# liuyuan-pal/Gen6D

Hardware: AMD Instinct MI355X
Metric: query images/sec (detect+select+3x refine), 64 ref views (higher is better)
Workload: dtype f32

## Files before the change

gen6d_amd/csrc/conv_igemm.hip:

```cpp
#include "g6d_common.h"
#include <type_traits>
#include <stdlib.h>

#define LDS_K 36
#define BK 32
#ifndef G6D_ABLATE
#define G6D_ABLATE 0
#endif

bool g6d_wino_eligible(const G6dConv& d);
int g6d_wino_launch(const G6dConv& d, hipStream_t stream);
bool g6d_wino43_eligible(const G6dConv& d);
int g6d_wino43_launch(const G6dConv& d, hipStream_t stream);
bool g6d_conv_patch_eligible(const G6dConv& d);
int g6d_conv_patch_launch(const G6dConv& d, int M, hipStream_t stream);

namespace {

__device__ __forceinline__ f32x4 ldg(const float* __restrict__ base, int elem_off) {
  return *reinterpret_cast<const f32x4*>(reinterpret_cast<const char*>(base) + ((unsigned)elem_off << 2));
}

template <int BM, int BN, int WGM, int WGN, int MODE, int MM>
__global__ void __launch_bounds__(256, 2) conv_igemm_kernel(const G6dConv p, const int M, const int T,
                                                         const int nChunks, const int itersPerSplit,
                                                         const int totalIters, const int splits, const unsigned in_bytes,
                                                         const unsigned w_bytes, const unsigned mul_bytes, const int pm_hw,
                                                         const int pm_tiles, const int pm_ny_count) {
  extern __shared__ __attribute__((aligned(16))) float lds[];
  constexpr int WM = BM / WGM, WN = BN / WGN;
  constexpr int MT = WM / 32, NT = WN / 32;
  constexpr int RA = BM / 32, RB = BN / 32;
  constexpr int STAGE = (BM + BN) * LDS_K;
  constexpr bool AFF = MODE != 0, PER_N = MODE == 2 || MODE == 4, MUL = MODE == 3 || MODE == 4;

  const int tid = threadIdx.x;
  const int lane = tid & 63, wave = tid >> 6;
  const int wm = wave / WGN, wn = wave % WGN;
  const int li = lane & 31, lh = lane >> 5;
  const int lrow = tid >> 3, lseg = tid & 7;

  int pm_pos = 0, pm_tile = blockIdx.x, pm_ny = blockIdx.y;
  if (pm_hw > 0) {
    const int per = 8 * pm_ny_count * pm_hw, g = blockIdx.x / per, r = blockIdx.x - g * per;
    const int m8 = min(8, pm_tiles - 8 * g);
    const int r2 = r / m8;
    pm_tile = 8 * g + (r - r2 * m8);
    pm_pos = r2 / pm_ny_count; pm_ny = r2 - pm_pos * pm_ny_count;
  }
  const int m0 = pm_tile * BM, n0 = pm_ny * BN;
  auto row_m = [&](int r) { return pm_hw > 0 ? (m0 + r) * pm_hw + pm_pos : m0 + r; };
  int ky0 = 0, ky1 = p.kh - 1, kx0 = 0, kx1 = p.kw - 1;
  if (pm_hw > 0) {
    const int oy = pm_pos / p.Wo, ox = pm_pos - oy * p.Wo;
    ky0 = max(0, p.ph - oy); ky1 = min(p.kh - 1, p.Hi - 1 + p.ph - oy);
    kx0 = max(0, p.pw - ox); kx1 = min(p.kw - 1, p.Wi - 1 + p.pw - ox);
  }
  const int it_begin = blockIdx.z * itersPerSplit;
  const int it_end = pm_hw > 0 ? p.kd * (ky1 - ky0 + 1) * (kx1 - kx0 + 1) * nChunks : min(totalIters, it_begin + itersPerSplit);

  const int Cin = p.Cin, khw = p.kh * p.kw;
  const float* __restrict__ gsc = p.in_scale;
  const float* __restrict__ gsh = p.in_shift;
  const int relu = p.in_relu;

  const int pad_a = ((p.pd * p.Hi + p.ph) * p.Wi + p.pw) * p.ld_in;
  const int pad_m = (p.ph * p.Wi + p.pw) * Cin;
  unsigned amz[RA], amy[RA], amx[RA], avoff[RA], mvoff[MUL ? RA : 1];
  int nbase[PER_N ? RA : 1];
#pragma unroll
  for (int j = 0; j < RA; ++j) {
    const int m = row_m(lrow + 32 * j);
    amz[j] = amy[j] = amx[j] = 0u; avoff[j] = 0u;
    if constexpr (MUL) mvoff[j] = 0u;
    if constexpr (PER_N) nbase[j] = 0;
    if (m < M) {
      const int ow = m % p.Wo, t1 = m / p.Wo;
      const int oh = t1 % p.Ho, t2 = t1 / p.Ho;
      const int od = t2 % p.Do, n = t2 / p.Do;
      const int az0 = od * p.sd - p.pd, ay0 = oh * p.sh - p.ph, ax0 = ow * p.sw - p.pw;
      for (int k = 0; k < p.kd; ++k) amz[j] |= (unsigned)((unsigned)(az0 + k) < (unsigned)p.Di) << k;
      for (int k = 0; k < p.kh; ++k) amy[j] |= (unsigned)((unsigned)(ay0 + k) < (unsigned)p.Hi) << k;
      for (int k = 0; k < p.kw; ++k) amx[j] |= (unsigned)((unsigned)(ax0 + k) < (unsigned)p.Wi) << k;
      const int n_in = p.in_image_mod > 0 ? n % p.in_image_mod : n;
      avoff[j] = (unsigned)((((n_in * p.Di + az0) * p.Hi + ay0) * p.Wi + ax0) * p.ld_in + pad_a + 4 * lseg) << 2;
      if constexpr (MUL) {
        const int mg = p.mul_group_images > 0 ? n / p.mul_group_images : 0;
        mvoff[j] = (unsigned)(((mg * p.Hi + ay0) * p.Wi + ax0) * Cin + pad_m + 4 * lseg) << 2;
      }
      if constexpr (PER_N) nbase[j] = (n / p.in_affine_per_n) * Cin;
    }
  }
  unsigned bvoff[RB];
#pragma unroll
  for (int j = 0; j < RB; ++j) {
    const int co = n0 + lrow + 32 * j;
    bvoff[j] = co < p.Cout ? (unsigned)(co * T * Cin + 4 * lseg) << 2 : 0x80000000u;
  }
  const auto rs_in = __builtin_amdgcn_make_buffer_rsrc(const_cast<float*>(p.in) - pad_a, 0, in_bytes, 0x00020000);
  const auto rs_w = __builtin_amdgcn_make_buffer_rsrc(const_cast<float*>(p.weight), 0, w_bytes, 0x00020000);
  const auto rs_mul = __builtin_amdgcn_make_buffer_rsrc(const_cast<float*>(MUL ? p.mul - pad_m : p.in), 0, mul_bytes, 0x00020000);
  const unsigned thr_last = 4 * lseg < Cin - 32 * (nChunks - 1) ? 0xffffffffu : 0u;

  f32x16 acc[MT][NT];
#pragma unroll
  for (int i = 0; i < MT; ++i)
#pragma unroll
    for (int j = 0; j < NT; ++j)
#pragma unroll
      for (int r = 0; r < 16; ++r) acc[i][j][r] = 0.f;

  f32x4 ra[2][RA], rm[2][MUL ? RA : 1], rb[2][RB], rsc[2][PER_N ? RA : 1], rsh[2][PER_N ? RA : 1];
  unsigned va[2][AFF ? RA : 1];

  int lt = it_begin;
  int cc = pm_hw > 0 ? 0 : it_begin / T;
  const int tap0 = it_begin - cc * T;
  int kz = pm_hw > 0 ? 0 : tap0 / khw, ky = pm_hw > 0 ? ky0 : (tap0 - kz * khw) / p.kw, kx = pm_hw > 0 ? kx0 : tap0 - kz * khw - ky * p.kw;
  auto advance = [&]() {
    lt += 1;
    kx += 1; const bool w1 = kx > kx1; kx = w1 ? kx0 : kx;
    ky += w1; const bool w2 = ky > ky1; ky = w2 ? ky0 : ky;
    kz += w2; const bool w3 = kz == p.kd; kz = w3 ? 0 : kz;
    cc += w3;
  };

  typedef unsigned u32x4 __attribute__((ext_vector_type(4)));
  auto bload = [&](const auto& rs, unsigned voff, int soff) {
    return __builtin_bit_cast(f32x4, __builtin_bit_cast(u32x4, __builtin_amdgcn_raw_buffer_load_b128(rs, voff, soff, 0)));
  };
  int toff = 0, moff = 0, cch = 0, woff = 0;
  unsigned cm = 0;
  bool cv = false;
  auto begin_step = [&](auto S) {
    constexpr int s = decltype(S)::value;
    const bool live = lt < it_end;
    cch = cc * BK + 4 * lseg;
    cv = (cch < Cin) & live;
    cm = live ? (cc == nChunks - 1 ? thr_last : 0xffffffffu) : 0u;
    toff = live ? (((kz * p.Hi + ky) * p.Wi + kx) * p.ld_in + cc * BK) << 2 : 0;
    moff = live ? ((ky * p.Wi + kx) * Cin + cc * BK) << 2 : 0;
    woff = live ? (((kz * p.kh + ky) * p.kw + kx) * Cin + cc * BK) << 2 : 0;
    if constexpr (AFF && !PER_N) { rsc[s][0] = ldg(gsc, cv ? cch : 0); rsh[s][0] = ldg(gsh, cv ? cch : 0); }
  };
  auto load_a = [&](auto S, int j) {
    constexpr int s = decltype(S)::value;
    const unsigned m = (unsigned)__builtin_amdgcn_sbfe(amz[j], kz, 1) & (unsigned)__builtin_amdgcn_sbfe(amy[j], ky, 1) &
                       (unsigned)__builtin_amdgcn_sbfe(amx[j], kx, 1) & cm;
    if constexpr (AFF) va[s][j] = m;
    ra[s][j] = bload(rs_in, (avoff[j] & m) | (~m & 0x80000000u), toff);
    if constexpr (MUL) rm[s][j] = bload(rs_mul, (mvoff[j] & m) | (~m & 0x80000000u), moff);
    if constexpr (PER_N) { rsc[s][j] = ldg(gsc, cv ? nbase[j] + cch : 0); rsh[s][j] = ldg(gsh, cv ? nbase[j] + cch : 0); }
  };
  auto load_b = [&](auto S, int j) {
    constexpr int s = decltype(S)::value;
    rb[s][j] = bload(rs_w, bvoff[j], woff);
  };
  auto store_a = [&](auto S, float* As, int j) {
    constexpr int s = decltype(S)::value;
    f32x4 v = ra[s][j];
    if constexpr (MUL) v *= rm[s][j];
    if constexpr (AFF) {
      v = v * rsc[s][PER_N ? j : 0] + rsh[s][PER_N ? j : 0];
      if (relu) {
#pragma unroll
        for (int e = 0; e < 4; ++e) asm("v_max_f32 %0, 0, %1" : "=v"(v[e]) : "v"(v[e]));
      }
      u32x4 b = __builtin_bit_cast(u32x4, v);
      b &= va[s][j];
      v = __builtin_bit_cast(f32x4, b);
    }
    *reinterpret_cast<f32x4*>(As + (lrow + 32 * j) * LDS_K + 4 * lseg) = v;
  };
  auto store_b = [&](auto S, float* Bs, int j) {
    constexpr int s = decltype(S)::value;
    *reinterpret_cast<f32x4*>(Bs + (lrow + 32 * j) * LDS_K + 4 * lseg) = rb[s][j];
  };

  f32x4 dummy = {0.f, 0.f, 0.f, 0.f};
  f32x4 fa[2][MT], fb[2][NT];
  auto read_frags = [&](const float* As, const float* Bs, int kc) {
#pragma unroll
    for (int i = 0; i < MT; ++i)
      fa[kc & 1][i] = *reinterpret_cast<const f32x4*>(As + (wm * WM + i * 32 + li) * LDS_K + kc * 8 + 4 * lh);
#pragma unroll
    for (int j = 0; j < NT; ++j)
      fb[kc & 1][j] = *reinterpret_cast<const f32x4*>(Bs + (wn * WN + j * 32 + li) * LDS_K + kc * 8 + 4 * lh);
  };
  constexpr bool ONE_ACC = MT * NT == 1;
  f32x16 acc_odd;
  if constexpr (ONE_ACC) {
#pragma unroll
    for (int r = 0; r < 16; ++r) acc_odd[r] = 0.f;
  }
  auto mfma_q = [&](int q) {
    const int kc = q / (4 * MT * NT), r = q % (4 * MT * NT);
    const int sidx = r / (MT * NT), i = (r % (MT * NT)) / NT, j = r % NT;
    if constexpr (ONE_ACC) {
      if (sidx & 1) { acc_odd = __builtin_amdgcn_mfma_f32_32x32x2f32(fa[kc & 1][0][sidx], fb[kc & 1][0][sidx], acc_odd, 0, 0, 0); return; }
    }
    acc[i][j] = __builtin_amdgcn_mfma_f32_32x32x2f32(fa[kc & 1][i][sidx], fb[kc & 1][j][sidx], acc[i][j], 0, 0, 0);
  };

  constexpr int NMFMA = MT * NT * 16, NP = NMFMA / 2, QPC = NMFMA / 4 / 2;
  constexpr int NROW = RA + RB;
  static_assert(NP >= NROW, "tile too small for the piece schedule");
  auto k_step = [&](auto PAR, const float* As, const float* Bs, float* An, float* Bn) {
    constexpr int par = decltype(PAR)::value;
    using SL = std::integral_constant<int, par>;
    using SS = std::integral_constant<int, par ^ 1>;
    if constexpr (MM != 0) {
#pragma unroll
      for (int j = 0; j < RA; ++j) load_a(SL{}, j);
#pragma unroll
      for (int j = 0; j < RB; ++j) load_b(SL{}, j);
#pragma unroll
      for (int kp = 0; kp < 2; ++kp) {
        f32x4 a0[MT], a1[MT], b0[NT], b1[NT];
#pragma unroll
        for (int i = 0; i < MT; ++i) {
          a0[i] = *reinterpret_cast<const f32x4*>(As + (wm * WM + i * 32 + li) * LDS_K + (2 * kp) * 8 + 4 * lh);
          a1[i] = *reinterpret_cast<const f32x4*>(As + (wm * WM + i * 32 + li) * LDS_K + (2 * kp + 1) * 8 + 4 * lh);
        }
#pragma unroll
        for (int j = 0; j < NT; ++j) {
          b0[j] = *reinterpret_cast<const f32x4*>(Bs + (wn * WN + j * 32 + li) * LDS_K + (2 * kp) * 8 + 4 * lh);
          b1[j] = *reinterpret_cast<const f32x4*>(Bs + (wn * WN + j * 32 + li) * LDS_K + (2 * kp + 1) * 8 + 4 * lh);
        }
#pragma unroll
        for (int i = 0; i < MT; ++i)
#pragma unroll
          for (int j = 0; j < NT; ++j) acc[i][j] = g6d_mfma_lowp<MM>(a0[i], a1[i], b0[j], b1[j], acc[i][j]);
      }
#pragma unroll
      for (int j = 0; j < RA; ++j) store_a(SS{}, An, j);
#pragma unroll
      for (int j = 0; j < RB; ++j) store_b(SS{}, Bn, j);
      advance(); begin_step(SS{});
      return;
    }
    read_frags(As, Bs, 0);
#pragma unroll
    for (int pc = 0; pc < NP; ++pc) {
      if (pc % QPC == 0 && pc / QPC < 3 && (G6D_ABLATE < 2 || G6D_ABLATE >= 6)) read_frags(As, Bs, pc / QPC + 1);
      mfma_q(2 * pc); mfma_q(2 * pc + 1);
      if (G6D_ABLATE < 1 || G6D_ABLATE >= 6) {
        if (pc < RA) load_a(SL{}, pc); else if (pc < NROW) load_b(SL{}, pc - RA);
        const int sr = pc - (NP - NROW);
        if (sr >= 0) {
          if (G6D_ABLATE == 6) {
            if (sr < RA) dummy += ra[par ^ 1][sr]; else dummy += rb[par ^ 1][sr - RA];
          } else if (sr < RA) store_a(SS{}, An, sr); else store_b(SS{}, Bn, sr - RA);
        }
        if (pc == NP - 1) { advance(); begin_step(SS{}); }
      }
      __builtin_amdgcn_sched_barrier(0);
    }
  };

  if (it_begin < it_end) {
    using S0 = std::integral_constant<int, 0>;
    using S1 = std::integral_constant<int, 1>;
    begin_step(S0{});
#pragma unroll
    for (int j = 0; j < RA; ++j) load_a(S0{}, j);
#pragma unroll
    for (int j = 0; j < RB; ++j) load_b(S0{}, j);
    advance(); begin_step(S1{});
#pragma unroll
    for (int j = 0; j < RA; ++j) load_a(S1{}, j);
#pragma unroll
    for (int j = 0; j < RB; ++j) load_b(S1{}, j);
#pragma unroll
    for (int j = 0; j < RA; ++j) store_a(S0{}, lds, j);
#pragma unroll
    for (int j = 0; j < RB; ++j) store_b(S0{}, lds + BM * LDS_K, j);
    advance(); begin_step(S0{});
    __syncthreads();
    float* L0 = lds; float* L1 = lds + STAGE;
    for (int it = it_begin; it < it_end; it += 2) {
      k_step(S0{}, L0, L0 + BM * LDS_K, L1, L1 + BM * LDS_K);
      if (G6D_ABLATE < 3 || G6D_ABLATE == 6) __syncthreads();
      if (it + 1 < it_end) {
        k_step(S1{}, L1, L1 + BM * LDS_K, L0, L0 + BM * LDS_K);
        if (G6D_ABLATE < 3 || G6D_ABLATE == 6) __syncthreads();
      }
    }
    if (G6D_ABLATE == 6) acc[0][0][0] += dummy[0] + dummy[1] + dummy[2] + dummy[3];
  }

  if constexpr (ONE_ACC) {
#pragma unroll
    for (int r = 0; r < 16; ++r) acc[0][0][r] += acc_odd[r];
  }
  const int Cout = p.Cout;
  if (splits > 1) {
    constexpr int TILE = BM * BN;
    constexpr int PIECES = MT * NT * 4;
    constexpr int ZU = 16 / PIECES;
    const int ntiles = gridDim.x * gridDim.y, tile = blockIdx.y * gridDim.x + blockIdx.x;
    float* part = p.workspace + G6D_WS_COUNTERS + (size_t)tile * TILE + tid * 4;
    const size_t zstride = (size_t)ntiles * TILE;
    float* mine = part + blockIdx.z * zstride;
#pragma unroll
    for (int i = 0; i < MT; ++i)
#pragma unroll
      for (int j = 0; j < NT; ++j)
#pragma unroll
        for (int q = 0; q < 4; ++q)
          g6d_store_wt(mine + ((i * NT + j) * 4 + q) * 1024,
                       f32x4{acc[i][j][4 * q], acc[i][j][4 * q + 1], acc[i][j][4 * q + 2], acc[i][j][4 * q + 3]});
    if (!g6d_split_arrive(reinterpret_cast<int*>(p.workspace) + tile, splits, reinterpret_cast<int*>(lds))) return;
    __syncthreads();
    f32x4 sum[PIECES];
#pragma unroll
    for (int k = 0; k < PIECES; ++k) sum[k] = f32x4{0.f, 0.f, 0.f, 0.f};
    for (int z0 = 0; z0 < splits; z0 += ZU) {
      f32x4 v[ZU][PIECES];
#pragma unroll
      for (int u = 0; u < ZU; ++u) {
        const float* src = part + (size_t)min(z0 + u, splits - 1) * zstride;
#pragma unroll
        for (int k = 0; k < PIECES; ++k) v[u][k] = *reinterpret_cast<const f32x4*>(src + k * 1024);
      }
#pragma unroll
      for (int u = 0; u < ZU; ++u)
        if (z0 + u < splits) {
#pragma unroll
          for (int k = 0; k < PIECES; ++k) sum[k] += v[u][k];
        }
    }
#pragma unroll
    for (int i = 0; i < MT; ++i)
#pragma unroll
      for (int j = 0; j < NT; ++j)
#pragma unroll
        for (int q = 0; q < 4; ++q) {
          const f32x4 t = sum[(i * NT + j) * 4 + q];
          acc[i][j][4 * q] = t[0]; acc[i][j][4 * q + 1] = t[1]; acc[i][j][4 * q + 2] = t[2]; acc[i][j][4 * q + 3] = t[3];
        }
  }

  const bool do_stats = p.stats != nullptr;
  const int rpg = p.stat_rows_per_group;
  const int mlast = pm_hw > 0 ? min(row_m(BM - 1), M - pm_hw + pm_pos) : min(m0 + BM, M) - 1;
  const int g0 = rpg > 0 ? row_m(0) / rpg : 0;
  const bool one_group = rpg <= 0 || (mlast / rpg) == g0;
  float* sred = lds;
  if (do_stats && one_group) {
    for (int i = tid; i < BN * 2; i += 256) sred[i] = 0.f;
    __syncthreads();
  }
#pragma unroll
  for (int j = 0; j < NT; ++j) {
    const int col = n0 + wn * WN + j * 32 + li;
    const bool cval = col < Cout;
    const float bv = (p.bias && cval) ? p.bias[col] : 0.f;
    float s1 = 0.f, s2 = 0.f;
#pragma unroll
    for (int i = 0; i < MT; ++i) {
#pragma unroll
      for (int r = 0; r < 16; ++r) {
        const int row = row_m(wm * WM + i * 32 + (r & 3) + 8 * (r >> 2) + 4 * lh);
        float v = apply_act(acc[i][j][r] + bv, p.out_act);
        if (row < M && cval) {
          p.out[(size_t)row * p.ld_out + col] = v;
          if (do_stats) {
            if (one_group) { s1 += v; s2 += v * v; }
            else {
              double* st = p.stats + ((size_t)(row / rpg) * Cout + col) * 2;
              atomicAdd(st, (double)v); atomicAdd(st + 1, (double)v * v);
            }
          }
        }
      }
    }
    if (do_stats && one_group) {
      s1 += __shfl_xor(s1, 32, 64);
      s2 += __shfl_xor(s2, 32, 64);
      if (lh == 0) {
        atomicAdd(&sred[(wn * WN + j * 32 + li) * 2], s1);
        atomicAdd(&sred[(wn * WN + j * 32 + li) * 2 + 1], s2);
      }
    }
  }
  if (do_stats && one_group) {
    __syncthreads();
    if (tid < BN && n0 + tid < Cout) {
      double* st = p.stats + ((size_t)g0 * Cout + n0 + tid) * 2;
      atomicAdd(st, (double)sred[tid * 2]);
      atomicAdd(st + 1, (double)sred[tid * 2 + 1]);
    }
  }
  if (do_stats && p.fin_scale) {
    __syncthreads();
    g6d_finalize_stats(g6d_fin_of(p), gridDim.x * gridDim.y, reinterpret_cast<int*>(lds));
  }
}

bool igemm_position_major(const G6dConv& d, int bm, int splits) {
  const int pm = (int)g6d_knob(G6D_KNOB_CONV_PM);
  return pm != 0 && (pm == 2 || d.in_scale != nullptr) && splits == 1 && d.Di == 1 && d.Do == 1 && d.kd == 1 && d.sh == 1 && d.sw == 1 && d.Ho == d.Hi &&
         d.Wo == d.Wi && d.Ho * d.Wo <= 64 && d.Ho * d.Wo > 1 && (d.kh > 1 || d.kw > 1) && d.kh == 2 * d.ph + 1 && d.kw == 2 * d.pw + 1 &&
         d.N >= 4 * bm;
}

template <int BM, int BN, int WGM, int WGN, int MODE, int MM>
int launch_mm(const G6dConv& d, int M, int T, int nChunks, int splits, hipStream_t stream) {
  const int total = T * nChunks;
  const int ips = (total + splits - 1) / splits;
  splits = (total + ips - 1) / ips;
  const bool pm = igemm_position_major(d, BM, splits);
  const int pm_hw = pm ? d.Ho * d.Wo : 0, pm_tiles = pm ? (d.N + BM - 1) / BM : 0;
  const int ny = (d.Cout + BN - 1) / BN;
  dim3 grid(pm ? pm_hw * pm_tiles * ny : (M + BM - 1) / BM, pm ? 1 : ny, splits);
  const size_t lds_bytes = 2 * (size_t)(BM + BN) * LDS_K * sizeof(float);
  g6d_allow_lds(reinterpret_cast<const void*>(&conv_igemm_kernel<BM, BN, WGM, WGN, MODE, MM>), (int)lds_bytes);
  const long long pad_a = ((long long)(d.pd * d.Hi + d.ph) * d.Wi + d.pw) * d.ld_in, pad_m = (long long)(d.ph * d.Wi + d.pw) * d.Cin;
  const long long n_in = d.in_image_mod > 0 ? d.in_image_mod : d.N;
  const long long n_mul = d.mul_group_images > 0 ? (d.N + d.mul_group_images - 1) / d.mul_group_images : 1;
  const unsigned in_bytes = (unsigned)((n_in * d.Di * d.Hi * d.Wi * d.ld_in + pad_a) * 4);
  const unsigned w_bytes = (unsigned)((long long)d.Cout * T * d.Cin * 4);
  const unsigned mul_bytes = (unsigned)((n_mul * d.Hi * d.Wi * d.Cin + pad_m) * 4);
  hipLaunchKernelGGL((conv_igemm_kernel<BM, BN, WGM, WGN, MODE, MM>), grid, dim3(256), lds_bytes, stream, d, M, T, nChunks,
                     ips, total, splits, in_bytes, w_bytes, mul_bytes, pm_hw, pm_tiles, ny);
  return g6d_check_launch("conv_igemm");
}

template <int BM, int BN, int WGM, int WGN, int MODE>
int launch_mode(const G6dConv& d, int M, int T, int nChunks, int splits, hipStream_t stream) {
  if (d.math_mode == 1) return launch_mm<BM, BN, WGM, WGN, MODE, 1>(d, M, T, nChunks, splits, stream);
  if (d.math_mode == 2) return launch_mm<BM, BN, WGM, WGN, MODE, 2>(d, M, T, nChunks, splits, stream);
  return launch_mm<BM, BN, WGM, WGN, MODE, 0>(d, M, T, nChunks, splits, stream);
}

template <int BM, int BN, int WGM, int WGN>
int launch_cfg(const G6dConv& d, int M, int T, int nChunks, int splits, hipStream_t stream) {
  if (d.mul) return d.in_affine_per_n ? launch_mode<BM, BN, WGM, WGN, 4>(d, M, T, nChunks, splits, stream)
                                      : launch_mode<BM, BN, WGM, WGN, 3>(d, M, T, nChunks, splits, stream);
  if (!d.in_scale) return launch_mode<BM, BN, WGM, WGN, 0>(d, M, T, nChunks, splits, stream);
  if (d.in_affine_per_n) return launch_mode<BM, BN, WGM, WGN, 2>(d, M, T, nChunks, splits, stream);
  return launch_mode<BM, BN, WGM, WGN, 1>(d, M, T, nChunks, splits, stream);
}

constexpr int NARROW_RUN = 8;
__global__ void __launch_bounds__(256) conv_narrow_kernel(const float* __restrict__ in, const float* __restrict__ w, const float* __restrict__ bias,
                                                         float* __restrict__ out, int NH, int H, int W, int Cin, int ld_in, int Cout, int ld_out,
                                                         int act, int runs_per_row, int nruns) {
  const int lane = threadIdx.x & 63;
  const int c4 = lane * 4;
  const bool on = c4 < Cin;
  f32x4 wr[4][9];
#pragma unroll
  for (int co = 0; co < 4; ++co)
#pragma unroll
    for (int t = 0; t < 9; ++t)
      wr[co][t] = (on && co < Cout) ? *reinterpret_cast<const f32x4*>(w + ((long)co * 9 + t) * Cin + c4) : f32x4{0.f, 0.f, 0.f, 0.f};
  const int wave = __builtin_amdgcn_readfirstlane((int)((blockIdx.x * blockDim.x + threadIdx.x) >> 6)), nwaves = (gridDim.x * blockDim.x) >> 6;
  const f32x4 zero = {0.f, 0.f, 0.f, 0.f};
  for (int run = wave; run < nruns; run += nwaves) {
    const int g = run / runs_per_row, x0 = (run - g * runs_per_row) * NARROW_RUN;
    const int y = g % H;
    const float* rowp[3];
    bool rv[3];
#pragma unroll
    for (int ky = 0; ky < 3; ++ky) {
      const int yy = y + ky - 1;
      rv[ky] = yy >= 0 && yy < H;
      rowp[ky] = in + ((long)(g + ky - 1) * W) * ld_in + c4;
    }
    auto column = [&](int x, f32x4 (&col)[3]) {
      const bool xv = x >= 0 && x < W;
#pragma unroll
      for (int ky = 0; ky < 3; ++ky) col[ky] = (on && xv && rv[ky]) ? *reinterpret_cast<const f32x4*>(rowp[ky] + (long)x * ld_in) : zero;
    };
    f32x4 win[3][3];
    column(x0 - 1, win[0]);
    column(x0, win[1]);
#pragma unroll
    for (int i = 0; i < NARROW_RUN; ++i) {
      const int x = x0 + i;
      column(x + 1, win[2]);
      float acc[4];
#pragma unroll
      for (int co = 0; co < 4; ++co) {
        f32x4 a = zero;
#pragma unroll
        for (int ky = 0; ky < 3; ++ky)
#pragma unroll
          for (int kx = 0; kx < 3; ++kx) a += win[kx][ky] * wr[co][3 * ky + kx];
        acc[co] = (a[0] + a[1]) + (a[2] + a[3]);
      }
#pragma unroll
      for (int off = 32; off >= 1; off >>= 1)
#pragma unroll
        for (int co = 0; co < 4; ++co) acc[co] += __shfl_xor(acc[co], off, 64);
      if (lane == 0 && x < W) {
#pragma unroll
        for (int co = 0; co < 4; ++co)
          if (co < Cout) {
            float v = acc[co] + (bias ? bias[co] : 0.f);
            if (act == 1) v = fmaxf(v, 0.f);
            else if (act == 2) v = v > 0.f ? v : 0.1f * v;
            out[((long)g * W + x) * ld_out + co] = v;
          }
      }
#pragma unroll
      for (int ky = 0; ky < 3; ++ky) { win[0][ky] = win[1][ky]; win[1][ky] = win[2][ky]; }
    }
  }
}

bool conv_narrow_eligible(const G6dConv& d) {
  return g6d_knob(G6D_KNOB_CONV_NARROW) != 0 && d.Cout <= 4 && d.Cin <= 256 && d.kd == 1 && d.kh == 3 && d.kw == 3 && d.sd == 1 && d.sh == 1 && d.sw == 1 &&
         d.pd == 0 && d.ph == 1 && d.pw == 1 && d.Di == 1 && d.Do == 1 && d.Ho == d.Hi && d.Wo == d.Wi && !d.mul && !d.in_scale && !d.stats &&
         !d.in_image_mod && d.out_act >= 0 && d.out_act <= 2;
}

int conv_narrow_launch(const G6dConv& d, hipStream_t stream) {
  const int rpr = (d.Wi + NARROW_RUN - 1) / NARROW_RUN;
  const long nruns = (long)d.N * d.Hi * rpr;
  if (nruns >= (1l << 31)) { g6d_set_error("conv (narrow): too many pixel runs"); return G6D_EINVAL; }
  const int blocks = (int)((nruns + 3) / 4 < 2048 ? (nruns + 3) / 4 : 2048);
  hipLaunchKernelGGL(conv_narrow_kernel, dim3(blocks), dim3(256), 0, stream, d.in, d.weight, d.bias, d.out, d.N * d.Hi, d.Hi, d.Wi, d.Cin, d.ld_in, d.Cout,
                     d.ld_out, d.out_act, rpr, (int)nruns);
  return g6d_check_launch("conv_narrow");
}

}

extern "C" int g6d_conv_plan(const G6dConv* desc) {
  if (!desc) return G6D_EINVAL;
  if (conv_narrow_eligible(*desc)) return 4;
  if (g6d_wino43_eligible(*desc)) return 3;
  if (g6d_wino_eligible(*desc)) return 2;
  const bool use_patch = g6d_knob(G6D_KNOB_CONV_PATCH) != 0;
  return (use_patch && g6d_conv_patch_eligible(*desc)) ? 1 : 0;
}

extern "C" int g6d_conv_igemm(const G6dConv* desc, g6d_stream_t stream_) {
  if (!desc) return G6D_EINVAL;
  const G6dConv& d = *desc;
  hipStream_t stream = reinterpret_cast<hipStream_t>(stream_);
  if (!d.in || !d.weight || !d.out) { g6d_set_error("conv: null pointer"); return G6D_EINVAL; }
  if (d.math_mode < 0 || d.math_mode > 2) { g6d_set_error("conv: math_mode must be 0 (fp32), 1 (bf16) or 2 (fp16)"); return G6D_EINVAL; }
  if (d.N <= 0 || d.Cin <= 0 || d.Cout <= 0 || d.Do <= 0 || d.Ho <= 0 || d.Wo <= 0 || d.kd <= 0 || d.kh <= 0 || d.kw <= 0) {
    g6d_set_error("conv: bad shape"); return G6D_EINVAL;
  }
  if ((d.Cin & 3) || (d.ld_in & 3) || d.ld_in < d.Cin || d.ld_out < d.Cout) { g6d_set_error("conv: Cin/ld_in must be multiples of 4"); return G6D_EINVAL; }
  if (!g6d_aligned16(d.in) || !g6d_aligned16(d.weight) || (d.mul && !g6d_aligned16(d.mul)) ||
      (d.in_scale && (!g6d_aligned16(d.in_scale) || !d.in_shift || !g6d_aligned16(d.in_shift)))) {
    g6d_set_error("conv: operand pointers must be 16-byte aligned"); return G6D_EINVAL;
  }
  if (d.mul && !d.in_scale) { g6d_set_error("conv: mul requires in_scale/in_shift"); return G6D_EINVAL; }
  if (d.in_affine_per_n < 0 || d.in_image_mod < 0 || d.mul_group_images < 0 || (d.mul_group_images > 0 && !d.mul) ||
      d.in_image_mod > d.N) {
    g6d_set_error("conv: in_affine_per_n / in_image_mod / mul_group_images must be >= 0 (mul_group_images needs mul; in_image_mod <= N)");
    return G6D_EINVAL;
  }
  if ((long long)(d.mul_group_images > 0 ? (d.N + d.mul_group_images - 1) / d.mul_group_images : 1) * d.Hi * d.Wi * d.Cin >= (1ll << 29)) {
    g6d_set_error("conv: multiplier tensor exceeds 2^31 bytes"); return G6D_EINVAL;
  }
  if (d.fin_scale && (!d.stats || !d.fin_shift || !d.fin_counter || d.fin_count <= 0 || d.fin_groups <= 0)) {
    g6d_set_error("conv: fin_scale needs stats, fin_shift, fin_counter, fin_count > 0 and fin_groups"); return G6D_EINVAL;
  }
  if ((long long)(d.in_image_mod > 0 ? d.in_image_mod : d.N) * d.Di * d.Hi * d.Wi * d.ld_in + ((long long)(d.pd * d.Hi + d.ph) * d.Wi + d.pw) * d.ld_in >= (1ll << 29) ||
      (long long)d.Cout * d.kd * d.kh * d.kw * d.Cin >= (1ll << 29) || d.kd > 32 || d.kh > 32 || d.kw > 32) {
    g6d_set_error("conv: tensor exceeds 2^31 bytes (buffer-load offsets) or kernel extent > 32"); return G6D_EINVAL;
  }
  const long long Mll = (long long)d.N * d.Do * d.Ho * d.Wo;
  if (Mll > (1ll << 30)) { g6d_set_error("conv: M too large"); return G6D_EINVAL; }
  const int M = (int)Mll;
  if (conv_narrow_eligible(d)) return conv_narrow_launch(d, stream);
  if (g6d_wino43_eligible(d)) return g6d_wino43_launch(d, stream);
  if (g6d_wino_eligible(d)) return g6d_wino_launch(d, stream);
  const bool use_patch = g6d_knob(G6D_KNOB_CONV_PATCH) != 0;
  if (use_patch && g6d_conv_patch_eligible(d)) return g6d_conv_patch_launch(d, M, stream);
  const int T = d.kd * d.kh * d.kw;
  const int nChunks = (d.Cin + BK - 1) / BK;
  const int total = T * nChunks;

  int bm = 128, bn = d.Cout <= 32 ? 32 : (d.Cout <= 64 ? 64 : 128);
  if (bn == 128 && (d.mul || (d.in_scale && d.in_affine_per_n))) bn = 64;
  if (M <= 64 && d.Cout > 32) { bm = 64; bn = 64; }
  const bool tile_policy = g6d_knob(G6D_KNOB_TILE_POLICY) != 0;
  bool no_split = false;
  if (tile_policy && d.Cout > 32 && bm == 128 && d.split_k <= 0) {
    const long long blocks128 = (long long)((M + 127) / 128) * ((d.Cout + bn - 1) / bn);
    const long long blocks64 = (long long)((M + 63) / 64) * ((d.Cout + 63) / 64);
    if (blocks128 < 256) {
      if (blocks64 >= 256) { bm = 64; bn = 64; no_split = true; }
      else if (M >= 2048) { bm = 64; bn = 64; }
      else if (M <= 1024 && bn == 128) bn = 64;
    }
  }
  const long long blocks = (long long)((M + bm - 1) / bm) * ((d.Cout + bn - 1) / bn);

  int splits = d.split_k;
  if (splits <= 0) {
    splits = 1;
    const int split_target = (int)g6d_knob(G6D_KNOB_SPLIT_TARGET);
    if (blocks < (split_target < 256 ? split_target : 256) && total >= 8 && !no_split) {
      splits = (int)((split_target + blocks - 1) / blocks);
      if (splits > total / 4) splits = total / 4;
      if (splits > 64) splits = 64;
      if (splits < 1) splits = 1;
    }
  }
  if (splits > total) splits = total;
  if (splits > 1) {
    const size_t per = (size_t)blocks * bm * bn * sizeof(float);
    const size_t room = d.workspace && d.workspace_bytes > G6D_WS_COUNTER_BYTES ? d.workspace_bytes - G6D_WS_COUNTER_BYTES : 0;
    if (room < (size_t)splits * per || blocks > G6D_WS_COUNTERS) {
      if (d.split_k > 1) { g6d_set_error("conv: workspace too small for forced split_k"); return G6D_ENOSPC; }
      splits = blocks > G6D_WS_COUNTERS ? 1 : (int)(room / per);
      if (splits < 2) splits = 1;
    }
  }
  if (bm == 64) return launch_cfg<64, 64, 2, 2>(d, M, T, nChunks, splits, stream);
  if (bn == 32) return launch_cfg<128, 32, 4, 1>(d, M, T, nChunks, splits, stream);
  if (bn == 64) return launch_cfg<128, 64, 2, 2>(d, M, T, nChunks, splits, stream);
  return launch_cfg<128, 128, 2, 2>(d, M, T, nChunks, splits, stream);
}
```

gen6d_amd/lib.py:

```python
import ctypes as C
import os

_HERE = os.path.dirname(os.path.abspath(__file__))
LIB_PATH = os.path.join(_HERE, "libgen6d_hip.so")

G6D_ERRORS = {-1: "G6D_EINVAL", -2: "G6D_ENOSPC", -3: "G6D_ELAUNCH"}


class G6dWinoSeg(C.Structure):
    _fields_ = [("in_", C.c_void_p), ("out_full", C.c_void_p), ("out_pool", C.c_void_p),
                ("N", C.c_int32), ("H", C.c_int32), ("W", C.c_int32), ("ld_in", C.c_int32), ("ld_full", C.c_int32), ("ld_pool", C.c_int32)]


class G6dConv16Seg(C.Structure):
    _fields_ = [("in_", C.c_void_p), ("out_full", C.c_void_p), ("out_pool", C.c_void_p),
                ("N", C.c_int32), ("D", C.c_int32), ("H", C.c_int32), ("W", C.c_int32), ("ld_in", C.c_int32), ("ld_full", C.c_int32),
                ("ld_pool", C.c_int32)]


class G6dRange16(C.Structure):
    _fields_ = [("exps", C.c_void_p), ("rec", C.c_void_p), ("slot_in", C.c_int32), ("slot_out", C.c_int32)]


class G6dCorrSeg(C.Structure):
    _fields_ = [("in_", C.c_void_p), ("out", C.c_void_p), ("H", C.c_int32), ("W", C.c_int32), ("ld_in", C.c_int32), ("ld_out", C.c_int32),
                ("N", C.c_int32), ("reserved_", C.c_int32)]


class G6dFrame(C.Structure):
    _fields_ = [("plane0", C.c_void_p), ("plane1", C.c_void_p), ("pitch0", C.c_int32), ("pitch1", C.c_int32), ("width", C.c_int32),
                ("height", C.c_int32), ("format", C.c_int32), ("rotate", C.c_int32), ("matrix", C.c_int32), ("slot", C.c_int32),
                ("out_w", C.c_int32), ("out_h", C.c_int32), ("K", C.c_float * 9)]


class G6dMesh(C.Structure):
    _fields_ = [("nodes", C.c_void_p), ("nx", C.c_int32), ("ny", C.c_int32), ("step_log2", C.c_int32), ("reserved", C.c_int32)]


class G6dSink(C.Structure):
    _fields_ = [("plane0", C.c_void_p), ("plane1", C.c_void_p), ("pitch0", C.c_int32), ("pitch1", C.c_int32), ("width", C.c_int32),
                ("height", C.c_int32), ("format", C.c_int32), ("matrix", C.c_int32), ("slot", C.c_int32), ("pic_w", C.c_int32),
                ("pic_h", C.c_int32), ("thickness", C.c_int32), ("dot_radius", C.c_int32), ("line_rgb", C.c_int32), ("dot_rgb", C.c_int32),
                ("box", C.c_int32)]


class G6dConv(C.Structure):
    _fields_ = [
        ("in_", C.c_void_p), ("mul", C.c_void_p), ("in_scale", C.c_void_p), ("in_shift", C.c_void_p),
        ("weight", C.c_void_p), ("bias", C.c_void_p), ("out", C.c_void_p), ("stats", C.c_void_p),
        ("workspace", C.c_void_p), ("workspace_bytes", C.c_size_t),
        ("N", C.c_int32), ("Di", C.c_int32), ("Hi", C.c_int32), ("Wi", C.c_int32), ("Cin", C.c_int32), ("ld_in", C.c_int32),
        ("Do", C.c_int32), ("Ho", C.c_int32), ("Wo", C.c_int32), ("Cout", C.c_int32), ("ld_out", C.c_int32),
        ("kd", C.c_int32), ("kh", C.c_int32), ("kw", C.c_int32),
        ("sd", C.c_int32), ("sh", C.c_int32), ("sw", C.c_int32),
        ("pd", C.c_int32), ("ph", C.c_int32), ("pw", C.c_int32),
        ("in_relu", C.c_int32), ("in_affine_per_n", C.c_int32), ("out_act", C.c_int32),
        ("stat_rows_per_group", C.c_int32), ("split_k", C.c_int32), ("math_mode", C.c_int32),
        ("weight_wino", C.c_void_p),
        ("fin_scale", C.c_void_p), ("fin_shift", C.c_void_p), ("fin_counter", C.c_void_p),
        ("fin_count", C.c_double), ("fin_eps", C.c_double), ("fin_groups", C.c_int32),
        ("in_image_mod", C.c_int32), ("mul_group_images", C.c_int32), ("reserved_", C.c_int32),
        ("weight_wino16", C.c_void_p), ("weight_wino43", C.c_void_p),
    ]


_P, _I, _F, _D = C.c_void_p, C.c_int, C.c_float, C.c_double

SIGNATURES = {
    "g6d_marker": [_I, _P],
    "g6d_conv_igemm": [C.POINTER(G6dConv), _P],
    "g6d_conv_plan": [C.POINTER(G6dConv)],
    "g6d_corr2d_patch": [_P, _I, _I, _I, _I, _P, _I, _I, _I, _P, _I, _P, C.c_size_t, _I, _P],
    "g6d_corr2d_patch_multi": [_P, _I, _I, _P, _I, _I, _I, _P, C.c_size_t, _I, _P],
    "g6d_corr2d_wino_multi": [_P, _I, _I, _P, _I, _I, _P, C.c_size_t, _P],
    "g6d_corr2d_patch16_multi": [_P, _I, _I, _P, _I, _I, _I, _P, C.c_size_t, _I, _P],
    "g6d_stats_finalize": [_P, _I, _D, _D, _P, _P, _P],
    "g6d_affine_act_pool": [_P, _I, _P, _P, _I, _I, _I, _I, _I, _I, _I, _P, _I, _P],
    "g6d_upsample_bilinear": [_P, _I, _P, _P, _I, _I, _I, _I, _I, _I, _P, _I, _P],
    "g6d_bias_relu_pool_nchw": [_P, _P, _I, _I, _I, _I, _I, _I, _P, _P],
    "g6d_vgg_conv1_pool": [_P, _I, _I, _I, _P, _P, _I, _I, _P, _P],
    "g6d_vgg_conv1_pool_nhwc": [_P, _I, _I, _I, _P, _P, _I, _I, _P, _P],
    "g6d_vgg_conv1_pool_nhwc16": [_P, _I, _I, _I, _P, _P, _I, _I, _P, _P, _P, _I, _P],
    "g6d_conv16_direct_multi": [_P, _I, _I, _P, _I, _F, _P, _I, _I, _I, _I, _I, _I, _P, _I, _P],
    "g6d_corr16_multi": [_P, _I, _I, _P, _F, _I, _I, _I, _P],
    "g6d_product_split16": [_P, _P, _P, _P, _P, _I, _I, _I, _I, _I, _P],
    "g6d_affine_split16": [_P, _I, _P, _P, _I, _I, _I, _I, _I, _I, _I, _P, _I, _P],
    "g6d_vgg_conv1_pool_nhwc16_ex": [_P, _I, _I, _I, _P, _P, _I, _I, _P, _P, _P, _I, _P, _P],
    "g6d_conv16_direct_multi_ex": [_P, _I, _I, _P, _I, _F, _P, _I, _I, _I, _I, _I, _I, _P, _I, _P, _P],
    "g6d_corr16_multi_ex": [_P, _I, _I, _P, _F, _I, _I, _I, _P, _P],
    "g6d_product_split16_ex": [_P, _P, _P, _P, _P, _I, _I, _I, _I, _I, _P, _P],
    "g6d_affine_split16_ex": [_P, _I, _P, _P, _I, _I, _I, _I, _I, _I, _I, _P, _I, _P, _P],
    "g6d_conv16_direct_plan": [_P, _I, _I, _P, _I, _I, _I, _I, _I, _I, _P, _I],
    "g6d_affine_split16_to": [_P, _I, _P, _P, _I, _I, _I, _I, _I, _I, _I, _P, _I, _I, _I, _I, _P, _P],
    "g6d_upsample_bilinear_split16": [_P, _I, _P, _P, _I, _I, _I, _I, _I, _I, _P, _I, _I, _I, _I, _P, _P],
    "g6d_l2norm_split16": [_P, _I, _I, _I, _P, _I, _P, _P],
    "g6d_vgg_conv1_pool_nhwc_norm": [_P, _I, _I, _I, _P, _P, _I, _I, _P, _P, _P, _P],
    "g6d_wino_conv3x3": [_P, _I, _I, _I, _I, _I, _P, _P, _I, _I, _P, _I, _P, _I, _P, C.c_size_t, _P],
    "g6d_wino_conv3x3_multi": [_P, _I, _I, _P, _P, _I, _I, _P, C.c_size_t, _P],
    "g6d_wino16_conv3x3_multi": [_P, _I, _I, _P, _P, _I, _I, _I, _P, C.c_size_t, _P],
    "g6d_wino43_conv3x3_multi": [_P, _I, _I, _P, _P, _I, _I, _P, C.c_size_t, _P],
    "g6d_corr2d_wino43_multi": [_P, _I, _I, _P, _I, _I, _P, C.c_size_t, _P],
    "g6d_l2norm_rows": [_P, _I, _I, _I, _P],
    "g6d_nchw_to_nhwc": [_P, _I, _I, _I, _I, _I, _P, _I, _P],
    "g6d_selector_ref_sums": [_P, _I, _I, _I, _P, _P, _P],
    "g6d_selector_prod_affine": [_P, _P, _P, _I, _I, _I, _D, _P, _P, _P],
    "g6d_selector_scan": [_P, _P, _I, _I, _I, _P, _P, _P],
    "g6d_selector_levels": [_I, _I, _P, _P, _P, _P, _P, _I, _I, _I, _D, _P, _P, _P, _P, _P],
    "g6d_refiner_volume": [_P, _P, _P, _P, _I, _I, _I, _I, _I, _I, _I, _P, _P, _P],
    "g6d_refiner_volume_kp": [_P, _P, _P, _P, _P, _P, _I, _I, _I, _I, _I, _I, _I, _P, _P, _I, _P],
    "g6d_refiner_volume_kp_pairs": [_P, _P, _P, _P, _P, _P, _I, _I, _I, _I, _I, _I, _I, _P, _P, _I, _P, _P, _P],
    "g6d_detector_assemble": [_P, _P, _P, _I, _I, _I, C.POINTER(C.c_float), _F, _I, _I, _I, _I, _P, _I, _P],
    "g6d_detector_score_mlp_max": [_P, _I, _I, _I, _P, _P, _P, _P, _P, _P],
    "g6d_detector_decode": [_P, _I, _P, _I, _P, _I, _I, _I, _I, _P, _I, _P],
    "g6d_resize_bilinear_pyramid": [_P, _I, _I, _I, _I, C.POINTER(C.c_int), C.POINTER(C.c_int), C.POINTER(C.c_void_p), _P],
    "g6d_zero_bytes": [_P, C.c_size_t, _P],
    "g6d_vps_norm": [_P, _I, _P, _I, _I, _I, _P],
    "g6d_max_an_add": [_P, _I, _I, _I, _I, _P, _P, _I, _I, _P],
    "g6d_attention": [_P, _P, _P, _I, _I, _I, _I, _P, _I, _I, _P],
    "g6d_layernorm": [_P, _I, _I, _I, _P, _P, _F, _P, _I, _P],
    "g6d_affine_act_add": [_P, _I, _P, _P, _I, _P, _I, _I, _I, _P, _I, _I, _P],
    "g6d_linear_gemv": [_P, _I, _I, _P, _P, _I, _I, _P, _P],
    "g6d_linear_gemv_batch": [_P, _I, _I, _P, _P, _I, _I, _P, _P, C.c_size_t, _P],
    "g6d_chain_crop_from_detection": [_P, _F, _P, _I, _P],
    "g6d_chain_pose_from_selection": [_P, _P, _P, _I, _P, _P, _P, _P, _P, _P, _I, _P],
    "g6d_chain_refine_prepare": [_P, _P, _P, _F, _F, _P, _P, _I, _I, _P, _P, _F, _P, _I, _P],
    "g6d_chain_refine_update": [_P, _P, _P, _P, _I, _P, _P, _I, _P],
    "g6d_warp_batch": [_P, _P, _P, _I, _I, _I, _I, _P, _P, _I, _I, _P],
    "g6d_warp_perspective": [_P, _I, _I, _I, C.POINTER(C.c_float), _P, _I, _I, _I, _F, _P],
    "g6d_track_gather": [_P, _P, _P, _P, _I, _P],
    "g6d_track_commit": [_P, _P, _P, _I, _P, _I, _F, _P, _P, _P, _P, _P, _I, _P],
    "g6d_track_gate": [_P, _P, _P, _P, _I, _P],
    "g6d_track_health": [_P, _P, _P, _P, _I, _I, _P, _I, _P, _D, _I, _D, _D, _D, _D, _D, _D, _P, _P, _P, _P, _I, _P],
    "g6d_track_verify": [_P, _P, _P, _P, _P, _D, _D, _D, _D, _I, _P, _P, _I, _P],
    "g6d_frame_ingest": [_P, _I, _P, _I, _I, _I, _P, _P],
    "g6d_sizeof_frame_desc": [],
    "g6d_frame_ingest_mesh": [_P, _P, _I, _P, _I, _I, _I, _P, _P],
    "g6d_sizeof_mesh_desc": [],
    "g6d_track_corners": [_P, _P, _P, _P, _P, _P, _I, _P],
    "g6d_frame_emit": [_P, _I, _P, _I, _I, _I, _P, _P, _P],
    "g6d_sizeof_sink_desc": [],
    "g6d_frame_emit_source": [_P, _I, _P, _I, _P, _P, _I, _I, _I, _I, _P],
}

_lib = None


def load():
    global _lib
    if _lib is not None:
        return _lib
    if not os.path.exists(LIB_PATH):
        raise RuntimeError(f"{LIB_PATH} is missing: build it with `python __graft_entry__.py` "
                           "(make -C gen6d_amd/csrc). There is no fallback path.")
    import torch
    lib = C.CDLL(LIB_PATH)
    for name, args in SIGNATURES.items():
        fn = getattr(lib, name)
        fn.argtypes = args
        fn.restype = C.c_int
    lib.g6d_abi_version.restype = C.c_int
    lib.g6d_sizeof_conv_desc.restype = C.c_int
    if lib.g6d_sizeof_conv_desc() != C.sizeof(G6dConv):
        raise RuntimeError("libgen6d_hip.so: G6dConv layout differs from the ctypes binding (stale build?)")
    if lib.g6d_sizeof_frame_desc() != C.sizeof(G6dFrame):
        raise RuntimeError("libgen6d_hip.so: G6dFrame layout differs from the ctypes binding (stale build?)")
    if lib.g6d_sizeof_mesh_desc() != C.sizeof(G6dMesh):
        raise RuntimeError("libgen6d_hip.so: G6dMesh layout differs from the ctypes binding (stale build?)")
    if lib.g6d_sizeof_sink_desc() != C.sizeof(G6dSink):
        raise RuntimeError("libgen6d_hip.so: G6dSink layout differs from the ctypes binding (stale build?)")
    lib.g6d_last_error.restype = C.c_char_p
    lib.g6d_set_knob.argtypes, lib.g6d_set_knob.restype = [C.c_char_p, C.c_double], C.c_int
    lib.g6d_get_knob.argtypes, lib.g6d_get_knob.restype = [C.c_char_p], C.c_double
    lib.g6d_reset_knobs.argtypes, lib.g6d_reset_knobs.restype = [], None
    _lib = lib
    return lib


def set_knob(name, value):
    check(load().g6d_set_knob(name.encode(), float(value)), f"g6d_set_knob({name})")


def get_knob(name):
    return load().g6d_get_knob(name.encode())


def reset_knobs():
    load().g6d_reset_knobs()


def check(rc, what):
    if rc != 0:
        msg = load().g6d_last_error().decode()
        raise RuntimeError(f"{what} failed: {G6D_ERRORS.get(rc, rc)} ({msg})")
```

gen6d_amd/network/refiner.py:

```python
import numpy as np
import torch
import torch.nn.functional as F

from .. import ops, specs
from .backbone import pack_trunk, trunk_features
from .operator import pose_apply_th
from .params import ParamBank, fold_vgg

F43_MIN_QUERIES = 4
FEATNET_F43_LAYERS = {("conv1", 0), ("conv_out", 0), ("conv_out", 3)}
FEATNET_PAIR_BRANCHES = ("conv0", "conv1", "conv2", "conv_out")
VOLUME_PAIR_LAYERS = ("mean_embed", "var_embed", "conv0", "conv2")
VOLUME_F43_LAYERS = ("conv0",)
MAX_BATCH = 32
_K3, _P3 = (3, 3, 3), (1, 1, 1)
_K2, _P2 = (1, 3, 3), (0, 1, 1)


_LIN = {}


def _linspace(sn, dev):
    key = (sn, str(dev))
    if key not in _LIN:
        _LIN[key] = torch.linspace(-1, 1, sn, dtype=torch.float32, device=dev)
    return _LIN[key]


class RefFeatureCache:

    def __init__(self, max_entries=2048):
        from collections import OrderedDict
        self.store, self.max_entries = OrderedDict(), max_entries
        self.hits = self.misses = 0

    def get(self, key):
        f = self.store.get(key)
        if f is None:
            self.misses += 1
            return None
        self.store.move_to_end(key)
        self.hits += 1
        return f

    def put(self, key, feat):
        self.store[key] = feat
        while len(self.store) > self.max_entries:
            self.store.popitem(last=False)

    def clear(self):
        self.store.clear()
        self.hits = self.misses = 0

    @property
    def hit_rate(self):
        return self.hits / max(1, self.hits + self.misses)


class VolumeRefiner(ParamBank):
    default_cfg = {"refiner_sample_num": 32, "ref_feat_cache_deg": 0.0, "lowp_keep_fp32": (), "lowp_only": None}

    def __init__(self, cfg):
        self.cfg = {**self.default_cfg, **cfg}
        super().__init__(specs.refiner_rows())
        self.ref_database = None
        self.ref_ids = None
        self.feat_cache = RefFeatureCache()

    def load_state_dict(self, *a, **k):
        self.feat_cache.clear()
        return super().load_state_dict(*a, **k)

    def _mm(self, *names):
        only = self.cfg.get("lowp_only")
        keep = self.cfg.get("lowp_keep_fp32") or ()
        fp32 = (not any(n in only for n in names)) if only is not None else any(n in keep for n in names)
        return ops.math_mode("fp32" if fp32 else None, inherit_if_none=True)

    def angle_step(self):
        return float(np.radians(self.cfg.get("ref_feat_cache_deg") or 0.0))

    def cached_ref_feats(self, keys, make_imgs):
        with ops.math_mode(self.cfg.get("math_mode"), inherit_if_none=True):
            keys = [(k, ops.MATH_MODE) for k in keys]
            got = [self.feat_cache.get(k) for k in keys]
            miss = [i for i, f in enumerate(got) if f is None]
            feats = self.run_feature_net(make_imgs(miss), f43=False) if miss else None
        if miss:
            for j, i in enumerate(miss):
                got[i] = feats[j].clone()
                self.feat_cache.put(keys[i], got[i])
        return torch.stack(got, 0)

    def _pack(self):
        if self._packed is None:
            pk = {"vgg": pack_trunk(fold_vgg(self, "feature_net.backbone.features"))}
            for name in ("conv0", "conv1", "conv2", "conv_out"):
                pk[name] = [self.conv_w(f"feature_net.{name}.{i}", wino_kd=1, f43=(name, i) in FEATNET_F43_LAYERS) for i in (0, 3)]
            for name in ("mean_embed", "var_embed", "conv5"):
                pk["v_" + name] = [self.conv_w(f"volume_net.{name}.{i}", wino_kd=0 if name == "conv5" else 3, f43=True) for i in (0, 3)]
            for name in ("conv0", "conv1", "conv2", "conv3", "conv4"):
                pk["v_" + name] = self.conv_w(f"volume_net.{name}.0", wino_kd=3 if name in ("conv0", "conv2", "conv4") else 0,
                                              f43=name in VOLUME_F43_LAYERS)
            w = self.p("regressor.fc.0.0.weight")
            pk["fc0"] = (w.reshape(512, 512, 64).permute(0, 2, 1).reshape(512, 32768).contiguous(),
                         self.p("regressor.fc.0.0.bias").contiguous())
            pk["fc1"] = (self.p("regressor.fc.1.0.weight").contiguous(), self.p("regressor.fc.1.0.bias").contiguous())
            heads = ("fcr", "fct", "fcs")
            pk["heads"] = (torch.cat([self.p(f"regressor.{h}.weight") for h in heads], 0).contiguous(),
                           torch.cat([self.p(f"regressor.{h}.bias") for h in heads], 0).contiguous())
            self._packed = pk
        return self._packed

    def run_feature_net(self, imgs, f43=None):
        pk = self._pack()
        n, _, h, w = imgs.shape
        dev = imgs.device
        big = (n >= F43_MIN_QUERIES * 7) if f43 is None else bool(f43)
        rng = self._pair_rng()
        on16 = self._featnet_pair_branches(n, h, w) if (big and rng is not None) else ()
        with self._mm("trunk"):
            f3, f5, f7 = trunk_features(pk["vgg"], imgs, ("c3", "c5", "c7_pre"), False, f43=big, rng=rng, pairs=self.pairs_on)

        def tap(name, f, slot):
            if name in on16:
                return ops.l2norm_split16(f[:, 0], 3, rng=(rng, rng.slot(slot)))
            ops.l2norm_rows(f)
            return f

        def pair(name, x):
            if name in on16:
                return pair16(name, x)
            (w0, b0), (w1, b1) = pk[name]
            u0, u1 = pk[name][0].u, pk[name][1].u
            v0, v1 = (pk[name][0].u43, pk[name][1].u43) if big else (None, None)
            _, _, hh, ww, _ = x.shape
            y0 = torch.empty((n, 1, hh, ww, w0.shape[0]), dtype=torch.float32, device=dev)
            s0 = ops.new_stats(n, w0.shape[0], dev)
            y1 = torch.empty((n, 1, hh, ww, w1.shape[0]), dtype=torch.float32, device=dev)
            s1 = ops.new_stats(n, w1.shape[0], dev)
            sc0, sh0 = ops.conv(x, w0, b0, y0, ksize=_K2, pad=_P2, stats=s0, rows_per_group=hh * ww, w_wino=u0, w_wino43=v0, finalize=hh * ww)
            sc1, sh1 = ops.conv(y0, w1, b1, y1, ksize=_K2, pad=_P2, in_scale=sc0, in_shift=sh0, in_relu=True, per_n=True,
                                stats=s1, rows_per_group=hh * ww, w_wino=u1, w_wino43=v1, finalize=hh * ww)
            return y1, sc1, sh1

        def pair16(name, x):
            _, hh, ww, _, _ = x.shape

            def conv16(layer, xin):
                co = layer[0].shape[0]
                y = torch.empty((n, 1, hh, ww, co), dtype=torch.float32, device=dev)
                st = ops.new_stats(n, co, dev)
                ops.conv16_direct_multi([xin], layer.w16(3), layer[1], relu=False, full=torch.float32, stats=st, rows_per_group=hh * ww,
                                        out_full=[y[:, 0]])
                return (y,) + ops.stats_finalize(st, hh * ww)

            y0, sc0, sh0 = conv16(pk[name][0], x)
            mid = ops.affine_split16(y0, sc0, sh0, 1, True, False, 3, rng=(rng, rng.slot(f"featnet.{name}.mid")))
            return conv16(pk[name][1], mid)

        hq, wq = h // 4, w // 4
        cat16 = "conv_out" in on16
        cat = ops.new_map16(n, hq, wq, 192, 3, dev, rng=(rng, rng.slot("featnet.cat"))) if cat16 else \
            torch.empty((n, 1, hq, wq, 192), dtype=torch.float32, device=dev)

        def branch(name, f, slot, c_off, factor):
            y, sc, sh = pair(name, tap(name, f, slot))
            if cat16:
                if factor == 1:
                    ops.affine_split16_to(y, sc, sh, 1, False, 3, cat, c_off)
                else:
                    ops.upsample_bilinear_split16(y, cat, c_off, factor, sc, sh, 1, 3)
            elif factor == 1:
                ops.affine_act_pool(y, cat[..., c_off:c_off + 64], sc, sh, per_n=True)
            else:
                ops.upsample_bilinear(y, cat[..., c_off:c_off + 64], factor, sc, sh, per_n=True)

        with self._mm("featnet"):
            ops.fork_join([lambda: branch("conv0", f3, "featnet.f3", 0, 1), lambda: branch("conv1", f5, "featnet.f5", 64, 2),
                           lambda: branch("conv2", f7, "featnet.f7", 128, 4)], dev)
            y, sc, sh = pair("conv_out", cat)
        out = torch.empty((n, 1, hq, wq, 128), dtype=torch.float32, device=dev)
        ops.affine_act_pool(y, out, sc, sh, per_n=True)
        return out.view(n, hq, wq, 128)

    def _featnet_pair_branches(self, n, h, w):
        key = (n, h, w)
        memo = self.__dict__.setdefault("_featnet16", {})
        if key not in memo:
            shapes = {"conv0": (4, 256, 64, 64), "conv1": (8, 512, 256, 64), "conv2": (16, 512, 256, 64), "conv_out": (4, 192, 128, 128)}

            def fits(name):
                d, ci, cm, co = shapes[name]
                hh, ww = h // d, w // d
                return all(ops.conv16_direct_plan(n, hh, ww, a, b, 3, stats_rows=hh * ww) in (1, 2) for a, b in ((ci, cm), (cm, co)))
            memo[key] = tuple(name for name in FEATNET_PAIR_BRANCHES if h % 16 == 0 and w % 16 == 0 and fits(name))
        return memo[key]

    def volume_pair_route(self, qn, sn):
        if qn < F43_MIN_QUERIES or self._pair_rng() is None or not {"mean_embed", "var_embed"} <= set(VOLUME_PAIR_LAYERS):
            return False
        memo = self.__dict__.setdefault("_volume16", {})
        key = (qn, sn, tuple(VOLUME_PAIR_LAYERS))
        if key not in memo:
            shapes = [(sn, 256, 64), (sn, 128, 64), (sn, 64, 64)] + ([(sn, 128, 64)] if "conv0" in VOLUME_PAIR_LAYERS else []) + \
                ([(sn // 2, 128, 128)] if "conv2" in VOLUME_PAIR_LAYERS else [])
            memo[key] = all(ops.conv16_direct_plan(qn, s, s, ci, co, 3, stats_rows=s ** 3, D=s) == 1 for s, ci, co in shapes)
        return memo[key]

    def feature_volumes(self, feats, ref_Ks, ref_poses, K_in, pose_in, h_in, w_in, sn):
        dev = feats.device
        lin = _linspace(sn, dev)
        C = feats.shape[-1]
        args = (feats, ref_Ks.contiguous(), ref_poses.contiguous(), K_in.contiguous(), pose_in.contiguous(), lin, h_in, w_in)
        if feats.dim() == 5 and self.volume_pair_route(feats.shape[0], sn):
            rng = self._pair_rng()
            return ops.refiner_volume_kp_pairs(*args, rng_mean=(rng, rng.slot("volume.mean_in")), rng_std=(rng, rng.slot("volume.std")))
        lead = (feats.shape[0],) if feats.dim() == 5 else ()
        mean_in = torch.empty(lead + (sn ** 3, 2 * C), dtype=torch.float32, device=dev)
        std = torch.empty(lead + (sn ** 3, C), dtype=torch.float32, device=dev)
        return ops.refiner_volume_kp(*args, mean_in, std)

    def run_volume_net(self, mean_in, std, sn):
        pk = self._pack()
        pairs_in = isinstance(mean_in, ops.PairMap)
        dev = mean_in.data.device if pairs_in else mean_in.device
        batched = pairs_in or mean_in.dim() == 3
        qn = mean_in.shape[0] if batched else 1
        pn = 1 if qn > 1 else 0

        def c3(x, wb, out, stride=1, aff=None, stats_c=None, count=None):
            st = ops.new_stats(qn, stats_c, dev) if stats_c else None
            sc, sh = aff if aff is not None else (None, None)
            return ops.conv(x, wb[0], wb[1], out, ksize=_K3, stride=(stride,) * 3, pad=_P3, in_scale=sc, in_shift=sh,
                            in_relu=aff is not None, per_n=pn if aff is not None else 0, stats=st,
                            rows_per_group=pn * (count or 0) if stats_c else 0,
                            w_wino=getattr(wb, "u", None) if stride == 1 else None,
                            w_wino43=getattr(wb, "u43", None) if (stride == 1 and qn >= F43_MIN_QUERIES) else None,
                            finalize=count if stats_c else None)

        def buf(s, c):
            return torch.empty((qn, s, s, s, c), dtype=torch.float32, device=dev)

        vox = sn ** 3
        rng = self._pair_rng() if pairs_in else None
        cat16 = pairs_in and "conv0" in VOLUME_PAIR_LAYERS
        cat = ops.new_map16(qn * sn, sn, sn, 128, 3, dev, rng=(rng, rng.slot("volume.cat"))) if cat16 else buf(sn, 128)

        def c16(layer, xin, y, stats_c=None, count=vox):
            st = ops.new_stats(qn, stats_c, dev) if stats_c else None
            ops.conv16_direct_multi([xin], layer.w16(3, layout=2), layer[1], relu=False, full=torch.float32, kd=3, stats=st,
                                    rows_per_group=count if stats_c else 0, out_full=[y])
            return ops.stats_finalize(st, count) if stats_c else None

        def embed(name, x, c_off):
            if pairs_in:
                return embed16(name, x, c_off)
            y = buf(sn, 64)
            aff = c3(x, pk[name][0], y, stats_c=64, count=vox)
            c3(y, pk[name][1], cat[..., c_off:c_off + 64], aff=aff)

        def embed16(name, x, c_off):
            y0 = buf(sn, 64)
            sc, sh = c16(pk[name][0], x, y0, stats_c=64)
            mid = ops.affine_split16(y0.view(qn * sn, 1, sn, sn, 64), sc, sh, sn, True, False, 3, rng=(rng, rng.slot(f"volume.{name[2:]}.mid")))
            if not cat16:
                c16(pk[name][1], mid.view(qn, sn, sn, sn, 2, 64), cat[..., c_off:c_off + 64])
                return
            y1 = buf(sn, 64)
            c16(pk[name][1], mid.view(qn, sn, sn, sn, 2, 64), y1)
            ops.affine_split16_to(y1.view(qn * sn, 1, sn, sn, 64), None, None, 0, False, 3, cat, c_off)

        with self._mm("embed"):
            embed("v_mean_embed", mean_in.view(qn, sn, sn, sn, 2, 256) if pairs_in else mean_in.view(qn, sn, sn, sn, 256), 0)
            embed("v_var_embed", std.view(qn, sn, sn, sn, 2, 128) if pairs_in else std.view(qn, sn, sn, sn, 128), 64)
        x, aff, s = cat, None, sn
        with self._mm("stack"):
            for name, co, stride in (("v_conv0", 64, 1), ("v_conv1", 128, 2), ("v_conv2", 128, 1), ("v_conv3", 256, 2),
                                     ("v_conv4", 256, 1)):
                s = s // stride
                y = buf(s, co)
                if name == "v_conv0" and cat16:
                    x, aff = y, c16(pk[name], cat.view(qn, sn, sn, sn, 2, 128), y, stats_c=co)
                    continue
                if name == "v_conv2" and pairs_in and "conv2" in VOLUME_PAIR_LAYERS:
                    xin = ops.affine_split16(x.view(qn * s, 1, s, s, 128), aff[0], aff[1], s, True, False, 3, rng=(rng, rng.slot("volume.conv2.in")))
                    x, aff = y, c16(pk[name], xin.view(qn, s, s, s, 2, 128), y, stats_c=co, count=s ** 3)
                    continue
                x, aff = y, c3(x, pk[name], y, stride=stride, aff=aff, stats_c=co, count=s ** 3)
        s = s // 2
        y = buf(s, 512)
        with self._mm("tail"):
            aff = c3(x, pk["v_conv5"][0], y, stride=2, aff=aff, stats_c=512, count=s ** 3)
            code = buf(s, 512)
            c3(y, pk["v_conv5"][1], code, aff=aff)
        return code.view(qn, s ** 3, 512) if batched else code.view(s ** 3, 512)

    def run_regressor(self, code):
        pk = self._pack()
        qn = code.shape[0] if code.dim() == 3 else 1
        x = ops.linear_gemv(code.reshape(qn, -1), pk["fc0"][0], pk["fc0"][1], act=2)
        x = ops.linear_gemv(x, pk["fc1"][0], pk["fc1"][1], act=2)
        o = ops.linear_gemv(x, pk["heads"][0], pk["heads"][1])
        ops.l2norm_rows(o[:, 0:4])
        return o[:, 0:4], o[:, 4:6], o[:, 6:7]

    def _step(self, *a, **k):
        with ops.math_mode(self.cfg.get("math_mode"), inherit_if_none=True):
            return self._step_fp(*a, **k)

    def _step_fp(self, que_img, K_in, pose_in, ref_imgs, ref_Ks, ref_poses, ref_feats=None):
        sn = self.cfg["refiner_sample_num"]
        dev = que_img.device
        ops.stats_arena_begin(dev)
        if ref_feats is not None:
            return self._step_from_feats(que_img, K_in, pose_in, ref_feats, ref_Ks, ref_poses)
        batched = ref_imgs.dim() == 5
        qn = ref_imgs.shape[0] if batched else 1
        rfn = ref_imgs.shape[-4]
        h_in, w_in = ref_imgs.shape[-2:]
        if batched:
            imgs = torch.cat([ref_imgs, que_img[:, None]], 1).reshape(qn * (rfn + 1), *ref_imgs.shape[-3:])
        else:
            imgs = torch.cat([ref_imgs, que_img], 0)
        feats = self.run_feature_net(imgs)
        feats = feats.contiguous()
        if batched:
            feats = feats.view(qn, rfn + 1, *feats.shape[1:])
        mean_in, std = self.feature_volumes(feats, ref_Ks, ref_poses, K_in, pose_in, h_in, w_in, sn)
        return self.run_regressor(self.run_volume_net(mean_in, std, sn))

    def _step_from_feats(self, que_img, K_in, pose_in, ref_feats, ref_Ks, ref_poses):
        sn = self.cfg["refiner_sample_num"]
        dev = que_img.device
        h_in, w_in = que_img.shape[-2:]
        batched = ref_feats.dim() == 5
        qf = self.run_feature_net(que_img)
        if batched:
            feats = torch.cat([ref_feats, qf[:, None]], 1).contiguous()
        else:
            feats = torch.cat([ref_feats, qf], 0).contiguous()
        mean_in, std = self.feature_volumes(feats, ref_Ks, ref_poses, K_in, pose_in, h_in, w_in, sn)
        return self.run_regressor(self.run_volume_net(mean_in, std, sn))

    def forward(self, data):
        is_inference = data["inference"] if "inference" in data else False
        que, ref = data["que_imgs_info"], data["ref_imgs_info"]
        qn_all = que["imgs"].shape[0]
        if qn_all == 1:
            outs = [self._step(que["imgs"], que["Ks_in"][0], que["poses_in"][0], ref["imgs"][0], ref["Ks"][0], ref["poses"][0])]
        else:
            outs = [self._step(que["imgs"][q0:q0 + MAX_BATCH], que["Ks_in"][q0:q0 + MAX_BATCH], que["poses_in"][q0:q0 + MAX_BATCH],
                               ref["imgs"][q0:q0 + MAX_BATCH], ref["Ks"][q0:q0 + MAX_BATCH], ref["poses"][q0:q0 + MAX_BATCH])
                    for q0 in range(0, qn_all, MAX_BATCH)]
        out = {"rotation": ops.cat1([o[0] for o in outs], 0), "offset": ops.cat1([o[1] for o in outs], 0),
               "scale": ops.cat1([o[2] for o in outs], 0)}
        if not is_inference:
            sn = self.cfg["refiner_sample_num"]
            g = torch.linspace(-1, 1, sn, dtype=torch.float32, device=que["imgs"].device)
            V = torch.stack(torch.meshgrid(g, g, g, indexing="ij"), -1).reshape(1, sn ** 3, 3) @ que["poses_in"][:, :3, :3]
            out["grids"] = pose_apply_th(que["poses_in"], V)
        return out

    def load_ref_imgs(self, ref_database, ref_ids):
        cache = getattr(self, "image_cache", None)
        if ref_database is not self.ref_database and cache is not None and not cache.holds(ref_database):
            cache.clear()
        if ref_database is not self.ref_database:
            self.feat_cache.clear()
        self.ref_database = ref_database
        self.ref_ids = ref_ids

    def refine_que_imgs(self, que_img, que_K, in_pose, size=128, ref_num=6, ref_even=False):
        from .. import estimator as E
        from .. import geometry as G
        margin, even_num = 0.05, min(128, len(self.ref_ids))
        dev = self.device_()
        cache = getattr(self, "image_cache", None)
        if cache is None:
            cache = self.image_cache = E.DeviceImageCache(dev)
        db = E.NormalizedDatabase(self.ref_database)
        in_pose = G.normalize_pose(np.asarray(in_pose, np.float64), db.scale, db.offset)
        center, diameter = db.object_center, db.object_diameter
        que_K = np.asarray(que_K, np.float64)
        _, new_f = G.let_me_look_at(in_pose, que_K, center)
        in_dist = np.linalg.norm(G.pose_inverse(in_pose)[:, 3] - center)
        scale = size * (1 - margin) / diameter * in_dist / new_f
        position = G.project_points(center[None], in_pose, que_K)[0][0]
        K_warp, pose_warp, pose_rect, H = G.look_at_crop_params(que_K, in_pose, position, 0, scale, size, size)
        if not torch.is_tensor(que_img):
            que_img = torch.from_numpy(np.ascontiguousarray(que_img)).to(dev)
        que_warp = ops.warp_perspective(que_img, H, size, size)
        ref_ids = E.select_reference_img_ids_refinement(db, center, self.ref_ids, pose_warp, ref_num, ref_even, even_num, cache)
        f = lambda a: torch.from_numpy(np.ascontiguousarray(a, dtype=np.float32)).to(dev)
        que_t = que_warp.float().div_(255).permute(2, 0, 1)[None].contiguous()
        step = self.angle_step()
        with torch.no_grad():
            out = self.range_guarded(lambda: self._refine_step(step, db, ref_ids, size, margin, pose_warp, K_warp, cache, que_t, f))
        quat, offset, scale_pr = out[:4], out[4:6], 2 ** out[6]
        pose_sim = G.compose_sim_pose(scale_pr, quat, offset, pose_warp, center)
        pose_pr = G.pose_sim_to_pose_rigid(pose_sim, pose_warp, K_warp, K_warp, center)
        pose_pr = G.pose_compose(pose_pr, G.pose_inverse(pose_rect))
        return G.denormalize_pose(pose_pr, db.scale, db.offset)

    def _range_fallback(self):
        self.feat_cache.clear()

    def _refine_step(self, step, db, ref_ids, size, margin, pose_warp, K_warp, cache, que_t, f):
        from .. import estimator as E
        if step > 0:
            ref_Ks, ref_poses, Hs, buckets = E.reference_view_params(db, ref_ids, size, margin, True, pose_warp, K_warp, angle_step=step)
            keys = [(id(self.ref_database), str(i), int(b), int(size)) for i, b in zip(ref_ids, buckets)]
            make = lambda miss: torch.stack([ops.warp_perspective(cache.get(db, ref_ids[k]), Hs[k], size, size) for k in miss], 0) \
                .float().div_(255).permute(0, 3, 1, 2).contiguous()
            ref_feats = self.cached_ref_feats(keys, make)
            rot, off, scl = self._step(que_t, f(K_warp), f(pose_warp), None, f(ref_Ks), f(ref_poses), ref_feats=ref_feats)
        else:
            ref_imgs, _, ref_Ks, ref_poses, _ = E.normalize_reference_views(db, ref_ids, size, margin, cache, True, pose_warp, K_warp,
                                                                         with_masks=False)
            rot, off, scl = self._step(que_t, f(K_warp), f(pose_warp), ref_imgs.float().div_(255).permute(0, 3, 1, 2).contiguous(),
                                       f(ref_Ks), f(ref_poses))
        return torch.cat([rot[0], off[0], scl[0]]).cpu().numpy()

    def refine_step_tensors(self, que_img_u8, K_in, pose_in, ref_imgs_u8, ref_Ks, ref_poses):
        dev = self.device_()
        f = lambda a: torch.from_numpy(np.ascontiguousarray(a, dtype=np.float32)).to(dev)
        q = torch.from_numpy(np.ascontiguousarray(que_img_u8)).to(dev).float().div_(255).permute(2, 0, 1)[None].contiguous()
        r = torch.from_numpy(np.ascontiguousarray(ref_imgs_u8)).to(dev).float().div_(255).permute(0, 3, 1, 2).contiguous()
        with torch.no_grad():
            rot, off, scl = self._step(q, f(K_in), f(pose_in), r, f(ref_Ks), f(ref_poses))
        return rot[0].cpu().numpy(), 2 ** scl[0].cpu().numpy(), off[0].cpu().numpy()
```

gen6d_amd/network/selector.py:

```python
import numpy as np
import torch
import torch.nn.functional as F

from .. import ops, parallel, specs
from .backbone import pack_trunk, trunk_features
from .params import ParamBank, fold_vgg

_CORR = (
    ((1, 1, 1, 0), (4, 1, 0, 1), (7, 1, 1, 0), (10, 1, 0, 1), (13, 1, 1, 0), (16, 0, 0, 0)),
    ((1, 1, 1, 0), (4, 1, 0, 1), (7, 1, 1, 0), (10, 0, 0, 0)),
    ((1, 1, 1, 0), (4, 0, 0, 0)),
)
_K133, _P011 = (1, 3, 3), (0, 1, 1)
MAX_BATCH = 32
FEAT_LD = 516


class ViewpointSelector(ParamBank):
    default_cfg = {"selector_angle_num": 5, "lowp_keep_fp32": ("trunk", "tail"), "lowp_only": None}

    def __init__(self, cfg):
        self.cfg = {**self.default_cfg, **cfg}
        super().__init__(specs.selector_rows(self.cfg["selector_angle_num"]))
        self.ref_feats_cache = None
        self.ref_sums = None
        self.ref_pose_embed = None
        self.rfn = self.an = None
        self.rank, self.world, self.group = 0, 1, None
        self.sharded = False
        self.r_begin, self.r_end = 0, None

    def set_shard(self, rank, world, group=None, force_collectives=False):
        self.rank, self.world, self.group = int(rank), int(world), group
        self.sharded = self.world > 1 or bool(force_collectives)

    def _allreduce(self, tensors):
        if not self.sharded:
            return
        flat = torch.cat([t.reshape(-1) for t in tensors])
        parallel.all_reduce_(flat, "sum", self.group)
        o = 0
        for t in tensors:
            t.copy_(flat[o:o + t.numel()].view_as(t)); o += t.numel()

    def _allgather_rows(self, rows, n_total):
        if not self.sharded:
            return rows
        return parallel.all_gather_ragged_rows(rows, n_total, self.world, self.group)

    def _allgather_batch(self, t, qn, n_local, n_total):
        if not self.sharded:
            return t
        F_ = t.shape[1]
        rows = t.view(qn, n_local, F_).permute(1, 0, 2).reshape(n_local, qn * F_).contiguous()
        return self._allgather_rows(rows, n_total).view(n_total, qn, F_).permute(1, 0, 2).reshape(qn * n_total, F_)

    def _pack(self):
        if self._packed is None:
            an = self.cfg["selector_angle_num"]
            pk = {"vgg": pack_trunk(fold_vgg(self, "backbone.features"))}
            pk["corr"] = [[self.conv_w(f"corr_conv_list.{l}.{i}", wino_kd=1) for i, *_ in layers] for l, layers in enumerate(_CORR)]
            pk["fuse0"] = self.conv_w("corr_feats_conv.0")
            pk["fuse3"] = self.conv_w("corr_feats_conv.3")
            pk["sp0"] = self.conv_w("score_process.0", cin_pad=FEAT_LD)
            pk["sp2"] = self.conv_w("score_process.2")
            pk["att"] = []
            for i in range(2):
                qkv = [self.conv_w(f"atts.{i}.{n}") for n in ("conv_query", "conv_key", "conv_feats")]
                pk["att"].append({
                    "qkv": (torch.cat([w for w, _ in qkv], 0).contiguous(), torch.cat([b for _, b in qkv], 0).contiguous()),
                    "merge": self.conv_w(f"atts.{i}.conv_merge"),
                    "ln": (self.p(f"atts.{i}.norm.norm.weight").contiguous(), self.p(f"atts.{i}.norm.norm.bias").contiguous()),
                    "mlp0": self.conv_w(f"mlps.{i}.0"), "mlp3": self.conv_w(f"mlps.{i}.3")})
            pk["pred0"] = self.conv_w("score_predict.0")
            pk["pred2"] = self.conv_w("score_predict.2")
            w, b = self.p("angle_predict.0.weight"), self.p("angle_predict.0.bias")
            w = w.reshape(512, 515, an).permute(0, 2, 1)
            w = F.pad(w, (0, FEAT_LD - 515)).reshape(512, 1, an * FEAT_LD).contiguous()
            pk["ang0"] = (w, b.contiguous())
            pk["ang2"] = self.conv_w("angle_predict.2")
            pk["ang4"] = self.conv_w("angle_predict.4")
            self._packed = pk
        return self._packed

    def _mm(self, *names):
        only = self.cfg.get("lowp_only")
        keep = self.cfg.get("lowp_keep_fp32") or ()
        fp32 = (not any(n in only for n in names)) if only is not None else any(n in keep for n in names)
        return ops.math_mode("fp32" if fp32 else None, inherit_if_none=True)

    def get_feats(self, imgs):
        with self._mm("trunk"):
            return trunk_features(self._pack()["vgg"], imgs, ("c5", "c7_pre", "p7"), True)

    def extract_ref_feats(self, ref_imgs, ref_poses, object_center, object_vert, is_train=False):
        if is_train:
            raise NotImplementedError("inference-only implementation (random object_forward is a training augmentation)")
        an, rfn, _, h, w = ref_imgs.shape
        if an != self.cfg["selector_angle_num"]:
            raise ValueError("number of rotations does not match selector_angle_num")
        self.rfn, self.an = rfn, an
        self.r_begin, self.r_end = parallel.shard_range(rfn, self.rank, self.world)
        if self.r_end == self.r_begin:
            raise ValueError("more ranks than reference views")
        ref_imgs = ref_imgs[:, self.r_begin:self.r_end]
        D = (self.r_end - self.r_begin) * an
        imgs = ref_imgs.permute(1, 0, 2, 3, 4).reshape(D, 3, h, w)
        dev = imgs.device
        cache = [torch.empty((D, 1, h >> s, w >> s, 512), dtype=torch.float32, device=dev) for s in (3, 4, 5)]
        for i0 in range(0, D, 64):
            feats = self.get_feats(imgs[i0:i0 + 64].contiguous())
            for l in range(3):
                cache[l][i0:i0 + 64].copy_(feats[l])
        self.ref_feats_cache = cache
        self.ref_sums = [ops.selector_ref_sums(c.view(D, -1, 512)) for c in cache]
        self._allreduce([t for pair in self.ref_sums for t in pair])

        cam = (-ref_poses[:, :3, :3].transpose(1, 2) @ ref_poses[:, :3, 3:])[..., 0] - object_center[None]
        fwd = cam[0]
        y = torch.linalg.cross(object_vert, fwd)
        x = torch.linalg.cross(y, object_vert)
        R = torch.stack([F.normalize(x, dim=0), F.normalize(y, dim=0), F.normalize(object_vert, dim=0)], 0)
        v = F.normalize(cam @ R.T, dim=1)
        for i in (0, 2, 4):
            v = F.linear(v, self.p(f"view_point_encoder.{i}.weight"), self.p(f"view_point_encoder.{i}.bias"))
            if i != 4: v = F.relu(v)
        self.ref_pose_embed = v.contiguous()

    def _level(self, l, q, cat, scale, shift, qn=1):
        pk = self._pack()
        cache = self.ref_feats_cache[l]
        D, _, h, w, _ = cache.shape
        dev = cache.device
        Dg = self.rfn * self.an
        grp = D if qn > 1 else 0
        x, mul, relu = cache, (q.view(qn, h, w, 512) if qn > 1 else q.view(h, w, 512)), False
        first = True
        layers = _CORR[l]
        for li, (idx, has_in, has_relu, has_pool) in enumerate(layers):
            wgt, bias = pk["corr"][l][li]
            wu = pk["corr"][l][li].u
            co = wgt.shape[0]
            last = li == len(layers) - 1
            out = cat[..., 256 * l:256 * l + 256] if last else torch.empty((qn * D, 1, h, w, co), dtype=torch.float32, device=dev)
            stats = ops.new_stats(qn, co, dev) if has_in else None
            fin = Dg * h * w if (has_in and not last and not self.sharded) else None
            with self._mm("product" if first else "stack", f"corr{l}.{li}"):
                mode16 = self._product16_mode(first, D * h * w, co) if first else self._stack16_mode(D * h * w, co, wgt.shape[2])
                if mode16 and not first:
                    x16 = ops.affine_split16(x, scale, shift, grp if scale is not None else 0, relu, False, mode16, **self._rng_kw(mode16, f"stack{l}.{li}"))
                    filt = pk["corr"][l][li].w16(mode16)
                    ci = wgt.shape[2]
                    per = max(1, ((1 << 31) - 1) // (D * h * w * ci * (4 if mode16 == 3 else 2)))
                    for q0 in range(0, qn, per):
                        q1 = min(qn, q0 + per)
                        ops.conv16_direct_multi([x16[q0 * D:q1 * D]], filt, bias, relu=False, full=torch.float32, pool=None,
                                                stats=stats[q0:q1] if stats is not None else None, rows_per_group=D * h * w,
                                                out_full=[out[q0 * D:q1 * D, 0]])
                    res, fin = out, None
                elif mode16:
                    prod = ops.product_split16(cache.view(D, h * w, 512), q.view(qn, h * w, 512), scale, shift, mode16, **self._rng_kw(mode16, f"prod{l}"))
                    prod = prod.view(qn * D, h, w, 2, 512) if mode16 == 3 else prod.view(qn * D, h, w, 512)
                    filt = pk["corr"][l][li].w16(mode16)
                    per = max(1, ((1 << 31) - 1) // (D * h * w * 512 * (4 if mode16 == 3 else 2)))
                    for q0 in range(0, qn, per):
                        q1 = min(qn, q0 + per)
                        ops.conv16_direct_multi([prod[q0 * D:q1 * D]], filt, bias, relu=False, full=torch.float32, pool=None, stats=stats[q0:q1],
                                                rows_per_group=D * h * w, out_full=[out[q0 * D:q1 * D]])
                    res, fin = out, None
                else:
                    res = ops.conv(x, wgt, bias, out, ksize=_K133, pad=_P011, mul=mul, in_scale=scale, in_shift=shift, in_relu=relu, stats=stats,
                                   w_wino=wu, finalize=fin, per_n=grp if scale is not None else 0, rows_per_group=grp * h * w,
                                   in_mod=grp if first else 0, mul_group=grp if mul is not None else 0)
            mul, first = None, False
            if last:
                break
            if fin is not None:
                scale, shift = res
            else:
                yield stats
                scale, shift = ops.stats_finalize(stats, Dg * h * w)
            if has_pool:
                pooled = torch.empty((qn * D, 1, h // 2, w // 2, co), dtype=torch.float32, device=dev)
                ops.affine_act_pool(out, pooled, scale, shift, per_n=grp, relu=bool(has_relu), pool=1)
                h, w = h // 2, w // 2
                x, scale, shift, relu = pooled, None, None, False
            else:
                x, relu = out, bool(has_relu)

    def _product16_mode(self, first, rows_per_query, co):
        if not (first and rows_per_query % 128 == 0):
            return 0
        mm = ops.MATH_MODE
        if mm == 0:
            return 3 if self.pairs_on else 0
        return mm if co % 128 == 0 else 0

    def _stack16_mode(self, rows_per_query, co, ci):
        if rows_per_query % 128:
            return 0
        mm = ops.MATH_MODE
        if mm == 0:
            return 3 if (co % 64 == 0 and ci % 32 == 0 and self.pairs_on) else 0
        return mm if (co % 128 == 0 and ci % 64 == 0) else 0

    def _rng_kw(self, mode16, name):
        r = self._pair_rng() if mode16 == 3 else None
        return {"rng": (r, r.slot(name))} if r is not None else {}

    def _query_batch(self, que_imgs):
        pk = self._pack()
        an = self.an
        qn = que_imgs.shape[0]
        rfn_all, rfn = self.rfn, self.r_end - self.r_begin
        D, Dg = rfn * an, rfn_all * an
        dev = que_imgs.device
        grp = D if qn > 1 else 0
        ops.stats_arena_begin(dev)
        qf = self.get_feats(que_imgs)
        cat = torch.empty((qn * D, 1, 4, 4, 768), dtype=torch.float32, device=dev)
        caches = [c.view(c.shape[0], c.shape[2] * c.shape[3], 512) for c in self.ref_feats_cache]
        vps, psc, psh, _ = ops.selector_levels([qf[l].view(qn, -1, 512) for l in range(3)], caches, self.ref_sums, Dg)
        levels = [self._level(l, qf[l], cat, psc[:, l].contiguous(), psh[:, l].contiguous(), qn) for l in range(3)]
        if not self.sharded:
            ops.fork_join([(lambda g=g: sum(1 for _ in g)) for g in levels], dev)
        else:
            while levels:
                pending, alive = [], []
                for g in levels:
                    st = next(g, None)
                    if st is not None:
                        pending.append(st); alive.append(g)
                if pending:
                    self._allreduce(pending)
                levels = alive

        with self._mm("fuse"):
            y = torch.empty((qn * D, 1, 4, 4, 512), dtype=torch.float32, device=dev)
            st = ops.new_stats(qn, 512, dev)
            if not self.sharded:
                sc, sh = ops.conv(cat, pk["fuse0"][0], pk["fuse0"][1], y, stats=st, finalize=Dg * 16, rows_per_group=grp * 16)
            else:
                ops.conv(cat, pk["fuse0"][0], pk["fuse0"][1], y, stats=st, rows_per_group=grp * 16)
                self._allreduce([st])
                sc, sh = ops.stats_finalize(st, Dg * 16)
            pooled = torch.empty((qn * D, 1, 1, 1, 512), dtype=torch.float32, device=dev)
            ops.affine_act_pool(y, pooled, sc, sh, per_n=grp, relu=True, pool=2)
            feats = torch.zeros((qn * D, FEAT_LD), dtype=torch.float32, device=dev)
            ops.conv(pooled.view(1, 1, 1, qn * D, 512), pk["fuse3"][0], pk["fuse3"][1], feats.view(1, 1, 1, qn * D, FEAT_LD)[..., :512])
        if not self.sharded:
            ops.vps_norm(vps, feats, 512)
        else:
            rows = vps.reshape(qn, 3, rfn, an).permute(2, 3, 0, 1).reshape(rfn, an * qn * 3).contiguous()
            vall = self._allgather_rows(rows, rfn_all).view(rfn_all, an, qn, 3).permute(2, 3, 0, 1).reshape(qn, 3, Dg).contiguous()
            fall = torch.zeros((qn * Dg, FEAT_LD), dtype=torch.float32, device=dev)
            ops.vps_norm(vall, fall, 512)
            feats.view(qn, D, FEAT_LD)[:, :, 512:515] = fall.view(qn, Dg, FEAT_LD)[:, self.r_begin * an:self.r_end * an, 512:515]

        with self._mm("tail"):
            t0 = torch.empty((1, 1, 1, qn * D, 512), dtype=torch.float32, device=dev)
            ops.conv(feats.view(1, 1, 1, qn * D, FEAT_LD), pk["sp0"][0], pk["sp0"][1], t0, out_act=1)
            t1 = torch.empty_like(t0)
            ops.conv(t0, pk["sp2"][0], pk["sp2"][1], t1)
            xl = torch.empty((qn * rfn, 512), dtype=torch.float32, device=dev)
            ops.max_an_add(t1.view(qn * D, 512), rfn, an, self.ref_pose_embed[self.r_begin:self.r_end].contiguous(), xl, batch=qn)
            feats_l, rfn_l = feats, rfn
            rfn = rfn_all
            xm = torch.empty((qn * rfn, 1024), dtype=torch.float32, device=dev)
            xm[:, :512] = self._allgather_batch(xl, qn, rfn_l, rfn_all)

            def tok(t, n_tok=None):
                n_tok = rfn if n_tok is None else n_tok
                return t.as_strided((qn, 1, 1, n_tok, t.shape[1]), (n_tok * t.stride(0), 0, 0, t.stride(0), 1), t.storage_offset())

            pn = 1 if qn > 1 else 0
            for i in range(2):
                a = pk["att"][i]
                qkv = torch.empty((qn * rfn, 1536), dtype=torch.float32, device=dev)
                ops.conv(tok(xm[:, :512]), a["qkv"][0], a["qkv"][1], tok(qkv))
                att = torch.empty((qn * rfn, 512), dtype=torch.float32, device=dev)
                ops.attention(qkv[:, 0:512], qkv[:, 512:1024], qkv[:, 1024:1536], 8, att, batch=qn)
                mrg = torch.empty((qn * rfn, 512), dtype=torch.float32, device=dev)
                ops.conv(tok(att), a["merge"][0], a["merge"][1], tok(mrg))
                ops.layernorm(mrg, a["ln"][0], a["ln"][1], xm[:, 512:])
                y0 = torch.empty((qn * rfn, 512), dtype=torch.float32, device=dev)
                s0 = ops.new_stats(qn, 512, dev)
                sc0, sh0 = ops.conv(tok(xm), a["mlp0"][0], a["mlp0"][1], tok(y0), stats=s0, finalize=rfn, rows_per_group=pn * rfn)
                y1 = torch.empty((qn * rfn, 512), dtype=torch.float32, device=dev)
                s1 = ops.new_stats(qn, 512, dev)
                sc1, sh1 = ops.conv(tok(y0), a["mlp3"][0], a["mlp3"][1], tok(y1), in_scale=sc0, in_shift=sh0, in_relu=True, per_n=pn, stats=s1,
                                    finalize=rfn, rows_per_group=pn * rfn)
                xn = torch.empty((qn * rfn, 1024), dtype=torch.float32, device=dev)
                ops.affine_act_add(y1, xn[:, :512], sc1, sh1, relu=True, residual=xm[:, :512], rows_per_group=pn * rfn)
                xm = xn
            p0 = torch.empty((qn * rfn, 512), dtype=torch.float32, device=dev)
            ops.conv(tok(xm[:, :512]), pk["pred0"][0], pk["pred0"][1], tok(p0), out_act=1)
            logits = torch.empty((qn * rfn, 1), dtype=torch.float32, device=dev)
            ops.conv(tok(p0), pk["pred2"][0], pk["pred2"][1], tok(logits))

            a0 = torch.empty((qn * rfn_l, 512), dtype=torch.float32, device=dev)
            ops.conv(tok(feats_l.view(qn * rfn_l, an * FEAT_LD), rfn_l), pk["ang0"][0], pk["ang0"][1], tok(a0, rfn_l), out_act=1)
            a1 = torch.empty_like(a0)
            ops.conv(tok(a0, rfn_l), pk["ang2"][0], pk["ang2"][1], tok(a1, rfn_l), out_act=1)
            angles = torch.empty((qn * rfn_l, 1), dtype=torch.float32, device=dev)
            ops.conv(tok(a1, rfn_l), pk["ang4"][0], pk["ang4"][1], tok(angles, rfn_l))
        return logits.view(qn, rfn), self._allgather_batch(angles, qn, rfn_l, rfn_all).view(qn, rfn_all)

    def compute_view_point_feats(self, *a, **k):
        with ops.math_mode(self.cfg.get("math_mode"), inherit_if_none=True):
            return self._compute_view_point_feats_fp(*a, **k)

    def _compute_view_point_feats_fp(self, que_imgs):
        c0 = self.ref_feats_cache[0]
        d_max = -(-self.rfn // self.world) * self.an
        per_query = d_max * c0.shape[2] * c0.shape[3] * 64 * 4
        step = max(1, min(MAX_BATCH, ((1 << 31) - 1) // per_query))
        if step >= 8:
            step -= step % 8
        outs = [self._query_batch(que_imgs[i:i + step].contiguous()) for i in range(0, que_imgs.shape[0], step)]
        return ops.cat1([o[0] for o in outs], 0), ops.cat1([o[1] for o in outs], 0)

    def forward(self, data):
        self.extract_ref_feats(data["ref_imgs"], data["ref_imgs_info"]["poses"], data["object_center"],
                               data["object_vert"], "eval" not in data)
        logits, angles = self.compute_view_point_feats(data["que_imgs_info"]["imgs"])
        return {"ref_vp_logits": logits, "angles_pr": angles}

    def load_ref_imgs(self, ref_imgs, ref_poses, object_center, object_vert):
        dev = self.device_()
        x = torch.from_numpy(np.ascontiguousarray(ref_imgs)).to(dev).float().div_(255).permute(0, 1, 4, 2, 3)
        f = lambda a: torch.from_numpy(np.asarray(a, dtype=np.float32)).to(dev)
        with torch.no_grad():
            self.range_guarded(lambda: self.extract_ref_feats(x, f(ref_poses), f(object_center), f(object_vert)))

    def select_que_imgs(self, que_imgs):
        x = torch.from_numpy(np.ascontiguousarray(que_imgs)).to(self.device_()).float().div_(255).permute(0, 3, 1, 2)
        with torch.no_grad():
            logits, angles = self.range_guarded(lambda: self.compute_view_point_feats(x.contiguous()))
            idx = torch.argmax(logits, 1)
            ang = angles[torch.arange(idx.shape[0], device=idx.device), idx]
        return {"ref_idx": idx.cpu().numpy(), "angles": ang.cpu().numpy(), "scores": logits.cpu().numpy()}
```

gen6d_amd/ops.py:

```python
import ctypes as C
import math

import numpy as np
import torch

from . import lib as _lib

_WS = {}
WORKSPACE_BYTES = 96 << 20
MATH_MODE = 0
_MATH_NAMES = {"fp32": 0, "f32": 0, "bf16": 1, "fp16": 2, "f16": 2, 0: 0, 1: 1, 2: 2, None: 0}


class math_mode:

    def __init__(self, mode, inherit_if_none=False):
        self.mode = None if (mode is None and inherit_if_none) else _MATH_NAMES[mode]

    def __enter__(self):
        global MATH_MODE
        self.prev = MATH_MODE
        if self.mode is not None:
            MATH_MODE = self.mode
        return self

    def __exit__(self, *exc):
        global MATH_MODE
        MATH_MODE = self.prev
        return False
PROFILE = None
PROFILE_HBM = None


_T16 = {1: torch.bfloat16, 2: torch.float16, 3: torch.float16}


def _timed(on, launch, book):
    if not on:
        return launch()
    e0, e1 = torch.cuda.Event(enable_timing=True), torch.cuda.Event(enable_timing=True)
    e0.record()
    launch()
    e1.record()
    book(e0, e1)


def _timed_hbm(name, nbytes, launch):
    _timed(PROFILE_HBM is not None, launch, lambda e0, e1: PROFILE_HBM.setdefault(name, []).append((float(nbytes), e0, e1)))


def _stream():
    return C.c_void_p(torch.cuda.current_stream().cuda_stream)


def _ptr(t):
    return C.c_void_p(t.data_ptr()) if t is not None else C.c_void_p(0)


def _need_gpu(*ts):
    for t in ts:
        if t is not None and not t.is_cuda:
            raise RuntimeError("gen6d_amd.ops: tensors must live on the GPU (HIP kernels only, no CPU fallback)")


def marker(i):
    _lib.check(_lib.load().g6d_marker(int(i), _stream()), "g6d_marker")


def workspace(device):
    key = (str(device), torch.cuda.current_stream(device).cuda_stream)
    if key not in _WS:
        _WS[key] = torch.zeros(WORKSPACE_BYTES // 4, dtype=torch.float32, device=device)
    return _WS[key]


_SIDE = {}
SERIAL = False


def fork_join(fns, device):
    if SERIAL:
        return [fn() for fn in fns]
    main = torch.cuda.current_stream(device)
    streams = _SIDE.setdefault((str(device), main.cuda_stream), [])
    while len(streams) < len(fns) - 1:
        streams.append(torch.cuda.Stream(device=device))
    results = [None] * len(fns)
    for i, fn in enumerate(fns[1:]):
        s = streams[i]
        s.wait_stream(main)
        with torch.cuda.stream(s):
            workspace(device)
            results[i + 1] = fn()
    results[0] = fns[0]()
    for i in range(len(fns) - 1):
        main.wait_stream(streams[i])
    return results


def _cl5(t, name):
    if t.dim() != 5 or t.dtype != torch.float32:
        raise ValueError(f"{name}: expected float32 [N,D,H,W,C], got {tuple(t.shape)} {t.dtype}")
    N, D, H, W, Cc = t.shape
    ld = t.stride(3)
    s = t.stride()
    ok = s[4] == 1 and ld >= Cc
    exp = (D * H * W * ld, H * W * ld, W * ld, ld)
    for dim, (got, want) in enumerate(zip(s[:4], exp)):
        if t.shape[dim] > 1 and got != want:
            ok = False
    if not ok:
        raise ValueError(f"{name}: not a channels-last view (shape {tuple(t.shape)}, strides {s})")
    return N, D, H, W, Cc, ld


FUSED_FINALIZE = True


def conv(x, w, bias, out, ksize=(1, 1, 1), stride=(1, 1, 1), pad=(0, 0, 0), mul=None, in_scale=None, in_shift=None,
         in_relu=False, per_n=False, out_act=0, stats=None, rows_per_group=0, split_k=0, w_wino=None, finalize=None, eps=1e-5,
         in_mod=0, mul_group=0, w_wino43=None):
    _need_gpu(x, w, out)
    Nx, Di, Hi, Wi, Cin, ld_in = _cl5(x, "conv.x")
    No, Do, Ho, Wo, Cout, ld_out = _cl5(out, "conv.out")
    N = No if in_mod else Nx
    if in_mod and Nx != in_mod:
        raise ValueError("conv: with in_mod the input must hold exactly in_mod images")
    per_n = int(per_n)
    kd, kh, kw = ksize
    if tuple(w.shape) != (Cout, kd * kh * kw, Cin) or not w.is_contiguous():
        raise ValueError(f"conv.w: expected contiguous {(Cout, kd * kh * kw, Cin)}, got {tuple(w.shape)}")
    for i, (di, do, k, s, p) in enumerate(zip((Di, Hi, Wi), (Do, Ho, Wo), ksize, stride, pad)):
        if do != (di + 2 * p - k) // s + 1:
            raise ValueError(f"conv: output extent mismatch on axis {i}: in {di} k {k} s {s} p {p} -> out {do}")
    if No != N:
        raise ValueError("conv: batch mismatch")
    if mul is not None:
        want = ((N + mul_group - 1) // mul_group, Hi, Wi, Cin) if mul_group else (Hi, Wi, Cin)
        if tuple(mul.shape) != want or not mul.is_contiguous():
            raise ValueError(f"conv.mul: expected contiguous {want}")
    if w_wino is not None and (tuple(w_wino.shape) != (kd * (Cin // 8), 16, Cout, 8) or not w_wino.is_contiguous()):
        raise ValueError(f"conv.w_wino: expected contiguous {(kd * (Cin // 8), 16, Cout, 8)}, got {tuple(w_wino.shape)}")
    if w_wino43 is not None and (tuple(w_wino43.shape) != w43_shape(kd * (Cin // 8), Cout) or not w_wino43.is_contiguous()):
        raise ValueError(f"conv.w_wino43: expected contiguous {w43_shape(kd * (Cin // 8), Cout)}, got {tuple(w_wino43.shape)}")
    u16 = None
    if MATH_MODE and w_wino is not None and Cin % 16 == 0 and Cout % 64 == 0:
        cache = w_wino.__dict__.setdefault("_g6d_u16", {})
        if MATH_MODE not in cache:
            from .network.backbone import winograd_filters16_taps
            cache[MATH_MODE] = winograd_filters16_taps(w, kd, _T16[MATH_MODE])
        u16 = cache[MATH_MODE]
    ws = workspace(x.device)
    d = _lib.G6dConv(
        in_=x.data_ptr(), mul=mul.data_ptr() if mul is not None else None,
        in_scale=in_scale.data_ptr() if in_scale is not None else None,
        in_shift=in_shift.data_ptr() if in_shift is not None else None,
        weight=w.data_ptr(), bias=bias.data_ptr() if bias is not None else None, out=out.data_ptr(),
        stats=stats.data_ptr() if stats is not None else None, workspace=ws.data_ptr(), workspace_bytes=ws.numel() * 4,
        N=N, Di=Di, Hi=Hi, Wi=Wi, Cin=Cin, ld_in=ld_in, Do=Do, Ho=Ho, Wo=Wo, Cout=Cout, ld_out=ld_out,
        kd=kd, kh=kh, kw=kw, sd=stride[0], sh=stride[1], sw=stride[2], pd=pad[0], ph=pad[1], pw=pad[2],
        in_relu=int(in_relu), in_affine_per_n=int(per_n), out_act=int(out_act),
        stat_rows_per_group=int(rows_per_group), split_k=int(split_k), math_mode=int(MATH_MODE),
        weight_wino=w_wino.data_ptr() if w_wino is not None else None, in_image_mod=int(in_mod), mul_group_images=int(mul_group),
        weight_wino16=u16.data_ptr() if u16 is not None else None,
        weight_wino43=w_wino43.data_ptr() if (w_wino43 is not None and not MATH_MODE) else None)
    fin = None
    if finalize is not None:
        if stats is None:
            raise ValueError("conv: finalize needs stats")
        if FUSED_FINALIZE:
            G = stats.shape[0]
            fin = (torch.empty((G, Cout), dtype=torch.float32, device=x.device), torch.empty((G, Cout), dtype=torch.float32, device=x.device))
            cnt = new_counter(x.device)
            d.fin_scale, d.fin_shift, d.fin_counter = fin[0].data_ptr(), fin[1].data_ptr(), cnt.data_ptr()
            d.fin_count, d.fin_eps, d.fin_groups = float(finalize), float(eps), G

    def book(e0, e1):
        fam = _lib.load().g6d_conv_plan(C.byref(d))
        fl = 2.0 * N * Do * Ho * Wo * Cout * kd * kh * kw * Cin
        if fam == 4:
            if PROFILE_HBM is not None:
                PROFILE_HBM.setdefault("conv_narrow", []).append((4.0 * (N * Di * Hi * Wi * Cin + w.numel() + N * Do * Ho * Wo * Cout), e0, e1))
        else:
            PROFILE.append((fl / 4 if fam == 3 else (fl / 2.25 if fam == 2 else fl), e0, e1,
                        ("wino3x3 F43 " if fam == 3 else "wino3x3 " if fam == 2 else "") + f"conv N={N} in={Di}x{Hi}x{Wi}x{Cin} out={Do}x{Ho}x{Wo}x{Cout} k={kd}x{kh}x{kw} s={stride[0]}{stride[1]}{stride[2]}"
                        f"{' mul' if mul is not None else ''}{' aff' if in_scale is not None else ''}{' stats' if stats is not None else ''}",
                        4.0 * ((in_mod or N) * Di * Hi * Wi * Cin + (mul.numel() if mul is not None else 0) + w.numel() + N * Do * Ho * Wo * Cout), fl))
    _timed(PROFILE is not None, lambda: _lib.check(_lib.load().g6d_conv_igemm(C.byref(d), _stream()), "g6d_conv_igemm"), book)
    if finalize is not None:
        return fin if fin is not None else stats_finalize(stats, finalize, eps)
    return out


def corr2d_patch(x, w, out, k):
    _need_gpu(x, w, out)
    N, D, H, W, Cin, ld_in = _cl5(x, "corr2d.x")
    _, _, Ho, Wo, Cout, ld_out = _cl5(out, "corr2d.out")
    if N * D != 1 or (Ho, Wo) != (H, W) or tuple(w.shape) != (Cout, k * k, Cin) or not w.is_contiguous():
        raise ValueError("corr2d_patch: shape mismatch")
    ws = workspace(x.device)
    _timed(PROFILE is not None,
           lambda: _lib.check(_lib.load().g6d_corr2d_patch(_ptr(x), H, W, Cin, ld_in, _ptr(w), Cout, k, k, _ptr(out), ld_out, _ptr(ws),
                                                          ws.numel() * 4, int(MATH_MODE), _stream()), "g6d_corr2d_patch"),
           lambda e0, e1: PROFILE.append((2.0 * H * W * Cout * k * k * Cin, e0, e1, f"corr2d_patch in={H}x{W}x{Cin} out={Cout} k={k}x{k}",
                                          4.0 * (H * W * (Cin + Cout) + w.numel()))))
    return out


def corr_filters16(w, k, dtype):
    Cout, taps, Cin = w.shape
    assert taps == k * k and Cin % 32 == 0 and Cout <= 32
    v = w.reshape(Cout, k, k, Cin // 32, 32).permute(3, 1, 2, 0, 4)
    out = torch.zeros((Cin // 32, k, k, 32, 40), dtype=dtype, device=w.device)
    out[:, :, :, :Cout, :32] = v.to(dtype)
    return torch.cat([out.reshape(-1), torch.zeros(512, dtype=dtype, device=w.device)]).contiguous()


def _corr_table(name, what, xs, outs, Cin, Cout, k, strided_single=False):
    segs = (_lib.G6dCorrSeg * len(xs))()
    flops, sizes = 0.0, []
    for i, (x, o) in enumerate(zip(xs, outs)):
        N, D, H, W, Cx, ld_in = _cl5(x, f"{what}.x")
        No, _, Ho, Wo, Co, ld_out = _cl5(o, f"{what}.out")
        dense = x.is_contiguous() and o.is_contiguous()
        if D != 1 or No != N or (Ho, Wo) != (H, W) or Cx != Cin or Co != Cout or not (dense or (strided_single and N == 1)):
            raise ValueError(f"{name}: shape mismatch ({'batched ' if strided_single else ''}maps must be dense)")
        segs[i] = _lib.G6dCorrSeg(in_=x.data_ptr(), out=o.data_ptr(), H=H, W=W, ld_in=ld_in, ld_out=ld_out, N=N)
        flops += 2.0 * N * H * W * Cout * k * k * Cin
        sizes.append(f"{N}x{H}x{W}" if N > 1 else f"{H}x{W}")
    return segs, flops, "+".join(sizes)


def _numel(*lists):
    return sum(t.numel() for ts in lists for t in ts)


def corr2d_patch_multi(xs, w, outs, k):
    _need_gpu(w, *xs, *outs)
    if not 1 <= len(xs) <= 4 or len(outs) != len(xs):
        raise ValueError("corr2d_patch_multi: 1..4 maps")
    Cout, _, Cin = w.shape
    segs, flops, sizes = _corr_table("corr2d_patch_multi", "corr2d_multi", xs, outs, Cin, Cout, k, strided_single=True)
    if tuple(w.shape) != (Cout, k * k, Cin) or not w.is_contiguous():
        raise ValueError("corr2d_patch_multi: filter shape mismatch")
    ws = workspace(w.device)
    wk, sfx = w, ""
    if MATH_MODE and Cin % 32 == 0 and k <= 15:
        cache = w.__dict__.setdefault("_g6d_c16", {})
        if MATH_MODE not in cache:
            cache[MATH_MODE] = corr_filters16(w, k, _T16[MATH_MODE])
        wk, sfx = cache[MATH_MODE], "16"
    entry = f"g6d_corr2d_patch{sfx}_multi"
    _timed(PROFILE is not None,
           lambda: _lib.check(getattr(_lib.load(), entry)(segs, len(xs), Cin, _ptr(wk), Cout, k, k, _ptr(ws), ws.numel() * 4, int(MATH_MODE), _stream()), entry),
           lambda e0, e1: PROFILE.append((flops, e0, e1, f"corr2d_patch{sfx} multi in={sizes}x{Cin} out={Cout} k={k}x{k}",
                                          4.0 * (_numel(xs, outs) + w.numel()))))
    return outs


def corr2d_wino_multi(xs, U, outs, kblocks=5):
    _need_gpu(U, *xs, *outs)
    if not 1 <= len(xs) <= 4 or len(outs) != len(xs):
        raise ValueError("corr2d_wino_multi: 1..4 map sizes")
    Cin, Cout = xs[0].shape[4], U.shape[2]
    if tuple(U.shape) != (kblocks * kblocks * (Cin // 8), 16, Cout, 8) or not U.is_contiguous():
        raise ValueError(f"corr2d_wino_multi: U must be contiguous {(kblocks * kblocks * (Cin // 8), 16, Cout, 8)}")
    k = 3 * kblocks
    segs, flops, sizes = _corr_table("corr2d_wino_multi", "corr2d_wino", xs, outs, Cin, Cout, k)
    ws = workspace(U.device)
    _timed(PROFILE is not None,
           lambda: _lib.check(_lib.load().g6d_corr2d_wino_multi(segs, len(xs), Cin, _ptr(U), Cout, int(kblocks), _ptr(ws), ws.numel() * 4, _stream()),
                              "g6d_corr2d_wino_multi"),
           lambda e0, e1: PROFILE.append((flops / 2.25, e0, e1, f"wino3x3 corr multi in={sizes}x{Cin} out={Cout} k={k}x{k} ({kblocks}x{kblocks} blocks of 3x3)",
                                          4.0 * (_numel(xs, outs) + U.numel()))))
    return outs


_ARENA = {}
_CUR_ARENA = None
USE_ARENA = True
ARENA_DOUBLES = 1 << 21


def stats_arena_begin(device):
    global _CUR_ARENA
    key = (str(device), torch.cuda.current_stream(device).cuda_stream)
    if key not in _ARENA:
        _ARENA[key] = [torch.zeros(ARENA_DOUBLES, dtype=torch.float64, device=device), 0, 0]
    a = _ARENA[key]
    n_clear = ARENA_DOUBLES if (a[0].is_cuda and torch.cuda.is_current_stream_capturing()) else a[2]
    if n_clear:
        _lib.check(_lib.load().g6d_zero_bytes(_ptr(a[0]), n_clear * 8, _stream()), "g6d_zero_bytes")
    a[1] = 0
    _CUR_ARENA = a


def new_stats(groups, channels, device):
    a = _CUR_ARENA if USE_ARENA else None
    n = groups * channels * 2
    if a is None or a[0].device != torch.device(device) or a[1] + n > ARENA_DOUBLES:
        return torch.zeros((groups, channels, 2), dtype=torch.float64, device=device)
    t = a[0][a[1]:a[1] + n].view(groups, channels, 2)
    a[1] += n
    a[2] = max(a[2], a[1])
    return t


def new_counter(device):
    a = _CUR_ARENA if USE_ARENA else None
    if a is None or a[0].device != torch.device(device) or a[1] + 1 > ARENA_DOUBLES:
        return torch.zeros((2,), dtype=torch.int32, device=device)
    t = a[0][a[1]:a[1] + 1].view(torch.int32)
    a[1] += 1
    a[2] = max(a[2], a[1])
    return t


def stats_finalize(stats, count, eps=1e-5):
    _need_gpu(stats)
    G, Cc, _ = stats.shape
    scale = torch.empty((G, Cc), dtype=torch.float32, device=stats.device)
    shift = torch.empty_like(scale)
    _lib.check(_lib.load().g6d_stats_finalize(_ptr(stats), G * Cc, float(count), float(eps), _ptr(scale), _ptr(shift),
                                             _stream()), "g6d_stats_finalize")
    return scale, shift


def affine_act_pool(x, out, scale=None, shift=None, per_n=False, relu=False, pool=0):
    _need_gpu(x, out)
    N, D, H, W, Cc, ld_in = _cl5(x, "affine_act_pool.x")
    _, _, _, _, Co, ld_out = _cl5(out, "affine_act_pool.out")
    if Co != Cc:
        raise ValueError("affine_act_pool: channel mismatch")
    _lib.check(_lib.load().g6d_affine_act_pool(_ptr(x), ld_in, _ptr(scale), _ptr(shift), int(per_n) * D, int(relu), int(pool),
                                              N * D, H, W, Cc, _ptr(out), ld_out, _stream()), "g6d_affine_act_pool")
    return out


def upsample_bilinear(x, out, factor, scale=None, shift=None, per_n=False):
    _need_gpu(x, out)
    N, D, H, W, Cc, ld_in = _cl5(x, "upsample.x")
    _, _, Ho, Wo, Co, ld_out = _cl5(out, "upsample.out")
    if (Ho, Wo, Co) != (H * factor, W * factor, Cc):
        raise ValueError("upsample: output shape mismatch")
    _lib.check(_lib.load().g6d_upsample_bilinear(_ptr(x), ld_in, _ptr(scale), _ptr(shift), int(per_n) * D, N * D, H, W, Cc,
                                                int(factor), _ptr(out), ld_out, _stream()), "g6d_upsample_bilinear")
    return out


def bias_relu_pool_nchw(x, bias, relu, pool):
    _need_gpu(x, bias)
    if not x.is_contiguous() or x.dtype != torch.float32:
        raise ValueError("bias_relu_pool_nchw: x must be contiguous float32 NCHW")
    N, Cc, H, W = x.shape
    out = torch.empty((N, Cc, H // 2, W // 2) if pool else (N, Cc, H, W), dtype=torch.float32, device=x.device)
    _lib.check(_lib.load().g6d_bias_relu_pool_nchw(_ptr(x), _ptr(bias), N, Cc, H, W, int(relu), int(pool), _ptr(out), _stream()),
               "g6d_bias_relu_pool_nchw")
    return out


def vgg_conv1_pool(x, w_oihw, bias):
    _need_gpu(x, w_oihw, bias)
    if x.dtype != torch.float32 or x.dim() != 4 or not x.is_contiguous() or not w_oihw.is_contiguous():
        raise ValueError("vgg_conv1_pool: x and w must be contiguous float32 NCHW / OIHW")
    N, Cin, H, W = x.shape
    Cout = w_oihw.shape[0]
    if tuple(w_oihw.shape) != (Cout, Cin, 3, 3) or bias.numel() != Cout:
        raise ValueError("vgg_conv1_pool: weight / bias shape mismatch")
    out = torch.empty((N, Cout, H // 2, W // 2), dtype=torch.float32, device=x.device)
    _lib.check(_lib.load().g6d_vgg_conv1_pool(_ptr(x), N, H, W, _ptr(w_oihw), _ptr(bias), Cin, Cout, _ptr(out), _stream()),
               "g6d_vgg_conv1_pool")
    return out


def vgg_conv1_pool_nhwc(x, w_oihw, bias, out=None, norm=None):
    _need_gpu(x, w_oihw, bias)
    if x.dtype != torch.float32 or x.dim() != 4 or not x.is_contiguous() or not w_oihw.is_contiguous():
        raise ValueError("vgg_conv1_pool_nhwc: x and w must be contiguous float32 NCHW / OIHW")
    N, Cin, H, W = x.shape
    Cout = w_oihw.shape[0]
    if tuple(w_oihw.shape) != (Cout, Cin, 3, 3) or bias.numel() != Cout:
        raise ValueError("vgg_conv1_pool_nhwc: weight / bias shape mismatch")
    if out is None:
        out = torch.empty((N, H // 2, W // 2, Cout), dtype=torch.float32, device=x.device)
    elif tuple(out.shape) != (N, H // 2, W // 2, Cout) or not out.is_contiguous() or out.dtype != torch.float32:
        raise ValueError("vgg_conv1_pool_nhwc: out must be contiguous float32 [N,H/2,W/2,Cout]")
    if norm is not None:
        m, sd = (C.c_float * 3)(*norm[0]), (C.c_float * 3)(*norm[1])
        _lib.check(_lib.load().g6d_vgg_conv1_pool_nhwc_norm(_ptr(x), N, H, W, _ptr(w_oihw), _ptr(bias), Cin, Cout, m, sd, _ptr(out),
                                                            _stream()), "g6d_vgg_conv1_pool_nhwc_norm")
        return out
    _lib.check(_lib.load().g6d_vgg_conv1_pool_nhwc(_ptr(x), N, H, W, _ptr(w_oihw), _ptr(bias), Cin, Cout, _ptr(out), _stream()),
               "g6d_vgg_conv1_pool_nhwc")
    return out


def wino_conv3x3(x, U, bias, relu=True, full=True, pool=False):
    _need_gpu(x, U, bias)
    if x.dim() != 4 or x.dtype != torch.float32 or x.stride(3) != 1:
        raise ValueError("wino_conv3x3: x must be a float32 channels-last [N,H,W,C] view")
    N, H, W, Cin = x.shape
    ld_in = x.stride(2)
    if (N > 1 and x.stride(0) != H * W * ld_in) or (H > 1 and x.stride(1) != W * ld_in):
        raise ValueError("wino_conv3x3: x rows must be dense")
    Cout = U.shape[2]
    if tuple(U.shape) != (Cin // 8, 16, Cout, 8) or not U.is_contiguous() or bias.numel() != Cout:
        raise ValueError(f"wino_conv3x3: U must be contiguous {(Cin // 8, 16, Cout, 8)}")
    y = torch.empty((N, H, W, Cout), dtype=torch.float32, device=x.device) if full else None
    yp = torch.empty((N, H // 2, W // 2, Cout), dtype=torch.float32, device=x.device) if pool else None
    ws = workspace(x.device)
    _timed(PROFILE is not None,
           lambda: _lib.check(_lib.load().g6d_wino_conv3x3(_ptr(x), N, H, W, Cin, ld_in, _ptr(U), _ptr(bias), Cout, int(relu), _ptr(y), Cout,
                                                          _ptr(yp), Cout, _ptr(ws), ws.numel() * 4, _stream()), "g6d_wino_conv3x3"),
           lambda e0, e1: PROFILE.append((2.0 * N * H * W * Cout * 9 * Cin / 2.25, e0, e1,
                                          f"wino3x3 N={N} in={H}x{W}x{Cin} out={Cout}{' full' if full else ''}{' pool' if pool else ''}",
                                          4.0 * (x.numel() + U.numel() + (y.numel() if full else 0) + (yp.numel() if pool else 0)))))
    return y, yp


def alloc_like_segments(shapes, device):
    sizes = [int(torch.Size(sh).numel()) for sh in shapes]
    starts, tot = [], 0
    for n in sizes:
        starts.append(tot)
        tot += (n + 3) // 4 * 4
    buf = torch.empty((max(tot, 1),), dtype=torch.float32, device=device)
    return [buf[st:st + n].view(sh) for st, n, sh in zip(starts, sizes, shapes)]


def _wino_table(name, xs, Cout, full, pool):
    if not 1 <= len(xs) <= 4:
        raise ValueError(f"{name}: 1..4 segments")
    Cin = xs[0].shape[3]
    for x in xs:
        if x.dim() != 4 or x.dtype != torch.float32 or not x.is_contiguous() or x.shape[3] != Cin:
            raise ValueError(f"{name}: segments must be contiguous float32 [N,H,W,Cin]")
    dev = xs[0].device
    ys = alloc_like_segments([(x.shape[0], x.shape[1], x.shape[2], Cout) for x in xs], dev) if full else None
    yps = alloc_like_segments([(x.shape[0], x.shape[1] // 2, x.shape[2] // 2, Cout) for x in xs], dev) if pool else None
    segs = (_lib.G6dWinoSeg * len(xs))()
    flops = 0.0
    for i, x in enumerate(xs):
        N, H, W, _ = x.shape
        segs[i] = _lib.G6dWinoSeg(in_=x.data_ptr(), out_full=ys[i].data_ptr() if full else None,
                                  out_pool=yps[i].data_ptr() if pool else None, N=N, H=H, W=W, ld_in=Cin, ld_full=Cout, ld_pool=Cout)
        flops += 2.0 * N * H * W * Cout * 9 * Cin

    def describe():
        sizes = "+".join(f"{x.shape[0]}x{x.shape[1]}x{x.shape[2]}" for x in xs)
        return f"in={sizes}x{Cin} out={Cout}{' full' if full else ''}{' pool' if pool else ''}", _numel(xs, ys or (), yps or ())
    return segs, Cin, ys, yps, flops, describe


def _wino_book(flops, kind, describe, filter_floats, *direct):
    def book(e0, e1):
        label, act = describe()
        PROFILE.append((flops, e0, e1, f"wino3x3 {kind}multi {label}", 4.0 * (act + filter_floats)) + direct)
    return book


def wino_conv3x3_multi(xs, U, bias, relu=True, full=True, pool=False):
    _need_gpu(U, bias, *xs)
    Cout = U.shape[2]
    segs, Cin, ys, yps, flops, describe = _wino_table("wino_conv3x3_multi", xs, Cout, full, pool)
    if tuple(U.shape) != (Cin // 8, 16, Cout, 8) or not U.is_contiguous() or bias.numel() != Cout:
        raise ValueError(f"wino_conv3x3_multi: U must be contiguous {(Cin // 8, 16, Cout, 8)}")
    ws = workspace(xs[0].device)
    _timed(PROFILE is not None,
           lambda: _lib.check(_lib.load().g6d_wino_conv3x3_multi(segs, len(xs), Cin, _ptr(U), _ptr(bias), Cout, int(relu), _ptr(ws), ws.numel() * 4,
                                                                _stream()), "g6d_wino_conv3x3_multi"),
           _wino_book(flops / 2.25, "", describe, U.numel()))
    return ys, yps


def w43_shape(chunks, Cout):
    cb = 32 if Cout % 64 else 64
    return (chunks, 2, Cout // cb, 18, cb // 32, 4, 16, 4)


def wino43_conv3x3_multi(xs, U43, bias, relu=True, full=True, pool=False):
    _need_gpu(U43, bias, *xs)
    Cout = bias.numel()
    segs, Cin, ys, yps, flops, describe = _wino_table("wino43_conv3x3_multi", xs, Cout, full, pool)
    if tuple(U43.shape) != w43_shape(Cin // 8, Cout) or not U43.is_contiguous():
        raise ValueError(f"wino43_conv3x3_multi: U43 must be contiguous {w43_shape(Cin // 8, Cout)}")
    ws = workspace(xs[0].device)
    _timed(PROFILE is not None,
           lambda: _lib.check(_lib.load().g6d_wino43_conv3x3_multi(segs, len(xs), Cin, _ptr(U43), _ptr(bias), Cout, int(relu), _ptr(ws), ws.numel() * 4,
                                                                  _stream()), "g6d_wino43_conv3x3_multi"),
           _wino_book(flops / 4, "F43 ", describe, U43.numel(), flops))
    return ys, yps


def corr2d_wino43_multi(xs, U43, outs, kblocks=5, k_true=None):
    _need_gpu(U43, *xs, *outs)
    if not 1 <= len(xs) <= 4 or len(outs) != len(xs):
        raise ValueError("corr2d_wino43_multi: 1..4 map sizes")
    Cin, Cout = xs[0].shape[4], outs[0].shape[4]
    if tuple(U43.shape) != w43_shape(kblocks * kblocks * (Cin // 8), Cout) or not U43.is_contiguous():
        raise ValueError(f"corr2d_wino43_multi: U43 must be contiguous {w43_shape(kblocks * kblocks * (Cin // 8), Cout)}")
    k = 3 * kblocks
    segs, flops, sizes = _corr_table("corr2d_wino43_multi", "corr2d_wino43", xs, outs, Cin, Cout, k)
    kt = k_true or k
    ws = workspace(U43.device)
    _timed(PROFILE is not None,
           lambda: _lib.check(_lib.load().g6d_corr2d_wino43_multi(segs, len(xs), Cin, _ptr(U43), Cout, int(kblocks), _ptr(ws), ws.numel() * 4, _stream()),
                              "g6d_corr2d_wino43_multi"),
           lambda e0, e1: PROFILE.append((flops / 4, e0, e1, f"wino3x3 F43 corr multi in={sizes}x{Cin} out={Cout} k={kt}x{kt} ({kblocks}x{kblocks} blocks of 3x3)",
                                          4.0 * (_numel(xs, outs) + U43.numel()), flops * kt * kt / (k * k))))
    return outs


def wino16_conv3x3_multi(xs, U16, bias, relu=True, full=True, pool=False):
    _need_gpu(U16, bias, *xs)
    mm = {torch.bfloat16: 1, torch.float16: 2}.get(U16.dtype)
    Cout = U16.shape[2]
    segs, Cin, ys, yps, flops, describe = _wino_table("wino16_conv3x3_multi", xs, Cout, full, pool)
    if mm is None or tuple(U16.shape) != (Cin // 16, 16, Cout, 16) or not U16.is_contiguous() or bias.numel() != Cout:
        raise ValueError(f"wino16_conv3x3_multi: U16 must be contiguous bfloat16 / float16 {(Cin // 16, 16, Cout, 16)}")
    ws = workspace(xs[0].device)
    _timed(PROFILE is not None,
           lambda: _lib.check(_lib.load().g6d_wino16_conv3x3_multi(segs, len(xs), Cin, _ptr(U16), _ptr(bias), Cout, int(relu), mm, _ptr(ws), ws.numel() * 4,
                                                                  _stream()), "g6d_wino16_conv3x3_multi"),
           _wino_book(flops / 2.25, "bf16 " if mm == 1 else "fp16 ", describe, U16.numel() / 2))
    return ys, yps


PAIR_KEEP = (2.0 ** -4, 2.0 ** 14)
PAIR_LIMIT = (2.0 ** -4, 2.0 ** 15)
PAIR_EXP_MAX = 100


def pair_exponent(a, e=0):
    if not math.isfinite(a):
        return e
    if a == 0.0 or PAIR_KEEP[0] <= a < PAIR_KEEP[1]:
        return 0
    return max(-PAIR_EXP_MAX, min(PAIR_EXP_MAX, math.frexp(a)[1] - 1))


def pair_out_of_window(a, e):
    if not math.isfinite(a):
        return True
    if a == 0.0:
        return False
    s = math.ldexp(a, -e)
    return s >= PAIR_LIMIT[1] or s < PAIR_LIMIT[0]


def bits_to_float(bits):
    return np.asarray(bits, dtype=np.int64).astype(np.uint32).view(np.float32).astype(np.float64)


class RangeTable:
    CAP = 64

    def __init__(self, device):
        self.device = device
        self.exps = torch.zeros(self.CAP, dtype=torch.int32, device=device)
        self.rec = torch.zeros(self.CAP, dtype=torch.int32, device=device)
        self.e = [0] * self.CAP
        self.names = {}

    def slot(self, name):
        if name not in self.names:
            if len(self.names) == self.CAP:
                raise RuntimeError("RangeTable: out of slots")
            self.names[name] = len(self.names)
        return self.names[name]

    def arg(self, slot_in=-1, slot_out=-1):
        return _lib.G6dRange16(exps=self.exps.data_ptr(), rec=self.rec.data_ptr(), slot_in=int(slot_in), slot_out=int(slot_out))

    def clear(self):
        _lib.check(_lib.load().g6d_zero_bytes(_ptr(self.rec), self.rec.numel() * 4, _stream()), "g6d_zero_bytes")

    def reset(self):
        self.e = [0] * self.CAP
        self.set_exponents({})
        self.clear()

    def read(self):
        a = bits_to_float(self.rec.cpu().numpy())
        return {n: float(a[i]) for n, i in self.names.items()}

    def set_exponents(self, es):
        for n, e in es.items():
            self.e[self.slot(n)] = int(e)
        self.exps.copy_(torch.tensor(self.e, dtype=torch.int32), non_blocking=False)


class PairMap:
    __slots__ = ("data", "table", "slot")

    def __init__(self, data, table, slot):
        self.data, self.table, self.slot = data, table, slot

    @property
    def shape(self):
        return self.data.shape

    def __getitem__(self, idx):
        return PairMap(self.data[idx], self.table, self.slot)

    def view(self, *shape):
        return PairMap(self.data.view(*shape), self.table, self.slot)


def _pair_inputs(xs):
    maps = [x for x in xs if isinstance(x, PairMap)]
    if not maps:
        return list(xs), None, -1
    if len(maps) != len(xs) or len({(id(m.table), m.slot) for m in maps}) != 1:
        raise ValueError("pair inputs of one launch must all be PairMaps of one slot")
    return [m.data for m in maps], maps[0].table, maps[0].slot


def _range_arg(table_in, slot_in, rng):
    table = rng[0] if rng is not None else table_in
    if table is None:
        return None
    if table_in is not None and table_in is not table:
        raise ValueError("pair input and output belong to different range tables")
    return C.byref(table.arg(slot_in, rng[1] if rng is not None else -1))


def _wrap(t, rng):
    return PairMap(t, rng[0], rng[1]) if (rng is not None and t is not None) else t


class Conv16Filters:

    def __init__(self, data, layout, mode, acc_scale, Cout, taps, Cin):
        self.data, self.layout, self.mode, self.acc_scale, self.Cout, self.taps, self.Cin = data, layout, mode, acc_scale, Cout, taps, Cin


def _split_hi_lo(w_taps):
    S = 2.0 ** min(14, math.floor(math.log2(2048.0 / max(float(w_taps.abs().max()), 1e-30))))
    w = w_taps.double() * S
    hi = w.to(torch.float16)
    return hi, (w - hi.double()).to(torch.float16), 1.0 / S


def conv16_fold_depth(w_taps):
    co, taps, ci = w_taps.shape
    if taps != 27:
        raise ValueError("conv16_fold_depth: [Cout, 27, Cin] expected")
    return w_taps.reshape(co, 3, 9, ci).permute(0, 2, 1, 3).reshape(co, 9, 3 * ci).contiguous()


def conv16_pack(w_taps, mode, layout=1):
    if layout == 2:
        if mode != 3 or w_taps.shape[1] != 27:
            raise ValueError("conv16_pack: the depth-folded layout takes 27-tap filters in mode 3 (fp16 pairs)")
        f = conv16_pack(conv16_fold_depth(w_taps), mode, layout=1)
        return Conv16Filters(f.data, 2, mode, f.acc_scale, f.Cout, 27, w_taps.shape[2])
    co, taps, ci = w_taps.shape
    bk = 32 if mode == 3 else 64
    co_true = co
    if co == 64 and layout == 1 and taps == 9:
        w_taps = torch.cat([w_taps, torch.zeros_like(w_taps)], 0)
        co = 128
    if co % 128 or ci % bk:
        raise ValueError("conv16_pack: Cout % 128 == 0 (pairs, 2-D: also 64) and Cin % 64 (pairs: 32) == 0 expected")
    acc_scale = 1.0
    if mode == 3:
        hi, lo, acc_scale = _split_hi_lo(w_taps)
        planes = torch.stack([hi, lo], 0)
    else:
        planes = w_taps.to(_T16[mode])[None]
    if layout == 0:
        if mode == 3:
            raise ValueError("conv16_pack: pairs need the fragment-major layout")
        return Conv16Filters(planes[0].contiguous(), 0, mode, 1.0, co, taps, ci)
    P, ks = planes.shape[0], bk // 16
    x = planes.reshape(P, co // 128, 4, 32, taps, ci // bk, ks, 2, 8)
    x = x.permute(1, 5, 4, 6, 0, 2, 7, 3, 8).contiguous()
    return Conv16Filters(x.reshape(-1), 1, mode, acc_scale, co_true, taps, ci)


def product_split16(ref, que, scale, shift, mode, rng=None):
    if rng is not None and mode != 3:
        raise ValueError("product_split16: a range applies to pairs (mode 3) only")
    _need_gpu(ref, que, scale, shift)
    D, P, Cc = ref.shape
    qn = que.shape[0]
    if tuple(que.shape) != (qn, P, Cc) or tuple(scale.shape) != (qn, Cc) or tuple(shift.shape) != (qn, Cc) or not all(
            t.is_contiguous() and t.dtype == torch.float32 for t in (ref, que, scale, shift)):
        raise ValueError("product_split16: dense fp32 ref [D,P,C], que [qn,P,C], scale / shift [qn,C] expected")
    out = torch.empty((qn * D, P, 2, Cc) if mode == 3 else (qn * D, P, Cc), dtype=_T16[mode], device=ref.device)
    nbytes = 4.0 * (ref.numel() + que.numel()) + 2.0 * out.numel()
    ra = _range_arg(None, -1, rng)
    _timed_hbm("product_split16", nbytes, lambda: _lib.check(_lib.load().g6d_product_split16_ex(
        _ptr(ref), _ptr(que), _ptr(scale), _ptr(shift), _ptr(out), qn, D, P, Cc, int(mode), ra, _stream()), "g6d_product_split16"))
    return _wrap(out, rng)


def affine_split16(x, scale, shift, per_n, relu, pool, mode, rng=None):
    if rng is not None and mode != 3:
        raise ValueError("affine_split16: a range applies to pairs (mode 3) only")
    _need_gpu(x)
    N, D, H, W, Cc, ld_in = _cl5(x, "affine_split16.x")
    if D != 1:
        raise ValueError("affine_split16: 2-D maps expected")
    Ho, Wo = (H // 2, W // 2) if pool else (H, W)
    out = torch.empty((N, Ho, Wo, 2, Cc) if mode == 3 else (N, Ho, Wo, Cc), dtype=_T16[mode], device=x.device)
    ra = _range_arg(None, -1, rng)
    _timed_hbm("affine_split16", 4.0 * N * H * W * Cc + 2.0 * out.numel(), lambda: _lib.check(_lib.load().g6d_affine_split16_ex(
        _ptr(x), ld_in, _ptr(scale), _ptr(shift), int(per_n), int(bool(relu)), int(bool(pool)), N, H, W, Cc, _ptr(out), int(mode), ra, _stream()),
        "g6d_affine_split16"))
    return _wrap(out, rng)


def new_map16(N, H, W, Cc, mode, device, rng=None):
    if rng is not None and mode != 3:
        raise ValueError("new_map16: a range applies to pairs (mode 3) only")
    return _wrap(torch.empty((N, H, W, 2, Cc) if mode == 3 else (N, H, W, Cc), dtype=_T16[mode], device=device), rng)


def _slice16(out, N, Ho, Wo, Cc, c_off, mode, what):
    table, slot = (out.table, out.slot) if isinstance(out, PairMap) else (None, -1)
    t = out.data if isinstance(out, PairMap) else out
    if table is not None and mode != 3:
        raise ValueError(f"{what}: a PairMap output needs mode 3")
    _need_gpu(t)
    Ct = t.shape[-1]
    want = (N, Ho, Wo, 2, Ct) if mode == 3 else (N, Ho, Wo, Ct)
    if t.dtype != _T16[mode] or not t.is_contiguous() or tuple(t.shape) != want or c_off < 0 or c_off % 8 or Ct % 8 or c_off + Cc > Ct:
        raise ValueError(f"{what}: out must be a dense {_T16[mode]} map of shape {want[:-1]} + (C,) that holds channels [{c_off}, {c_off + Cc})")
    return t, (2 * Ct if mode == 3 else Ct), Ct, (C.byref(table.arg(-1, slot)) if table is not None else None)


def affine_split16_to(x, scale, shift, per_n, relu, mode, out, c_off=0):
    _need_gpu(x)
    N, D, H, W, Cc, ld_in = _cl5(x, "affine_split16_to.x")
    if D != 1:
        raise ValueError("affine_split16_to: 2-D maps expected")
    t, ld_out, plane, ra = _slice16(out, N, H, W, Cc, c_off, mode, "affine_split16_to")
    _timed_hbm("affine_split16", (4.0 + (4.0 if mode == 3 else 2.0)) * N * H * W * Cc, lambda: _lib.check(_lib.load().g6d_affine_split16_to(
        _ptr(x), ld_in, _ptr(scale), _ptr(shift), int(per_n), int(bool(relu)), 0, N, H, W, Cc, _ptr(t), ld_out, plane, int(c_off), int(mode), ra,
        _stream()), "g6d_affine_split16_to"))
    return out


def upsample_bilinear_split16(x, out, c_off, factor, scale, shift, per_n, mode):
    _need_gpu(x)
    N, D, H, W, Cc, ld_in = _cl5(x, "upsample_bilinear_split16.x")
    if D != 1:
        raise ValueError("upsample_bilinear_split16: 2-D maps expected")
    Ho, Wo = H * int(factor), W * int(factor)
    t, ld_out, plane, ra = _slice16(out, N, Ho, Wo, Cc, c_off, mode, "upsample_bilinear_split16")
    _timed_hbm("upsample_split16", 4.0 * N * H * W * Cc + (4.0 if mode == 3 else 2.0) * N * Ho * Wo * Cc, lambda: _lib.check(
        _lib.load().g6d_upsample_bilinear_split16(_ptr(x), ld_in, _ptr(scale), _ptr(shift), int(per_n), N, H, W, Cc, int(factor), _ptr(t), ld_out,
                                                  plane, int(c_off), int(mode), ra, _stream()), "g6d_upsample_bilinear_split16"))
    return out


def l2norm_split16(x, mode, rng=None):
    if rng is not None and mode != 3:
        raise ValueError("l2norm_split16: a range applies to pairs (mode 3) only")
    _need_gpu(x)
    if x.dtype != torch.float32 or not x.is_contiguous() or x.dim() != 4:
        raise ValueError("l2norm_split16: a dense float32 [N,H,W,C] tap expected")
    N, H, W, Cc = x.shape
    out = torch.empty((N, H, W, 2, Cc) if mode == 3 else (N, H, W, Cc), dtype=_T16[mode], device=x.device)
    ra = _range_arg(None, -1, rng)
    _timed_hbm("l2norm_split16", 4.0 * x.numel() + 2.0 * out.numel(), lambda: _lib.check(_lib.load().g6d_l2norm_split16(
        _ptr(x), Cc, N * H * W, Cc, _ptr(out), int(mode), ra, _stream()), "g6d_l2norm_split16"))
    return _wrap(out, rng)


def vgg_conv1_pool_nhwc16(x, w_oihw, bias, out=None, norm=None, mode=None, rng=None):
    _need_gpu(x, w_oihw, bias)
    mode = MATH_MODE if mode is None else mode
    if mode not in _T16:
        raise RuntimeError("vgg_conv1_pool_nhwc16: mode 1 (bf16), 2 (fp16) or 3 (fp16 pairs)")
    if rng is not None and mode != 3:
        raise ValueError("vgg_conv1_pool_nhwc16: a range applies to pairs (mode 3) only")
    N, Cin, H, W = x.shape
    Cout = w_oihw.shape[0]
    shape = (N, H // 2, W // 2, 2, Cout) if mode == 3 else (N, H // 2, W // 2, Cout)
    if out is None:
        out = torch.empty(shape, dtype=_T16[mode], device=x.device)
    if out.dtype != _T16[mode] or not out.is_contiguous() or tuple(out.shape) != shape:
        raise ValueError(f"vgg_conv1_pool_nhwc16: out must be a dense {_T16[mode]} tensor of shape {shape}")
    mean = std = None
    if norm is not None:
        mean, std = (C.c_float * 3)(*norm[0]), (C.c_float * 3)(*norm[1])
    _lib.check(_lib.load().g6d_vgg_conv1_pool_nhwc16_ex(_ptr(x.contiguous()), N, H, W, _ptr(w_oihw.contiguous()), _ptr(bias), Cin, Cout,
                                                        mean, std, _ptr(out), int(mode), _range_arg(None, -1, rng), _stream()),
               "g6d_vgg_conv1_pool_nhwc16")
    return _wrap(out, rng)


def conv16_direct_multi(xs, filt, bias, relu=True, full=None, pool=None, kd=1, stats=None, rows_per_group=0, out_full=None, rng=None):
    xs, table_in, slot_in = _pair_inputs(xs)
    if (table_in is not None or rng is not None) and filt.mode != 3:
        raise ValueError("conv16_direct_multi: ranges apply to pairs (mode 3) only")
    ra = _range_arg(table_in, slot_in, rng)
    _need_gpu(filt.data, *xs)
    mode = filt.mode
    t16 = _T16[mode]
    Cout, taps, Cin = filt.Cout, filt.taps, filt.Cin
    if taps != 9 * kd:
        raise ValueError("conv16_direct_multi: filters / kd mismatch")
    pair = mode == 3
    code = {None: 0, "t16": 3 if pair else 1, torch.float32: 2}
    if full not in code or pool not in code:
        raise ValueError('conv16_direct_multi: output types are None, torch.float32 or "t16"')
    segs = (_lib.G6dConv16Seg * len(xs))()
    fulls, pools, flops, sizes, nbytes = [], [], 0.0, [], 2.0 * filt.data.numel()
    nd = (4 if kd == 1 else 5) + (1 if pair else 0)
    for i, x in enumerate(xs):
        if x.dtype != t16 or not x.is_contiguous() or x.dim() != nd or x.shape[-1] != Cin or (pair and x.shape[-2] != 2):
            raise ValueError(f"conv16_direct_multi: input {i} must be a dense {t16} channels-last tensor with {Cin} channels{' in hi / lo planes' if pair else ''}")
        N, D, H, W = (x.shape[0], 1, x.shape[1], x.shape[2]) if kd == 1 else tuple(x.shape[:4])
        lead = (N, H, W) if kd == 1 else (N, D, H, W)

        def alloc(kind, lead_):
            if kind is None:
                return None
            if kind == "t16":
                return torch.empty(lead_ + ((2, Cout) if pair else (Cout,)), dtype=t16, device=x.device)
            return torch.empty(lead_ + (Cout,), dtype=torch.float32, device=x.device)
        q = alloc(pool, (N, H // 2, W // 2))
        ld_f = None
        if out_full is not None:
            f = out_full[i]
            want_t = torch.float32 if full is torch.float32 else t16
            nel = N * D * H * W * Cout * (2 if (pair and full == "t16") else 1)
            if full is None or f.dtype != want_t or f.numel() != nel or f.stride(-1) != 1:
                raise ValueError("conv16_direct_multi: out_full must hold the outputs' type and size")
            if not f.is_contiguous():
                ld_f = f.stride(-2)
                if full is not torch.float32 or f.shape[-1] != Cout or any(f.stride(d) != f.stride(d + 1) * f.shape[d + 1] for d in range(f.dim() - 2)):
                    raise ValueError("conv16_direct_multi: a strided out_full must be an fp32 channel slice of dense rows")
        else:
            f = alloc(full, lead)
        fulls.append(f); pools.append(q)
        ld = lambda t_: (2 * Cout if t_.dtype != torch.float32 and pair else Cout)
        segs[i] = _lib.G6dConv16Seg(in_=x.data_ptr(), out_full=f.data_ptr() if f is not None else None,
                                    out_pool=q.data_ptr() if q is not None else None, N=N, D=D, H=H, W=W, ld_in=(2 if pair else 1) * Cin,
                                    ld_full=(ld_f or ld(f)) if f is not None else 0, ld_pool=ld(q) if q is not None else 0)
        flops += 2.0 * N * D * H * W * Cout * taps * Cin
        nbytes += x.numel() * 2.0 + sum(t.numel() * t.element_size() for t in (f, q) if t is not None)
        sizes.append("x".join(str(v) for v in lead))
    _timed(PROFILE is not None,
           lambda: _lib.check(_lib.load().g6d_conv16_direct_multi_ex(
               segs, len(xs), Cin, _ptr(filt.data), int(filt.layout), float(filt.acc_scale), _ptr(bias), Cout, int(kd), int(bool(relu)), code[full],
               code[pool], int(mode), _ptr(stats), int(rows_per_group), ra, _stream()), "g6d_conv16_direct_multi"),
           lambda e0, e1: PROFILE.append((flops, e0, e1, f"{'conv16x3' if pair else 'conv16'} direct in={'+'.join(sizes)}x{Cin} out={Cout} k={'3x' if kd == 3 else ''}3x3"
                                          f"{' full' if full is not None else ''}{' pool' if pool is not None else ''}{' stats' if stats is not None else ''}", nbytes, flops)))
    if rng is not None:
        fulls = [_wrap(f, rng) if full == "t16" else f for f in fulls]
        pools = [_wrap(q, rng) if pool == "t16" else q for q in pools]
    return fulls, pools


def conv16_direct_plan(N, H, W, Cin, Cout, mode, stats_rows=0, full=torch.float32, D=None):
    pair = mode == 3
    code = {None: 0, "t16": 3 if pair else 1, torch.float32: 2}[full]
    any_ = 1 << 12
    ldf = 2 * Cout if code == 3 else Cout
    seg = (_lib.G6dConv16Seg * 1)(_lib.G6dConv16Seg(in_=any_, out_full=any_ if code else None, out_pool=None, N=N, D=D or 1, H=H, W=W,
                                                    ld_in=(2 if pair else 1) * Cin, ld_full=ldf if code else 0, ld_pool=0))
    rc = _lib.load().g6d_conv16_direct_plan(seg, 1, Cin, C.c_void_p(any_), 2 if D else 1, Cout, 3 if D else 1, code, 0, int(mode),
                                            C.c_void_p(any_ if stats_rows else 0), int(stats_rows))
    return rc if rc >= 0 else None


def corr16_pack(w_taps, mode):
    co, taps, ci = w_taps.shape
    if co != 32 or ci % 32:
        raise ValueError("corr16_pack: 32 references and Cin % 32 == 0 expected")
    acc_scale = 1.0
    if mode == 3:
        hi, lo, acc_scale = _split_hi_lo(w_taps)
        x = torch.stack([hi, lo], 0).reshape(2, 32, taps, ci // 16, 2, 8)
        x = x.permute(3, 2, 0, 4, 1, 5).contiguous()
    else:
        x = w_taps.to(_T16[mode]).reshape(32, taps, ci // 32, 2, 2, 8)
        x = x.permute(2, 1, 3, 4, 0, 5).contiguous()
    k = int(round(taps ** 0.5))
    f = Conv16Filters(x.reshape(-1), 1, mode, acc_scale, co, taps, ci)
    f.k = k
    return f


def corr16_multi(xs, filt, outs):
    xs, table_in, slot_in = _pair_inputs(xs)
    if table_in is not None and filt.mode != 3:
        raise ValueError("corr16_multi: PairMaps need pair filters (mode 3)")
    ra = _range_arg(table_in, slot_in, None)
    _need_gpu(filt.data, *xs, *outs)
    mode, Cin = filt.mode, filt.Cin
    pair = mode == 3
    segs = (_lib.G6dConv16Seg * len(xs))()
    flops, sizes, nbytes = 0.0, [], 2.0 * filt.data.numel()
    for i, (x, o) in enumerate(zip(xs, outs)):
        if x.dtype != _T16[mode] or not x.is_contiguous() or x.dim() != (5 if pair else 4) or x.shape[-1] != Cin or not o.is_contiguous() \
                or o.dtype != torch.float32 or o.shape[-1] != 32:
            raise ValueError("corr16_multi: dense 16-bit channels-last inputs and dense fp32 outputs with 32 channels expected")
        N, H, W = x.shape[0], x.shape[1], x.shape[2]
        if o.numel() != N * H * W * 32:
            raise ValueError("corr16_multi: output shape mismatch")
        segs[i] = _lib.G6dConv16Seg(in_=x.data_ptr(), out_full=o.data_ptr(), out_pool=None, N=N, D=1, H=H, W=W, ld_in=(2 if pair else 1) * Cin,
                                    ld_full=32, ld_pool=0)
        flops += 2.0 * N * H * W * 32 * filt.taps * Cin
        nbytes += x.numel() * 2.0 + o.numel() * 4.0
        sizes.append(f"{N}x{H}x{W}")
    _timed(PROFILE is not None,
           lambda: _lib.check(_lib.load().g6d_corr16_multi_ex(segs, len(xs), Cin, _ptr(filt.data), float(filt.acc_scale), 32, int(filt.k), int(mode), ra,
                                                             _stream()), "g6d_corr16_multi"),
           lambda e0, e1: PROFILE.append((flops, e0, e1, f"{'conv16x3' if pair else 'conv16'} corr in={'+'.join(sizes)}x{Cin} out=32 k={filt.k}x{filt.k}",
                                          nbytes, flops)))
    return outs


def l2norm_rows(x):
    _need_gpu(x)
    Cc = x.shape[-1]
    if x.dtype == torch.float32 and x.dim() == 2 and x.stride(1) == 1 and not x.is_contiguous():
        _lib.check(_lib.load().g6d_l2norm_rows(_ptr(x), x.shape[0], Cc, x.stride(0), _stream()), "g6d_l2norm_rows")
        return x
    if x.dtype != torch.float32 or not x.is_contiguous():
        raise ValueError("l2norm_rows: contiguous float32 expected")
    _lib.check(_lib.load().g6d_l2norm_rows(_ptr(x), x.numel() // Cc, Cc, Cc, _stream()), "g6d_l2norm_rows")
    return x


def nchw_to_nhwc(x, out, l2norm):
    _need_gpu(x, out)
    if not x.is_contiguous() or x.dtype != torch.float32:
        raise ValueError("nchw_to_nhwc: x must be contiguous float32 NCHW")
    N, Cc, H, W = x.shape
    _, _, Ho, Wo, Co, ld_out = _cl5(out, "nchw_to_nhwc.out")
    if (Ho, Wo, Co) != (H, W, Cc):
        raise ValueError("nchw_to_nhwc: shape mismatch")
    _lib.check(_lib.load().g6d_nchw_to_nhwc(_ptr(x), N, Cc, H, W, int(l2norm), _ptr(out), ld_out, _stream()), "g6d_nchw_to_nhwc")
    return out

# ... 551 lines not shown
```

include/gen6d_hip.h:

```cpp
#ifndef GEN6D_HIP_H
#define GEN6D_HIP_H

#include <stddef.h>
#include <stdint.h>

#ifdef __cplusplus
extern "C" {
#endif

typedef void* g6d_stream_t;

enum {
  G6D_OK = 0,
  G6D_EINVAL = -1,
  G6D_ENOSPC = -2,
  G6D_ELAUNCH = -3
};

int g6d_abi_version(void);
const char* g6d_last_error(void);

int g6d_set_knob(const char* name, double value);
double g6d_get_knob(const char* name);
void g6d_reset_knobs(void);

int g6d_marker(int id, g6d_stream_t stream);

#define G6D_WORKSPACE_COUNTER_BYTES 16384

typedef struct G6dConv {
  const float* in;
  const float* mul;
  const float* in_scale;
  const float* in_shift;
  const float* weight;
  const float* bias;
  float* out;
  double* stats;
  float* workspace;
  size_t workspace_bytes;
  int32_t N, Di, Hi, Wi, Cin, ld_in;
  int32_t Do, Ho, Wo, Cout, ld_out;
  int32_t kd, kh, kw;
  int32_t sd, sh, sw;
  int32_t pd, ph, pw;
  int32_t in_relu;
  int32_t in_affine_per_n;
  int32_t out_act;
  int32_t stat_rows_per_group;
  int32_t split_k;
  int32_t math_mode;
  const float* weight_wino;
  float* fin_scale;
  float* fin_shift;
  int32_t* fin_counter;
  double fin_count, fin_eps;
  int32_t fin_groups;
  int32_t in_image_mod;
  int32_t mul_group_images;
  int32_t reserved_;
  const void* weight_wino16;
  const float* weight_wino43;
} G6dConv;

int g6d_conv_igemm(const G6dConv* desc, g6d_stream_t stream);
int g6d_conv_plan(const G6dConv* desc);
int g6d_sizeof_conv_desc(void);

int g6d_corr2d_patch(const float* in, int H, int W, int Cin, int ld_in, const float* wgt, int Cout, int kh, int kw,
                     float* out, int ld_out, float* workspace, size_t workspace_bytes, int math_mode ,
                     g6d_stream_t stream);
typedef struct G6dCorrSeg {
  const float* in;
  float* out;
  int32_t H, W, ld_in, ld_out;
  int32_t N, reserved_;
} G6dCorrSeg;
int g6d_corr2d_patch_multi(const G6dCorrSeg* segs, int nseg, int Cin, const float* wgt, int Cout, int kh, int kw,
                           float* workspace, size_t workspace_bytes, int math_mode, g6d_stream_t stream);
int g6d_corr2d_patch16_multi(const G6dCorrSeg* segs, int nseg, int Cin, const void* w16, int Cout, int kh, int kw,
                             float* workspace, size_t workspace_bytes, int math_mode, g6d_stream_t stream);

int g6d_corr2d_wino_multi(const G6dCorrSeg* segs, int nseg, int Cin, const float* U, int Cout, int kblocks, float* workspace,
                          size_t workspace_bytes, g6d_stream_t stream);

int g6d_corr2d_wino43_multi(const G6dCorrSeg* segs, int nseg, int Cin, const float* U43, int Cout, int kblocks, float* workspace,
                            size_t workspace_bytes, g6d_stream_t stream);

int g6d_stats_finalize(const double* stats, int n, double count, double eps, float* scale, float* shift, g6d_stream_t stream);

int g6d_affine_act_pool(const float* in, int ld_in, const float* scale, const float* shift, int affine_per_n, int relu,
                        int pool, int N, int H, int W, int C, float* out, int ld_out, g6d_stream_t stream);

int g6d_upsample_bilinear(const float* in, int ld_in, const float* scale, const float* shift, int affine_per_n,
                          int N, int H, int W, int C, int factor, float* out, int ld_out, g6d_stream_t stream);

int g6d_bias_relu_pool_nchw(const float* in, const float* bias, int N, int C, int H, int W, int relu, int pool, float* out,
                            g6d_stream_t stream);

int g6d_vgg_conv1_pool(const float* in, int N, int H, int W, const float* w_oihw, const float* bias, int Cin, int Cout,
                       float* out, g6d_stream_t stream);

int g6d_vgg_conv1_pool_nhwc(const float* in, int N, int H, int W, const float* w_oihw, const float* bias, int Cin, int Cout,
                            float* out, g6d_stream_t stream);
int g6d_vgg_conv1_pool_nhwc_norm(const float* in, int N, int H, int W, const float* w_oihw, const float* bias, int Cin, int Cout,
                                 const float* mean_host, const float* std_host, float* out, g6d_stream_t stream);
int g6d_vgg_conv1_pool_nhwc16(const float* in, int N, int H, int W, const float* w_oihw, const float* bias, int Cin, int Cout,
                              const float* mean_host, const float* std_host, void* out16, int math_mode, g6d_stream_t stream);


int g6d_wino_conv3x3(const float* in, int N, int H, int W, int Cin, int ld_in, const float* U, const float* bias, int Cout,
                     int relu, float* out_full, int ld_full, float* out_pool, int ld_pool, float* workspace,
                     size_t workspace_bytes, g6d_stream_t stream);

typedef struct G6dWinoSeg {
  const float* in;
  float* out_full;
  float* out_pool;
  int32_t N, H, W, ld_in, ld_full, ld_pool;
} G6dWinoSeg;
int g6d_wino_conv3x3_multi(const G6dWinoSeg* segs, int nseg, int Cin, const float* U, const float* bias, int Cout, int relu,
                           float* workspace, size_t workspace_bytes, g6d_stream_t stream);

int g6d_wino16_conv3x3_multi(const G6dWinoSeg* segs, int nseg, int Cin, const void* U16, const float* bias, int Cout, int relu,
                             int math_mode, float* workspace, size_t workspace_bytes, g6d_stream_t stream);

typedef struct G6dConv16Seg {
  const void* in;
  void* out_full;
  void* out_pool;
  int32_t N, D, H, W, ld_in, ld_full, ld_pool;
} G6dConv16Seg;
int g6d_conv16_direct_multi(const G6dConv16Seg* segs, int nseg, int Cin, const void* W16, int w_layout, float acc_scale, const float* bias,
                            int Cout, int kd, int relu, int full_type, int pool_type, int math_mode, double* stats, int stat_rows_per_group,
                            g6d_stream_t stream);

int g6d_product_split16(const float* ref, const float* que, const float* scale, const float* shift, void* out, int qn, int D, int P, int C,
                        int math_mode, g6d_stream_t stream);

int g6d_affine_split16(const float* in, int ld_in, const float* scale, const float* shift, int affine_per_n, int relu, int pool, int N, int H, int W,
                       int C, void* out, int math_mode, g6d_stream_t stream);

int g6d_corr16_multi(const G6dConv16Seg* segs, int nseg, int Cin, const void* W16, float acc_scale, int Cout, int k, int math_mode,
                     g6d_stream_t stream);

typedef struct G6dRange16 {
  const int32_t* exps;
  uint32_t* rec;
  int32_t slot_in, slot_out;
} G6dRange16;
int g6d_conv16_direct_multi_ex(const G6dConv16Seg* segs, int nseg, int Cin, const void* W16, int w_layout, float acc_scale, const float* bias,
                               int Cout, int kd, int relu, int full_type, int pool_type, int math_mode, double* stats, int stat_rows_per_group,
                               const G6dRange16* range, g6d_stream_t stream);
int g6d_conv16_direct_plan(const G6dConv16Seg* segs, int nseg, int Cin, const void* W16, int w_layout, int Cout, int kd, int full_type, int pool_type,
                           int math_mode, double* stats, int stat_rows_per_group);
int g6d_corr16_multi_ex(const G6dConv16Seg* segs, int nseg, int Cin, const void* W16, float acc_scale, int Cout, int k, int math_mode,
                        const G6dRange16* range, g6d_stream_t stream);
int g6d_product_split16_ex(const float* ref, const float* que, const float* scale, const float* shift, void* out, int qn, int D, int P, int C,
                           int math_mode, const G6dRange16* range, g6d_stream_t stream);
int g6d_affine_split16_ex(const float* in, int ld_in, const float* scale, const float* shift, int affine_per_n, int relu, int pool, int N, int H,
                          int W, int C, void* out, int math_mode, const G6dRange16* range, g6d_stream_t stream);
int g6d_vgg_conv1_pool_nhwc16_ex(const float* in, int N, int H, int W, const float* w_oihw, const float* bias, int Cin, int Cout,
                                 const float* mean_host, const float* std_host, void* out16, int math_mode, const G6dRange16* range,
                                 g6d_stream_t stream);

int g6d_affine_split16_to(const float* in, int ld_in, const float* scale, const float* shift, int affine_per_n, int relu, int pool, int N, int H,
                          int W, int C, void* out, int ld_out, int plane, int c_off, int math_mode, const G6dRange16* range, g6d_stream_t stream);
int g6d_upsample_bilinear_split16(const float* in, int ld_in, const float* scale, const float* shift, int affine_per_n, int N, int H, int W, int C,
                                  int factor, void* out, int ld_out, int plane, int c_off, int math_mode, const G6dRange16* range,
                                  g6d_stream_t stream);
int g6d_l2norm_split16(const float* in, int ld_in, int rows, int C, void* out, int math_mode, const G6dRange16* range, g6d_stream_t stream);

int g6d_wino43_conv3x3_multi(const G6dWinoSeg* segs, int nseg, int Cin, const float* U43, const float* bias, int Cout, int relu,
                             float* workspace, size_t workspace_bytes, g6d_stream_t stream);

int g6d_l2norm_rows(float* x, int rows, int C, int ld, g6d_stream_t stream);

int g6d_nchw_to_nhwc(const float* in, int N, int C, int H, int W, int l2norm, float* out, int ld_out, g6d_stream_t stream);

int g6d_selector_ref_sums(const float* refs, int D, int HW, int C, double* r1, double* r2, g6d_stream_t stream);
int g6d_selector_prod_affine(const float* que, const double* r1, const double* r2, int D, int HW, int C, double eps,
                             float* scale, float* shift, g6d_stream_t stream);
int g6d_selector_scan(const float* que, const float* refs, int D, int HW, int C, float* score_map, float* vps,
                      g6d_stream_t stream);
int g6d_selector_levels(int nlev, int qn, const float* const* que, const float* const* refs, const double* const* r1,
                        const double* const* r2, const int* HW, int D, int Dg, int C, double eps, float* const* score_maps,
                        float* vps, float* scale, float* shift, g6d_stream_t stream);

int g6d_refiner_volume(const float* feats, const float* projs, const float* rot_in, const float* lin, int rfn, int fh,
                       int fw, int C, int h_in, int w_in, int sn, float* mean_in, float* std, g6d_stream_t stream);
int g6d_refiner_volume_kp(const float* feats, const float* ref_Ks, const float* ref_poses, const float* K_in, const float* pose_in,
                          const float* lin, int rfn, int fh, int fw, int C, int h_in, int w_in, int sn, float* mean_in, float* stdv,
                          int batch, g6d_stream_t stream);
int g6d_refiner_volume_kp_pairs(const float* feats, const float* ref_Ks, const float* ref_poses, const float* K_in, const float* pose_in,
                                const float* lin, int rfn, int fh, int fw, int C, int h_in, int w_in, int sn, void* mean_in16, void* std16,
                                int batch, const G6dRange16* range_mean, const G6dRange16* range_std, g6d_stream_t stream);

int g6d_detector_assemble(const float* s0, const float* s1, const float* s2, int hc, int wc, int rfn,
                          const float* mu_sigma , float clip, int hs, int ws,
                          int scale_idx, int nch, float* stacked, int batch, g6d_stream_t stream);

int g6d_detector_score_mlp_max(const float* stacked, int P, int rfn, int nch, const float* w0, const float* b0,
                               const float* w1, const float* b1, float* out, g6d_stream_t stream);

int g6d_detector_decode(const float* scores, int ld_s, const float* offset, int ld_o, const float* scale, int ld_c,
                        int hs, int ws, int pool_ratio, float* result, int batch, g6d_stream_t stream);
int g6d_resize_bilinear_pyramid(const float* src, int planes, int H, int W, int nscale, const int* hs, const int* ws,
                                float* const* dsts, g6d_stream_t stream);
int g6d_zero_bytes(void* ptr, size_t bytes, g6d_stream_t stream);

int g6d_vps_norm(const float* vps, int D, float* feats, int ld, int c_off, int batch, g6d_stream_t stream);
int g6d_max_an_add(const float* in, int ld_in, int rfn, int an, int C, const float* embed, float* out, int ld_out, int batch,
                   g6d_stream_t stream);
int g6d_attention(const float* q, const float* k, const float* v, int ld, int n, int C, int heads, float* out,
                  int ld_out, int batch, g6d_stream_t stream);
int g6d_layernorm(const float* in, int ld_in, int n, int C, const float* gamma, const float* beta, float eps,
                  float* out, int ld_out, g6d_stream_t stream);
int g6d_affine_act_add(const float* in, int ld_in, const float* scale, const float* shift, int relu,
                       const float* residual, int ld_res, int n, int C, float* out, int ld_out, int rows_per_group,
                       g6d_stream_t stream);

int g6d_warp_perspective(const unsigned char* src, int sh, int sw, int ch, const float* hinv, void* dst, int dh, int dw,
                         int out_float, float out_scale, g6d_stream_t stream);

int g6d_chain_crop_from_detection(const float* det, float size, float* hinv, int batch, g6d_stream_t stream);
int g6d_chain_pose_from_selection(const float* det, const float* logits, const float* angles, int rfn, const float* ref_poses,
                                  const float* ref_Ks, const float* que_K, const float* center, float* pose_out, float* sel_out,
                                  int batch, g6d_stream_t stream);
int g6d_chain_refine_prepare(const float* pose_in, const float* que_K, const float* norm, float size, float margin,
                             const float* sub_poses, const float* sub_Ks, int n_sub, int ref_num, float* geo, int* ref_idx,
                             float angle_step, int* ref_bucket, int batch, g6d_stream_t stream);
int g6d_chain_refine_update(const float* rot, const float* off, const float* scl, const float* geo, int geo_floats ,
                            const float* norm, float* pose_out, int batch, g6d_stream_t stream);
int g6d_warp_batch(const unsigned char* stack, const unsigned char* single, const int* idx, int B, int sh, int sw, int ch,
                   const float* hinv, float* dst, int dh, int dw, g6d_stream_t stream);

int g6d_linear_gemv(const float* x, int B, int K, const float* W, const float* bias, int O, int act, float* out,
                    g6d_stream_t stream);

int g6d_linear_gemv_batch(const float* x, int B, int K, const float* W, const float* bias, int O, int act, float* out, float* workspace,
                          size_t workspace_bytes, g6d_stream_t stream);

int g6d_track_gather(const float* pose_table, const int* slot_stream, const float* parking_pose, float* pose_out, int batch,
                     g6d_stream_t stream);
#define G6D_TRACK_MAX_NUM 64
int g6d_track_commit(const float* pose, const float* K, const int* slot_stream, int reset, const float* box, int num, float std,
                     float* pose_table, double* hist, int* hist_count, float* smooth_table, float* out, int batch, g6d_stream_t stream);

enum { G6D_TRACK_NONE = 0, G6D_TRACK_TRACKING = 1, G6D_TRACK_SUSPECT = 2, G6D_TRACK_LOST = 3 };
enum { G6D_TRACK_NONFINITE = 1, G6D_TRACK_BEHIND = 2, G6D_TRACK_SMALL = 4, G6D_TRACK_LARGE = 8, G6D_TRACK_OUTSIDE = 16, G6D_TRACK_ROT = 32,
       G6D_TRACK_SHIFT = 64, G6D_TRACK_SCALE = 128, G6D_TRACK_VERIFY_POS = 256, G6D_TRACK_VERIFY_SCALE = 512 };
int g6d_track_gate(const float* pose_table, int32_t* health, const int* slot_stream, int* slot_eff, int batch, g6d_stream_t stream);
int g6d_track_health(const float* pose_prev, const float* pose_new, const float* K, const int32_t* pic, int W, int H, const int* slot_eff,
                     int reset, const float* center, double diameter, int patience, double min_px, double max_px, double margin,
                     double max_rot_deg, double max_shift, double max_log2_scale, int32_t* health, float* measures, int* slot_commit,
                     int* slot_draw, int batch, g6d_stream_t stream);
int g6d_track_verify(const float* det, const float* pose_table, const float* K, const int* slot_commit, const float* center,
                     double diameter, double ref_px, double verify_shift, double verify_log2_scale, int verify_patience, int32_t* health,
                     float* measures, int batch, g6d_stream_t stream);

enum { G6D_FMT_RGB24 = 0, G6D_FMT_BGR24 = 1, G6D_FMT_RGBA32 = 2, G6D_FMT_BGRA32 = 3, G6D_FMT_NV12 = 4 };
typedef struct G6dFrame {
  const void* plane0;
  const void* plane1;
  int32_t pitch0, pitch1;
  int32_t width, height;
  int32_t format;
  int32_t rotate;
  int32_t matrix;
  int32_t slot;
  int32_t out_w, out_h;
  float   K[9];
} G6dFrame;
int g6d_frame_ingest(const G6dFrame* frames, int n, uint8_t* out, int B, int H, int W, float* K_out, g6d_stream_t stream);
int g6d_sizeof_frame_desc(void);

typedef struct G6dMesh {
  const int32_t* nodes;
  int32_t nx, ny;
  int32_t step_log2;
  int32_t reserved;
} G6dMesh;
int g6d_frame_ingest_mesh(const G6dFrame* frames, const G6dMesh* meshes, int n, uint8_t* out, int B, int H, int W, float* K_out,
                          g6d_stream_t stream);
int g6d_sizeof_mesh_desc(void);

int g6d_track_corners(const float* table, const float* K, const int* slot_stream, const float* box, int32_t* pts, int32_t* valid,
                      int batch, g6d_stream_t stream);
typedef struct G6dSink {
  void* plane0;
  void* plane1;
  int32_t pitch0, pitch1;
  int32_t width, height;
  int32_t format;
  int32_t matrix;
  int32_t slot;
  int32_t pic_w, pic_h;
  int32_t thickness, dot_radius;
  int32_t line_rgb, dot_rgb;
  int32_t box;
} G6dSink;
int g6d_frame_emit(const G6dSink* sinks, int n, const uint8_t* imgs, int B, int H, int W, const int32_t* pts, const int32_t* valid,
                   g6d_stream_t stream);
int g6d_sizeof_sink_desc(void);

int g6d_frame_emit_source(const G6dSink* sinks, int n, const G6dFrame* frames, int nf, const int32_t* pts, const int32_t* valid, int sets,
                          int B, int max_w, int max_h, g6d_stream_t stream);

#ifdef __cplusplus
}
#endif
#endif
```

Before: 354.3.

## Add fp16 hi/lo pair math mode to implicit-GEMM conv for volume layers

Adds math_mode 3 to the implicit-GEMM conv kernel. Activations and weights are scaled by power-of-two exponents and split into fp16 hi/lo pairs in LDS, then multiplied with three f16 32x32x16 MFMAs (hi*hi, hi*lo, lo*hi) in place of fp32 MFMAs. The kernel also records the input range max for later exponent choice. The refiner volume-net layers conv1, conv3 and conv5 are routed to this path when the query batch is large enough, bypassing Winograd for them. This trades extra MFMAs and conversion work for faster f16 tensor-core throughput, with some precision risk from the dropped lo*lo term and the exponent scaling.

```diff
diff --git a/gen6d_amd/csrc/conv_igemm.hip b/gen6d_amd/csrc/conv_igemm.hip
--- a/gen6d_amd/csrc/conv_igemm.hip
+++ b/gen6d_amd/csrc/conv_igemm.hip
@@ -19,6 +19,18 @@
 
 __device__ __forceinline__ f32x4 ldg(const float* __restrict__ base, int elem_off) {
   return *reinterpret_cast<const f32x4*>(reinterpret_cast<const char*>(base) + ((unsigned)elem_off << 2));
+}
+
+__device__ __forceinline__ const int* pair_exp_ptr(const G6dConv& p) { return reinterpret_cast<const int*>(p.weight_wino16); }
+__device__ __forceinline__ unsigned* pair_rec_ptr(const G6dConv& p) { return reinterpret_cast<unsigned*>(const_cast<float*>(p.weight_wino43)); }
+typedef _Float16 f16x4 __attribute__((ext_vector_type(4)));
+__device__ __forceinline__ void store_pair(float* row, int seg, f32x4 u) {
+  f16x4 hi, lo;
+#pragma unroll
+  for (int e = 0; e < 4; ++e) { hi[e] = (_Float16)u[e]; lo[e] = (_Float16)(u[e] - (float)hi[e]); }
+  char* r = reinterpret_cast<char*>(row);
+  *reinterpret_cast<f16x4*>(r + 8 * seg) = hi;
+  *reinterpret_cast<f16x4*>(r + 64 + 8 * seg) = lo;
 }
 
 template <int BM, int BN, int WGM, int WGN, int MODE, int MM>
@@ -63,6 +75,12 @@
   const float* __restrict__ gsc = p.in_scale;
   const float* __restrict__ gsh = p.in_shift;
   const int relu = p.in_relu;
+  float a_mul = 1.f, w_mul = 1.f, o_mul = 1.f;
+  unsigned amax = 0u;
+  if constexpr (MM == 3) {
+    const int e_in = pair_exp_ptr(p) ? *pair_exp_ptr(p) : 0;
+    a_mul = __builtin_ldexpf(1.f, -e_in); w_mul = __builtin_ldexpf(1.f, p.w_exp); o_mul = __builtin_ldexpf(1.f, e_in - p.w_exp);
+  }
 
   const int pad_a = ((p.pd * p.Hi + p.ph) * p.Wi + p.pw) * p.ld_in;
   const int pad_m = (p.ph * p.Wi + p.pw) * Cin;
@@ -170,11 +188,18 @@
       b &= va[s][j];
       v = __builtin_bit_cast(f32x4, b);
     }
-    *reinterpret_cast<f32x4*>(As + (lrow + 32 * j) * LDS_K + 4 * lseg) = v;
+    if constexpr (MM == 3) {
+      const u32x4 b = __builtin_bit_cast(u32x4, v) & 0x7fffffffu;
+      amax = max(amax, max(max(b[0], b[1]), max(b[2], b[3])));
+      store_pair(As + (lrow + 32 * j) * LDS_K, lseg, v * a_mul);
+    } else {
+      *reinterpret_cast<f32x4*>(As + (lrow + 32 * j) * LDS_K + 4 * lseg) = v;
+    }
   };
   auto store_b = [&](auto S, float* Bs, int j) {
     constexpr int s = decltype(S)::value;
-    *reinterpret_cast<f32x4*>(Bs + (lrow + 32 * j) * LDS_K + 4 * lseg) = rb[s][j];
+    if constexpr (MM == 3) store_pair(Bs + (lrow + 32 * j) * LDS_K, lseg, rb[s][j] * w_mul);
+    else *reinterpret_cast<f32x4*>(Bs + (lrow + 32 * j) * LDS_K + 4 * lseg) = rb[s][j];
   };
 
   f32x4 dummy = {0.f, 0.f, 0.f, 0.f};
@@ -209,7 +234,48 @@
     constexpr int par = decltype(PAR)::value;
     using SL = std::integral_constant<int, par>;
     using SS = std::integral_constant<int, par ^ 1>;
-    if constexpr (MM != 0) {
+    if constexpr (MM == 3) {
+#pragma unroll
+      for (int j = 0; j < RA; ++j) load_a(SL{}, j);
+#pragma unroll
+      for (int j = 0; j < RB; ++j) load_b(SL{}, j);
+      const char* Ab = reinterpret_cast<const char*>(As + (wm * WM + li) * LDS_K) + 16 * lh;
+      const char* Bb = reinterpret_cast<const char*>(Bs + (wn * WN + li) * LDS_K) + 16 * lh;
+#pragma unroll
+      for (int ks = 0; ks < 2; ++ks) {
+        f16x8 ah[MT], al[MT], bh[NT], bl[NT];
+#pragma unroll
+        for (int i = 0; i < MT; ++i) {
+          ah[i] = *reinterpret_cast<const f16x8*>(Ab + i * 32 * LDS_K * 4 + 32 * ks);
+          al[i] = *reinterpret_cast<const f16x8*>(Ab + i * 32 * LDS_K * 4 + 64 + 32 * ks);
+        }
+#pragma unroll
+        for (int j = 0; j < NT; ++j) {
+          bh[j] = *reinterpret_cast<const f16x8*>(Bb + j * 32 * LDS_K * 4 + 32 * ks);
+          bl[j] = *reinterpret_cast<const f16x8*>(Bb + j * 32 * LDS_K * 4 + 64 + 32 * ks);
+        }
+#pragma unroll
+        for (int i = 0; i < MT; ++i)
+#pragma unroll
+          for (int j = 0; j < NT; ++j) {
+            if (ONE_ACC && ks == 1) {
+              acc_odd = __builtin_amdgcn_mfma_f32_32x32x16_f16(ah[i], bh[j], acc_odd, 0, 0, 0);
+              acc_odd = __builtin_amdgcn_mfma_f32_32x32x16_f16(ah[i], bl[j], acc_odd, 0, 0, 0);
+              acc_odd = __builtin_amdgcn_mfma_f32_32x32x16_f16(al[i], bh[j], acc_odd, 0, 0, 0);
+            } else {
+              acc[i][j] = __builtin_amdgcn_mfma_f32_32x32x16_f16(ah[i], bh[j], acc[i][j], 0, 0, 0);
+              acc[i][j] = __builtin_amdgcn_mfma_f32_32x32x16_f16(ah[i], bl[j], acc[i][j], 0, 0, 0);
+              acc[i][j] = __builtin_amdgcn_mfma_f32_32x32x16_f16(al[i], bh[j], acc[i][j], 0, 0, 0);
+            }
+          }
+      }
+#pragma unroll
+      for (int j = 0; j < RA; ++j) store_a(SS{}, An, j);
+#pragma unroll
+      for (int j = 0; j < RB; ++j) store_b(SS{}, Bn, j);
+      advance(); begin_step(SS{});
+      return;
+    } else if constexpr (MM != 0) {
 #pragma unroll
       for (int j = 0; j < RA; ++j) load_a(SL{}, j);
 #pragma unroll
@@ -289,6 +355,15 @@
     if (G6D_ABLATE == 6) acc[0][0][0] += dummy[0] + dummy[1] + dummy[2] + dummy[3];
   }
 
+  if constexpr (MM == 3) {
+    if (pair_rec_ptr(p)) {
+      unsigned* red = reinterpret_cast<unsigned*>(lds + STAGE);
+      amax = g6d_wave_max_u(amax);
+      if (lane == 0) red[wave] = amax;
+      __syncthreads();
+      if (tid == 0) g6d_range_max(pair_rec_ptr(p), max(max(red[0], red[1]), max(red[2], red[3])));
+    }
+  }
   if constexpr (ONE_ACC) {
 #pragma unroll
     for (int r = 0; r < 16; ++r) acc[0][0][r] += acc_odd[r];
@@ -362,7 +437,7 @@
 #pragma unroll
       for (int r = 0; r < 16; ++r) {
         const int row = row_m(wm * WM + i * 32 + (r & 3) + 8 * (r >> 2) + 4 * lh);
-        float v = apply_act(acc[i][j][r] + bv, p.out_act);
+        float v = apply_act((MM == 3 ? acc[i][j][r] * o_mul : acc[i][j][r]) + bv, p.out_act);
         if (row < M && cval) {
           p.out[(size_t)row * p.ld_out + col] = v;
           if (do_stats) {
@@ -406,7 +481,7 @@
 }
 
 template <int BM, int BN, int WGM, int WGN, int MODE, int MM>
-int launch_mm(const G6dConv& d, int M, int T, int nChunks, int splits, hipStream_t stream) {
+int launch_mm(const G6dConv& d, const G6dRange16& rng, int M, int T, int nChunks, int splits, hipStream_t stream) {
   const int total = T * nChunks;
   const int ips = (total + splits - 1) / splits;
   splits = (total + ips - 1) / ips;
@@ -422,25 +497,35 @@
   const unsigned in_bytes = (unsigned)((n_in * d.Di * d.Hi * d.Wi * d.ld_in + pad_a) * 4);
   const unsigned w_bytes = (unsigned)((long long)d.Cout * T * d.Cin * 4);
   const unsigned mul_bytes = (unsigned)((n_mul * d.Hi * d.Wi * d.Cin + pad_m) * 4);
-  hipLaunchKernelGGL((conv_igemm_kernel<BM, BN, WGM, WGN, MODE, MM>), grid, dim3(256), lds_bytes, stream, d, M, T, nChunks,
+  G6dConv k = d;
+  if constexpr (MM == 3) {
+    k.weight_wino = nullptr;
+    k.weight_wino16 = rng.exps && rng.slot_out >= 0 ? rng.exps + rng.slot_out : nullptr;
+    k.weight_wino43 = rng.rec && rng.slot_out >= 0 ? reinterpret_cast<const float*>(rng.rec + rng.slot_out) : nullptr;
+  }
+  hipLaunchKernelGGL((conv_igemm_kernel<BM, BN, WGM, WGN, MODE, MM>), grid, dim3(256), lds_bytes, stream, k, M, T, nChunks,
                      ips, total, splits, in_bytes, w_bytes, mul_bytes, pm_hw, pm_tiles, ny);
   return g6d_check_launch("conv_igemm");
 }
 
 template <int BM, int BN, int WGM, int WGN, int MODE>
-int launch_mode(const G6dConv& d, int M, int T, int nChunks, int splits, hipStream_t stream) {
-  if (d.math_mode == 1) return launch_mm<BM, BN, WGM, WGN, MODE, 1>(d, M, T, nChunks, splits, stream);
-  if (d.math_mode == 2) return launch_mm<BM, BN, WGM, WGN, MODE, 2>(d, M, T, nChunks, splits, stream);
-  return launch_mm<BM, BN, WGM, WGN, MODE, 0>(d, M, T, nChunks, splits, stream);
+int launch_mode(const G6dConv& d, const G6dRange16& rng, int M, int T, int nChunks, int splits, hipStream_t stream) {
+  if (d.math_mode == 1) return launch_mm<BM, BN, WGM, WGN, MODE, 1>(d, rng, M, T, nChunks, splits, stream);
+  if (d.math_mode == 2) return launch_mm<BM, BN, WGM, WGN, MODE, 2>(d, rng, M, T, nChunks, splits, stream);
+  if (d.math_mode == 3) {
+    if constexpr (MODE <= 2 && BN >= 64 && !(BN == 128 && MODE == 2)) return launch_mm<BM, BN, WGM, WGN, MODE, 3>(d, rng, M, T, nChunks, splits, stream);
+    g6d_set_error("conv: math_mode 3 (fp16 pairs) has no kernel for this tile / prologue"); return G6D_EINVAL;
+  }
+  return launch_mm<BM, BN, WGM, WGN, MODE, 0>(d, rng, M, T, nChunks, splits, stream);
 }
 
 template <int BM, int BN, int WGM, int WGN>
-int launch_cfg(const G6dConv& d, int M, int T, int nChunks, int splits, hipStream_t stream) {
-  if (d.mul) return d.in_affine_per_n ? launch_mode<BM, BN, WGM, WGN, 4>(d, M, T, nChunks, splits, stream)
-                                      : launch_mode<BM, BN, WGM, WGN, 3>(d, M, T, nChunks, splits, stream);
-  if (!d.in_scale) return launch_mode<BM, BN, WGM, WGN, 0>(d, M, T, nChunks, splits, stream);
-  if (d.in_affine_per_n) return launch_mode<BM, BN, WGM, WGN, 2>(d, M, T, nChunks, splits, stream);
-  return launch_mode<BM, BN, WGM, WGN, 1>(d, M, T, nChunks, splits, stream);
+int launch_cfg(const G6dConv& d, const G6dRange16& rng, int M, int T, int nChunks, int splits, hipStream_t stream) {
+  if (d.mul) return d.in_affine_per_n ? launch_mode<BM, BN, WGM, WGN, 4>(d, rng, M, T, nChunks, splits, stream)
+                                      : launch_mode<BM, BN, WGM, WGN, 3>(d, rng, M, T, nChunks, splits, stream);
+  if (!d.in_scale) return launch_mode<BM, BN, WGM, WGN, 0>(d, rng, M, T, nChunks, splits, stream);
+  if (d.in_affine_per_n) return launch_mode<BM, BN, WGM, WGN, 2>(d, rng, M, T, nChunks, splits, stream);
+  return launch_mode<BM, BN, WGM, WGN, 1>(d, rng, M, T, nChunks, splits, stream);
 }
 
 constexpr int NARROW_RUN = 8;
@@ -531,6 +616,7 @@
 
 extern "C" int g6d_conv_plan(const G6dConv* desc) {
   if (!desc) return G6D_EINVAL;
+  if (desc->math_mode == 3) return 5;
   if (conv_narrow_eligible(*desc)) return 4;
   if (g6d_wino43_eligible(*desc)) return 3;
   if (g6d_wino_eligible(*desc)) return 2;
@@ -538,12 +624,23 @@
   return (use_patch && g6d_conv_patch_eligible(*desc)) ? 1 : 0;
 }
 
-extern "C" int g6d_conv_igemm(const G6dConv* desc, g6d_stream_t stream_) {
+extern "C" int g6d_conv_igemm(const G6dConv* desc, g6d_stream_t stream_) { return g6d_conv_igemm_ex(desc, nullptr, stream_); }
+
+extern "C" int g6d_conv_igemm_ex(const G6dConv* desc, const G6dRange16* range, g6d_stream_t stream_) {
   if (!desc) return G6D_EINVAL;
   const G6dConv& d = *desc;
+  const G6dRange16 rng = range ? *range : G6dRange16{nullptr, nullptr, -1, -1};
   hipStream_t stream = reinterpret_cast<hipStream_t>(stream_);
   if (!d.in || !d.weight || !d.out) { g6d_set_error("conv: null pointer"); return G6D_EINVAL; }
-  if (d.math_mode < 0 || d.math_mode > 2) { g6d_set_error("conv: math_mode must be 0 (fp32), 1 (bf16) or 2 (fp16)"); return G6D_EINVAL; }
+  if (d.math_mode < 0 || d.math_mode > 3) { g6d_set_error("conv: math_mode must be 0 (fp32), 1 (bf16), 2 (fp16) or 3 (fp16 pairs)"); return G6D_EINVAL; }
+  const bool pairs = d.math_mode == 3;
+  if (pairs) {
+    if (d.weight_wino16) { g6d_set_error("conv: math_mode 3 (fp16 pairs) runs on the implicit-GEMM kernel: weight_wino16 must be NULL"); return G6D_EINVAL; }
+    if (d.Cin & 7) { g6d_set_error("conv: math_mode 3 (fp16 pairs) needs Cin % 8 == 0 (a fragment is 8 channels of one plane)"); return G6D_EINVAL; }
+    if (d.Cout <= 32) { g6d_set_error("conv: math_mode 3 (fp16 pairs) needs Cout > 32 (no 32-channel tile)"); return G6D_EINVAL; }
+    if (d.mul) { g6d_set_error("conv: math_mode 3 (fp16 pairs) takes no multiplier"); return G6D_EINVAL; }
+    if (d.w_exp < -64 || d.w_exp > 64) { g6d_set_error("conv: w_exp out of range (|w_exp| <= 64)"); return G6D_EINVAL; }
+  } else if (range) { g6d_set_error("conv: a G6dRange16 applies to math_mode 3 only"); return G6D_EINVAL; }
   if (d.N <= 0 || d.Cin <= 0 || d.Cout <= 0 || d.Do <= 0 || d.Ho <= 0 || d.Wo <= 0 || d.kd <= 0 || d.kh <= 0 || d.kw <= 0) {
     g6d_set_error("conv: bad shape"); return G6D_EINVAL;
   }
@@ -571,11 +668,13 @@
   const long long Mll = (long long)d.N * d.Do * d.Ho * d.Wo;
   if (Mll > (1ll << 30)) { g6d_set_error("conv: M too large"); return G6D_EINVAL; }
   const int M = (int)Mll;
-  if (conv_narrow_eligible(d)) return conv_narrow_launch(d, stream);
-  if (g6d_wino43_eligible(d)) return g6d_wino43_launch(d, stream);
-  if (g6d_wino_eligible(d)) return g6d_wino_launch(d, stream);
-  const bool use_patch = g6d_knob(G6D_KNOB_CONV_PATCH) != 0;
-  if (use_patch && g6d_conv_patch_eligible(d)) return g6d_conv_patch_launch(d, M, stream);
+  if (!pairs) {
+    if (conv_narrow_eligible(d)) return conv_narrow_launch(d, stream);
+    if (g6d_wino43_eligible(d)) return g6d_wino43_launch(d, stream);
+    if (g6d_wino_eligible(d)) return g6d_wino_launch(d, stream);
+    const bool use_patch = g6d_knob(G6D_KNOB_CONV_PATCH) != 0;
+    if (use_patch && g6d_conv_patch_eligible(d)) return g6d_conv_patch_launch(d, M, stream);
+  }
   const int T = d.kd * d.kh * d.kw;
   const int nChunks = (d.Cin + BK - 1) / BK;
   const int total = T * nChunks;
@@ -617,8 +716,8 @@
       if (splits < 2) splits = 1;
     }
   }
-  if (bm == 64) return launch_cfg<64, 64, 2, 2>(d, M, T, nChunks, splits, stream);
-  if (bn == 32) return launch_cfg<128, 32, 4, 1>(d, M, T, nChunks, splits, stream);
-  if (bn == 64) return launch_cfg<128, 64, 2, 2>(d, M, T, nChunks, splits, stream);
-  return launch_cfg<128, 128, 2, 2>(d, M, T, nChunks, splits, stream);
-}
+  if (bm == 64) return launch_cfg<64, 64, 2, 2>(d, rng, M, T, nChunks, splits, stream);
+  if (bn == 32) return launch_cfg<128, 32, 4, 1>(d, rng, M, T, nChunks, splits, stream);
+  if (bn == 64) return launch_cfg<128, 64, 2, 2>(d, rng, M, T, nChunks, splits, stream);
+  return launch_cfg<128, 128, 2, 2>(d, rng, M, T, nChunks, splits, stream);
+}
diff --git a/gen6d_amd/lib.py b/gen6d_amd/lib.py
--- a/gen6d_amd/lib.py
+++ b/gen6d_amd/lib.py
@@ -64,11 +64,21 @@
     ]
 
 
+def _conv_init(self, *a, w_exp=0, **k):
+    C.Structure.__init__(self, *a, **k)
+    if w_exp:
+        self.reserved_ = int(w_exp)
+
+
+G6dConv.__init__ = _conv_init
+G6dConv.w_exp = property(lambda self: self.reserved_, lambda self, v: setattr(self, "reserved_", int(v)))
+
 _P, _I, _F, _D = C.c_void_p, C.c_int, C.c_float, C.c_double
 
 SIGNATURES = {
     "g6d_marker": [_I, _P],
     "g6d_conv_igemm": [C.POINTER(G6dConv), _P],
+    "g6d_conv_igemm_ex": [C.POINTER(G6dConv), _P, _P],
     "g6d_conv_plan": [C.POINTER(G6dConv)],
     "g6d_corr2d_patch": [_P, _I, _I, _I, _I, _P, _I, _I, _I, _P, _I, _P, C.c_size_t, _I, _P],
     "g6d_corr2d_patch_multi": [_P, _I, _I, _P, _I, _I, _I, _P, C.c_size_t, _I, _P],
diff --git a/gen6d_amd/network/refiner.py b/gen6d_amd/network/refiner.py
--- a/gen6d_amd/network/refiner.py
+++ b/gen6d_amd/network/refiner.py
@@ -11,6 +11,7 @@
 FEATNET_F43_LAYERS = {("conv1", 0), ("conv_out", 0), ("conv_out", 3)}
 FEATNET_PAIR_BRANCHES = ("conv0", "conv1", "conv2", "conv_out")
 VOLUME_PAIR_LAYERS = ("mean_embed", "var_embed", "conv0", "conv2")
+VOLUME_IGEMM_PAIR_LAYERS = ("conv1", "conv3", "conv5.0", "conv5.3")
 VOLUME_F43_LAYERS = ("conv0",)
 MAX_BATCH = 32
 _K3, _P3 = (3, 3, 3), (1, 1, 1)
@@ -102,6 +103,8 @@
             for name in ("conv0", "conv1", "conv2", "conv3", "conv4"):
                 pk["v_" + name] = self.conv_w(f"volume_net.{name}.0", wino_kd=3 if name in ("conv0", "conv2", "conv4") else 0,
                                               f43=name in VOLUME_F43_LAYERS)
+            for wb in (pk["v_conv1"], pk["v_conv3"], pk["v_conv4"], pk["v_conv5"][0], pk["v_conv5"][1]):
+                ops.pair_filter_prepare(wb[0])
             w = self.p("regressor.fc.0.0.weight")
             pk["fc0"] = (w.reshape(512, 512, 64).permute(0, 2, 1).reshape(512, 32768).contiguous(),
                          self.p("regressor.fc.0.0.bias").contiguous())
@@ -229,15 +232,16 @@
         qn = mean_in.shape[0] if batched else 1
         pn = 1 if qn > 1 else 0
 
-        def c3(x, wb, out, stride=1, aff=None, stats_c=None, count=None):
+        def c3(x, wb, out, stride=1, aff=None, stats_c=None, count=None, name=None):
             st = ops.new_stats(qn, stats_c, dev) if stats_c else None
             sc, sh = aff if aff is not None else (None, None)
+            r = self._pair_rng() if (qn >= F43_MIN_QUERIES and name in VOLUME_IGEMM_PAIR_LAYERS) else None
+            route = {"pairs": (r, r.slot(f"volume.{name}.igemm"))} if r is not None else \
+                {"w_wino": getattr(wb, "u", None) if stride == 1 else None,
+                 "w_wino43": getattr(wb, "u43", None) if (stride == 1 and qn >= F43_MIN_QUERIES) else None}
             return ops.conv(x, wb[0], wb[1], out, ksize=_K3, stride=(stride,) * 3, pad=_P3, in_scale=sc, in_shift=sh,
                             in_relu=aff is not None, per_n=pn if aff is not None else 0, stats=st,
-                            rows_per_group=pn * (count or 0) if stats_c else 0,
-                            w_wino=getattr(wb, "u", None) if stride == 1 else None,
-                            w_wino43=getattr(wb, "u43", None) if (stride == 1 and qn >= F43_MIN_QUERIES) else None,
-                            finalize=count if stats_c else None)
+                            rows_per_group=pn * (count or 0) if stats_c else 0, finalize=count if stats_c else None, **route)
 
         def buf(s, c):
             return torch.empty((qn, s, s, s, c), dtype=torch.float32, device=dev)
@@ -287,13 +291,13 @@
                     xin = ops.affine_split16(x.view(qn * s, 1, s, s, 128), aff[0], aff[1], s, True, False, 3, rng=(rng, rng.slot("volume.conv2.in")))
                     x, aff = y, c16(pk[name], xin.view(qn, s, s, s, 2, 128), y, stats_c=co, count=s ** 3)
                     continue
-                x, aff = y, c3(x, pk[name], y, stride=stride, aff=aff, stats_c=co, count=s ** 3)
+                x, aff = y, c3(x, pk[name], y, stride=stride, aff=aff, stats_c=co, count=s ** 3, name=name[2:])
         s = s // 2
         y = buf(s, 512)
         with self._mm("tail"):
-            aff = c3(x, pk["v_conv5"][0], y, stride=2, aff=aff, stats_c=512, count=s ** 3)
+            aff = c3(x, pk["v_conv5"][0], y, stride=2, aff=aff, stats_c=512, count=s ** 3, name="conv5.0")
             code = buf(s, 512)
-            c3(y, pk["v_conv5"][1], code, aff=aff)
+            c3(y, pk["v_conv5"][1], code, aff=aff, name="conv5.3")
         return code.view(qn, s ** 3, 512) if batched else code.view(s ** 3, 512)
 
     def run_regressor(self, code):
diff --git a/gen6d_amd/network/selector.py b/gen6d_amd/network/selector.py
--- a/gen6d_amd/network/selector.py
+++ b/gen6d_amd/network/selector.py
@@ -14,6 +14,7 @@
 _K133, _P011 = (1, 3, 3), (0, 1, 1)
 MAX_BATCH = 32
 FEAT_LD = 516
+SELECTOR_IGEMM_PAIR_LAYERS = ()
 
 
 class ViewpointSelector(ParamBank):
@@ -239,7 +240,9 @@
             y = torch.empty((qn * D, 1, 4, 4, 512), dtype=torch.float32, device=dev)
             st = ops.new_stats(qn, 512, dev)
             if not self.sharded:
-                sc, sh = ops.conv(cat, pk["fuse0"][0], pk["fuse0"][1], y, stats=st, finalize=Dg * 16, rows_per_group=grp * 16)
+                r = self._pair_rng() if (qn > 1 and "fuse0" in SELECTOR_IGEMM_PAIR_LAYERS) else None
+                kw = {"pairs": (r, r.slot("fuse0.igemm"))} if r is not None else {}
+                sc, sh = ops.conv(cat, pk["fuse0"][0], pk["fuse0"][1], y, stats=st, finalize=Dg * 16, rows_per_group=grp * 16, **kw)
             else:
                 ops.conv(cat, pk["fuse0"][0], pk["fuse0"][1], y, stats=st, rows_per_group=grp * 16)
                 self._allreduce([st])
diff --git a/gen6d_amd/ops.py b/gen6d_amd/ops.py
--- a/gen6d_amd/ops.py
+++ b/gen6d_amd/ops.py
@@ -119,7 +119,7 @@
 
 def conv(x, w, bias, out, ksize=(1, 1, 1), stride=(1, 1, 1), pad=(0, 0, 0), mul=None, in_scale=None, in_shift=None,
          in_relu=False, per_n=False, out_act=0, stats=None, rows_per_group=0, split_k=0, w_wino=None, finalize=None, eps=1e-5,
-         in_mod=0, mul_group=0, w_wino43=None):
+         in_mod=0, mul_group=0, w_wino43=None, pairs=None):
     _need_gpu(x, w, out)
     Nx, Di, Hi, Wi, Cin, ld_in = _cl5(x, "conv.x")
     No, Do, Ho, Wo, Cout, ld_out = _cl5(out, "conv.out")
@@ -143,7 +143,12 @@
         raise ValueError(f"conv.w_wino: expected contiguous {(kd * (Cin // 8), 16, Cout, 8)}, got {tuple(w_wino.shape)}")
     if w_wino43 is not None and (tuple(w_wino43.shape) != w43_shape(kd * (Cin // 8), Cout) or not w_wino43.is_contiguous()):
         raise ValueError(f"conv.w_wino43: expected contiguous {w43_shape(kd * (Cin // 8), Cout)}, got {tuple(w_wino43.shape)}")
+    if MATH_MODE:
+        pairs = None
     u16 = None
+    if pairs is not None:
+        w_wino = w_wino43 = None
+        w_exp = pair_filter_prepare(w)
     if MATH_MODE and w_wino is not None and Cin % 16 == 0 and Cout % 64 == 0:
         cache = w_wino.__dict__.setdefault("_g6d_u16", {})
         if MATH_MODE not in cache:
@@ -160,7 +165,8 @@
         N=N, Di=Di, Hi=Hi, Wi=Wi, Cin=Cin, ld_in=ld_in, Do=Do, Ho=Ho, Wo=Wo, Cout=Cout, ld_out=ld_out,
         kd=kd, kh=kh, kw=kw, sd=stride[0], sh=stride[1], sw=stride[2], pd=pad[0], ph=pad[1], pw=pad[2],
         in_relu=int(in_relu), in_affine_per_n=int(per_n), out_act=int(out_act),
-        stat_rows_per_group=int(rows_per_group), split_k=int(split_k), math_mode=int(MATH_MODE),
+        stat_rows_per_group=int(rows_per_group), split_k=int(split_k), math_mode=3 if pairs is not None else int(MATH_MODE),
+        w_exp=int(w_exp) if pairs is not None else 0,
         weight_wino=w_wino.data_ptr() if w_wino is not None else None, in_image_mod=int(in_mod), mul_group_images=int(mul_group),
         weight_wino16=u16.data_ptr() if u16 is not None else None,
         weight_wino43=w_wino43.data_ptr() if (w_wino43 is not None and not MATH_MODE) else None)
@@ -183,10 +189,14 @@
                 PROFILE_HBM.setdefault("conv_narrow", []).append((4.0 * (N * Di * Hi * Wi * Cin + w.numel() + N * Do * Ho * Wo * Cout), e0, e1))
         else:
             PROFILE.append((fl / 4 if fam == 3 else (fl / 2.25 if fam == 2 else fl), e0, e1,
-                        ("wino3x3 F43 " if fam == 3 else "wino3x3 " if fam == 2 else "") + f"conv N={N} in={Di}x{Hi}x{Wi}x{Cin} out={Do}x{Ho}x{Wo}x{Cout} k={kd}x{kh}x{kw} s={stride[0]}{stride[1]}{stride[2]}"
+                        ("wino3x3 F43 " if fam == 3 else "wino3x3 " if fam == 2 else "conv16x3 igemm " if fam == 5 else "") + f"conv N={N} in={Di}x{Hi}x{Wi}x{Cin} out={Do}x{Ho}x{Wo}x{Cout} k={kd}x{kh}x{kw} s={stride[0]}{stride[1]}{stride[2]}"
                         f"{' mul' if mul is not None else ''}{' aff' if in_scale is not None else ''}{' stats' if stats is not None else ''}",
                         4.0 * ((in_mod or N) * Di * Hi * Wi * Cin + (mul.numel() if mul is not None else 0) + w.numel() + N * Do * Ho * Wo * Cout), fl))
-    _timed(PROFILE is not None, lambda: _lib.check(_lib.load().g6d_conv_igemm(C.byref(d), _stream()), "g6d_conv_igemm"), book)
+    if pairs is not None:
+        ra = C.byref(pairs[0].arg(-1, pairs[1]))
+        _timed(PROFILE is not None, lambda: _lib.check(_lib.load().g6d_conv_igemm_ex(C.byref(d), ra, _stream()), "g6d_conv_igemm_ex"), book)
+    else:
+        _timed(PROFILE is not None, lambda: _lib.check(_lib.load().g6d_conv_igemm(C.byref(d), _stream()), "g6d_conv_igemm"), book)
     if finalize is not None:
         return fin if fin is not None else stats_finalize(stats, finalize, eps)
     return out
@@ -635,8 +645,19 @@
         self.data, self.layout, self.mode, self.acc_scale, self.Cout, self.taps, self.Cin = data, layout, mode, acc_scale, Cout, taps, Cin
 
 
+def pair_filter_exponent(w_taps):
+    return min(14, math.floor(math.log2(2048.0 / max(float(w_taps.abs().max()), 1e-30))))
+
+
+def pair_filter_prepare(w):
+    e = w.__dict__.get("_g6d_w_exp")
+    if e is None:
+        e = w.__dict__["_g6d_w_exp"] = pair_filter_exponent(w)
+    return e
+
+
 def _split_hi_lo(w_taps):
-    S = 2.0 ** min(14, math.floor(math.log2(2048.0 / max(float(w_taps.abs().max()), 1e-30))))
+    S = 2.0 ** pair_filter_exponent(w_taps)
     w = w_taps.double() * S
     hi = w.to(torch.float16)
     return hi, (w - hi.double()).to(torch.float16), 1.0 / S
diff --git a/include/gen6d_hip.h b/include/gen6d_hip.h
--- a/include/gen6d_hip.h
+++ b/include/gen6d_hip.h
@@ -58,12 +58,14 @@
   int32_t fin_groups;
   int32_t in_image_mod;
   int32_t mul_group_images;
-  int32_t reserved_;
+  int32_t w_exp;
   const void* weight_wino16;
   const float* weight_wino43;
 } G6dConv;
 
 int g6d_conv_igemm(const G6dConv* desc, g6d_stream_t stream);
+struct G6dRange16;
+int g6d_conv_igemm_ex(const G6dConv* desc, const struct G6dRange16* range, g6d_stream_t stream);
 int g6d_conv_plan(const G6dConv* desc);
 int g6d_sizeof_conv_desc(void);
 
```

After: 360.3 (median of 6 runs). 1.7% higher.
